# larskaislaniemi/PyLamp

Hardware: AMD Instinct MI355X
Metric: stokes_heat_mic_cell_updates_per_s (higher is better)
Workload: dtype f64

## Files before the change

include/pylamp_hip.h:

```cpp
#ifndef PYLAMP_HIP_H
#define PYLAMP_HIP_H

#include <stddef.h>
#include <stdint.h>

#ifdef __cplusplus
extern "C" {
#endif

typedef struct pl_ctx pl_ctx;

enum { PL_BC_NOSLIP = 0, PL_BC_FREESLIP = 1, PL_BC_CYCLIC = 2, PL_BC_FLOWTHRU = 4 };
enum { PL_BC_FIXTEMP = 0, PL_BC_FIXFLOW = 1 };
enum { PL_AVG_ARITHMETIC = 1, PL_AVG_GEOMETRIC = 2, PL_AVG_WEIGHTED = 4 };
enum { PL_INTERP_NEAREST = 8, PL_INTERP_LINEAR = 16, PL_INTERP_VELDIV = 32 };

typedef struct pl_solve_stats {
    int    iterations;
    int    converged;
    double rel_residual;
    double solve_ms;
    int    operator_applies;
    int    precond_applies;
    int    used_direct;
    int    reserved_;
    double error_estimate;
} pl_solve_stats;

int  pl_create(pl_ctx** out, int device, int nz, int nx, const double* zc, const double* xc);
void pl_destroy(pl_ctx* ctx);
const char* pl_last_error(const pl_ctx* ctx);
int  pl_sync(pl_ctx* ctx);
int  pl_device_info(pl_ctx* ctx, char* name, size_t name_len, int* cu_count, size_t* hbm_bytes);

typedef struct pl_comm_ops {
    int (*sendrecv)(void* user, int nmsg, const int* peer, const double* const* send, const int64_t* nsend,
                    double* const* recv, const int64_t* nrecv);
    int (*allreduce_host)(void* user, double* buf, int64_t n, int op);
    int (*allgather)(void* user, const double* send, double* recv, int64_t count);
    void* user;
} pl_comm_ops;
int  pl_set_comm(pl_ctx* ctx, int rank, int nranks, const pl_comm_ops* ops);
int  pl_set_comm_2d(pl_ctx* ctx, int rank, int Pz, int Px, const pl_comm_ops* ops);
int  pl_local_rows(pl_ctx* ctx, int* first_row, int* n_rows);
int  pl_local_block(pl_ctx* ctx, int* first_row, int* n_rows, int* first_col, int* n_cols, int* Pz, int* Px);
typedef struct pl_local_group pl_local_group;
int  pl_local_group_create(pl_local_group** out, int nranks);
void pl_local_group_destroy(pl_local_group* g);
void pl_local_group_abort(pl_local_group* g);
int  pl_set_comm_local(pl_ctx* ctx, pl_local_group* g, int rank, int Pz, int Px);
void pl_local_group_enter(pl_local_group* g);
void pl_local_group_leave(pl_local_group* g, pl_ctx* ctx);
int  pl_comm_info(pl_ctx* ctx, int* rank, int* nranks, int* native);
int  pl_comm_stats(pl_ctx* ctx, int64_t out[4], int reset);
int  pl_comm_times(pl_ctx* ctx, double out_ms[4], int reset);
int  pl_memcpy_d2h(pl_ctx* ctx, void* dst_host, const void* src_dev, size_t bytes);
int  pl_memcpy_h2d(pl_ctx* ctx, void* dst_dev, const void* src_host, size_t bytes);
int  pl_dev_add(pl_ctx* ctx, double* dst_dev, const double* src_dev, int64_t n);

int  pl_timer_start(pl_ctx* ctx);
int  pl_timer_stop_ms(pl_ctx* ctx, double* ms);

int  pl_stokes_set_coeffs(pl_ctx* ctx, const double* etas, const double* etan, const double* rho,
                          const int bc[4], int surfstab, double tstep, double theta);
int  pl_stokes_get_scaling(pl_ctx* ctx, double* kcont, double* kbond);
int  pl_stokes_apply(pl_ctx* ctx, const double* x, double* y);
int  pl_stokes_rhs(pl_ctx* ctx, double* rhs);
int  pl_stokes_residual_dd(pl_ctx* ctx, const double* rhs, const double* x, double* r);
int  pl_stokes_direct_info(pl_ctx* ctx, int* band, int* nb, double* factor_ms, double* solve_ms, int* nsolve);
int  pl_stokes_solve(pl_ctx* ctx, const double* rhs, double* x, int use_x0, double rtol,
                     int maxit, pl_solve_stats* stats);
int  pl_stokes_apply_bench(pl_ctx* ctx, int reps, double* avg_ms);
int  pl_stokes_apply_scaled_bench(pl_ctx* ctx, int reps, double* avg_ms);
int  pl_stream_triad_bench(pl_ctx* ctx, int64_t n, int reps, double* avg_ms);

int  pl_stokes_precond_apply(pl_ctx* ctx, const double* r, double* z);
int  pl_stokes_apply_reduce(pl_ctx* ctx, int mode, int rows, const double* x, const double* aux1, const double* aux2,
                            double* out, double* out2, double* sums);
int  pl_stokes_apply_probe(pl_ctx* ctx, int scaled, int mode, int rows, const double* x, const double* aux1,
                           const double* aux2, const double* add, double coef, double* out, double* out2, double* sums);
int  pl_stokes_scale_rows(pl_ctx* ctx, const double* v, double* out);
int  pl_stokes_mg_info(pl_ctx* ctx, int* nlevels, double* lmax, int max_levels);
int  pl_stokes_mg_plan(pl_ctx* ctx, int* smoother, int max_levels, int* nu, double* ratio, int* wall_ps);
int  pl_stokes_sweep_bench(pl_ctx* ctx, int reps, double* avg_ms);
int  pl_stokes_mg_precision(pl_ctx* ctx, int* nlevels, int* nlevels_fp32);
int  pl_stokes_set_mg_precision(pl_ctx* ctx, int fp32, long long min_nodes);
int  pl_mg_tail_launches(pl_ctx* ctx, long long* lds, long long* global);

int  pl_heat_set_coeffs(pl_ctx* ctx, const double* zmp, const double* xmp, const double* T,
                        const double* kz, const double* kx, const double* cp, const double* rho,
                        const double* H, const int bc[4], const double bcvalue[4], double tstep);
int  pl_heat_apply(pl_ctx* ctx, const double* x, double* y);
int  pl_heat_rhs(pl_ctx* ctx, double* rhs);
int  pl_heat_solve(pl_ctx* ctx, const double* rhs, double* x, double rtol, int maxit,
                   pl_solve_stats* stats);
int  pl_heat_apply_bench(pl_ctx* ctx, int reps, double* avg_ms);
int  pl_heat_fused_launches(pl_ctx* ctx, long long* n);

int  pl_trac2grid(pl_ctx* ctx, int64_t n, const double* tr_x, const double* tr_f, int64_t ld_f,
                  int nf, const int* avgscheme, double z0, double hz, double x0, double hx,
                  double* const* out);
int  pl_trac2grid_rect(pl_ctx* ctx, int64_t n, const double* tr_x, const double* tr_f, int64_t ld_f,
                       int nf, const int* avgscheme, const double* zc, const double* xc, double* const* out);
int  pl_mic_set_search(pl_ctx* ctx, int on);
int  pl_grid2trac(pl_ctx* ctx, int64_t n, const double* tr_x, int nf, const double* const* fields,
                  int gnz, int gnx, const double* gz, const double* gx, int method, double defval,
                  int stop_on_error, double* out, int64_t ld_out, int64_t* n_outside);
int  pl_rk4(pl_ctx* ctx, int64_t n, const double* tr_x, int gnz, int gnx, const double* gz,
            const double* gx, const double* vz, const double* vx, double tstep, double* v_out,
            double* x_out);

typedef struct pl_step_config {
    int    do_heatdiff, do_subgrid_heatdiff, tdep_rho, tdep_eta;
    double etamin, etamax, tref;
    double tstep_adv_max, tstep_adv_min, tstep_dif_max, tstep_dif_min, tstep_modifier;
    int    bcstokes[4];
    int    bcheat[4];
    double bcheatvals[4];
    double stokes_rtol, heat_rtol;
    int    stokes_maxit, heat_maxit;
    double length[2];
    int    tracdens, tracdens_min;
    uint64_t inject_seed;
    int    surface_stabilization;
    double surfstab_theta, surfstab_tstep;
    int    inject_unique_ids;
    int    tracs_fence_disabled;
} pl_step_config;

typedef struct pl_step_report {
    double tstep;
    int    limiter;
    double tstep_heat, tstep_stokes;
    pl_solve_stats stokes, heat;
    double ms_props, ms_scatter, ms_stokes, ms_heat, ms_gather, ms_advect, ms_sort, ms_total;
    int64_t ntrac;
    int64_t ninjected;
    int     stokes_resolves;
    int64_t nremoved;
} pl_step_report;

int  pl_tracers_upload(pl_ctx* ctx, int64_t n, const double* tr_x, const double* tr_f);
int  pl_tracers_download(pl_ctx* ctx, int64_t n, double* tr_x, double* tr_f);
int  pl_tracers_count(pl_ctx* ctx, int64_t* n);
int  pl_tracers_census(pl_ctx* ctx, int64_t ncells, int32_t* counts, int* first_cell_row, int* n_cell_rows);
int  pl_tracers_layout(pl_ctx* ctx, int* epoch_age, int* lazy);
int  pl_step(pl_ctx* ctx, const pl_step_config* cfg, int it, pl_step_report* rep);
int  pl_resident_scatter(pl_ctx* ctx, const pl_step_config* cfg, int it);
int  pl_resident_temp_to_tracers(pl_ctx* ctx, const pl_step_config* cfg, int first, const double* newtemp, double tstep);
int  pl_resident_rk4(pl_ctx* ctx, const double* vz_pad, const double* vx_pad, double tstep, int fence, const double length[2]);
int  pl_get_field(pl_ctx* ctx, const char* name, double* out);
int  pl_get_tracer_velocity(pl_ctx* ctx, int64_t n, double* out);

typedef struct pl3_ctx pl3_ctx;
int  pl3_create(pl3_ctx** out, int device, int nz, int nx, int ny, const double* zc, const double* xc, const double* yc);
void pl3_destroy(pl3_ctx* ctx);
const char* pl3_last_error(const pl3_ctx* ctx);
int  pl3_set_comm(pl3_ctx* ctx, pl_ctx* comm, int Pz, int Px, int Py);
int  pl3_local_block(pl3_ctx* ctx, int first[3], int count[3]);
int  pl3_comm_stats(pl3_ctx* ctx, int64_t out[2], int reset);
int  pl3_stokes_set_coeffs(pl3_ctx* ctx, const double* etas, const double* etan, const double* rho, const double grav[3]);
int  pl3_stokes_set_wall_rows(pl3_ctx* ctx, int slaved);
int  pl3_stokes_set_walls(pl3_ctx* ctx, const int bc[6]);
int  pl3_stokes_set_wall_velocity(pl3_ctx* ctx, const double vel[18]);
int  pl3_stokes_get_wall_velocity(pl3_ctx* ctx, double vel[18]);
int  pl3_stokes_get_scaling(pl3_ctx* ctx, double* kcont, double* kbond);
int  pl3_stokes_apply(pl3_ctx* ctx, const double* x, double* y);
int  pl3_stokes_rhs(pl3_ctx* ctx, double* rhs);
int  pl3_stokes_rhs_scaled(pl3_ctx* ctx, double* rhs);
int  pl3_stokes_solve(pl3_ctx* ctx, const double* rhs, double* x, int use_x0, double rtol, int maxit, pl_solve_stats* stats);
int  pl3_stokes_apply_bench(pl3_ctx* ctx, int scaled, int reps, double* avg_ms);
int  pl3_stokes_mg_info(pl3_ctx* ctx, int* nlevels, double* lmax, int max_levels);
int  pl3_stokes_precond_apply(pl3_ctx* ctx, const double* r, double* z);
int  pl3_stokes_mg_plan(pl3_ctx* ctx, int* nu, double* ratio, int* coarse_sweeps, double* coarse_ratio, int* lds, int max_levels);
int  pl3_heat_set_coeffs(pl3_ctx* ctx, const double* zmp, const double* xmp, const double* ymp, const double* T, const double* kz,
                         const double* kx, const double* ky, const double* cp, const double* rho, const double* H, const int bc[6],
                         const double bcvalue[6], double tstep);
int  pl3_heat_apply(pl3_ctx* ctx, const double* x, double* y);
int  pl3_heat_rhs(pl3_ctx* ctx, double* rhs);
int  pl3_heat_solve(pl3_ctx* ctx, const double* rhs, double* x, double rtol, int maxit, pl_solve_stats* stats);
int  pl3_get_solution(pl3_ctx* ctx, int which, double* out);

int  pl3_trac2grid(pl3_ctx* ctx, int64_t n, const double* tr_x, const double* tr_f, int64_t ld_f, int nf, const int* avgscheme,
                   const double* zc, int nzc, const double* xc, int nxc, const double* yc, int nyc, double* const* out);
int  pl3_grid2trac(pl3_ctx* ctx, int64_t n, const double* tr_x, int nf, const double* const* fields, int gnz, int gnx, int gny,
                   const double* gz, const double* gx, const double* gy, int method, double defval, int stop_on_error, double* out,
                   int64_t ld_out, int64_t* n_outside);
int  pl3_rk4(pl3_ctx* ctx, int64_t n, const double* tr_x, int gnz, int gnx, int gny, const double* gz, const double* gx, const double* gy,
             const double* vz, const double* vx, const double* vy, double tstep, double* v_out, double* x_out);
int  pl3_mic_set_search(pl3_ctx* ctx, int on);
int  pl3_mic_get_search(pl3_ctx* ctx, int* on);
int  pl3_mic_set_deletion(pl3_ctx* ctx, int on);
int  pl3_mic_get_deletion(pl3_ctx* ctx, int* on);
int  pl3_tracers_removed(pl3_ctx* ctx, int64_t out[2]);
int  pl3_tracers_upload(pl3_ctx* ctx, int64_t n, const double* tr_x, const double* tr_f);
int  pl3_tracers_download(pl3_ctx* ctx, int64_t n, double* tr_x, double* tr_f);
int  pl3_tracers_count(pl3_ctx* ctx, int64_t* n);
int  pl3_tracers_census(pl3_ctx* ctx, int64_t ncell, int32_t* counts);
int  pl3_resident_props(pl3_ctx* ctx, int tdep_rho, int tdep_eta, double tref, double etamin, double etamax);
int  pl3_resident_trac2grid(pl3_ctx* ctx, int nf, const int* columns, const int* avgscheme, const double* zc, int nzc, const double* xc,
                            int nxc, const double* yc, int nyc, double* const* out);
int  pl3_resident_temp_to_tracers(pl3_ctx* ctx, int absolute, const double* field, int subgrid, double tstep);
int  pl3_resident_rk4(pl3_ctx* ctx, const double* gz, const double* gx, const double* gy, const double* vz, const double* vx,
                      const double* vy, double tstep, int fence);
int  pl3_get_tracer_velocity(pl3_ctx* ctx, int64_t n, double* out);
int  pl3_resident_refill(pl3_ctx* ctx, int tracdens, int tracdens_min, uint64_t seed, int it, int unique_ids, int64_t out[4]);
int  pl3_resident_advect(pl3_ctx* ctx, const double* gz, const double* gx, const double* gy, const double* vz, const double* vx,
                         const double* vy, double tstep, int fence, int tracdens, int tracdens_min, uint64_t seed, int it,
                         int unique_ids, int64_t out[4]);
int  pl3_resident_times(pl3_ctx* ctx, double ms[4]);

typedef struct pl3_step_config {
    int    do_heatdiff, do_subgrid_heatdiff, tdep_rho, tdep_eta;
    double etamin, etamax, tref;
    double tstep_adv_max, tstep_adv_min, tstep_dif_max, tstep_dif_min, tstep_modifier;
    int    bcheat[6];
    double bcheatvals[6];
    double stokes_rtol, heat_rtol;
    int    stokes_maxit, heat_maxit;
    int    use_grav;
    int    reserved_;
    double grav[3];
    int    tracdens, tracdens_min;
    uint64_t inject_seed;
    int    inject_unique_ids;
    int    reserved2_;
} pl3_step_config;
typedef struct pl3_step_report {
    double tstep;
    int    limiter;
    int    reserved_;
    double tstep_heat, tstep_stokes;
    pl_solve_stats stokes, heat;
    int64_t ninjected, nrefilled, nempty, mincount;
    int64_t ntrac;
    int64_t nan_rho, nan_etas;
    double ms_scatter, ms_stokes, ms_heat, ms_gather, ms_rk4, ms_sort;
    double ms_total;
    int64_t nremoved;
} pl3_step_report;
// ... 13 lines not shown
```

pylamp_amd/_lib.py:

```python
import ctypes as C
import os

import numpy as np

_HERE = os.path.dirname(os.path.abspath(__file__))
LIB_PATH = os.path.join(_HERE, "libpylamp_hip.so")

c_double_p = C.POINTER(C.c_double)
c_int_p = C.POINTER(C.c_int)


class SolveStats(C.Structure):
    _fields_ = [("iterations", C.c_int), ("converged", C.c_int), ("rel_residual", C.c_double),
                ("solve_ms", C.c_double), ("operator_applies", C.c_int), ("precond_applies", C.c_int),
                ("used_direct", C.c_int), ("reserved_", C.c_int), ("error_estimate", C.c_double)]

    def as_dict(self):
        return {k: getattr(self, k) for k, _ in self._fields_}


class StepConfig(C.Structure):
    _fields_ = [("do_heatdiff", C.c_int), ("do_subgrid_heatdiff", C.c_int), ("tdep_rho", C.c_int),
                ("tdep_eta", C.c_int), ("etamin", C.c_double), ("etamax", C.c_double), ("tref", C.c_double),
                ("tstep_adv_max", C.c_double), ("tstep_adv_min", C.c_double), ("tstep_dif_max", C.c_double),
                ("tstep_dif_min", C.c_double), ("tstep_modifier", C.c_double), ("bcstokes", C.c_int * 4),
                ("bcheat", C.c_int * 4), ("bcheatvals", C.c_double * 4), ("stokes_rtol", C.c_double),
                ("heat_rtol", C.c_double), ("stokes_maxit", C.c_int), ("heat_maxit", C.c_int),
                ("length", C.c_double * 2), ("tracdens", C.c_int), ("tracdens_min", C.c_int),
                ("inject_seed", C.c_uint64), ("surface_stabilization", C.c_int), ("surfstab_theta", C.c_double),
                ("surfstab_tstep", C.c_double), ("inject_unique_ids", C.c_int), ("tracs_fence_disabled", C.c_int)]


class StepReport(C.Structure):
    _fields_ = [("tstep", C.c_double), ("limiter", C.c_int), ("tstep_heat", C.c_double),
                ("tstep_stokes", C.c_double), ("stokes", SolveStats), ("heat", SolveStats),
                ("ms_props", C.c_double), ("ms_scatter", C.c_double), ("ms_stokes", C.c_double),
                ("ms_heat", C.c_double), ("ms_gather", C.c_double), ("ms_advect", C.c_double),
                ("ms_sort", C.c_double), ("ms_total", C.c_double), ("ntrac", C.c_int64), ("ninjected", C.c_int64),
                ("stokes_resolves", C.c_int), ("nremoved", C.c_int64)]


class Step3Config(C.Structure):
    _fields_ = [("do_heatdiff", C.c_int), ("do_subgrid_heatdiff", C.c_int), ("tdep_rho", C.c_int), ("tdep_eta", C.c_int),
                ("etamin", C.c_double), ("etamax", C.c_double), ("tref", C.c_double),
                ("tstep_adv_max", C.c_double), ("tstep_adv_min", C.c_double), ("tstep_dif_max", C.c_double),
                ("tstep_dif_min", C.c_double), ("tstep_modifier", C.c_double), ("bcheat", C.c_int * 6),
                ("bcheatvals", C.c_double * 6), ("stokes_rtol", C.c_double), ("heat_rtol", C.c_double),
                ("stokes_maxit", C.c_int), ("heat_maxit", C.c_int), ("use_grav", C.c_int), ("reserved_", C.c_int),
                ("grav", C.c_double * 3), ("tracdens", C.c_int), ("tracdens_min", C.c_int), ("inject_seed", C.c_uint64),
                ("inject_unique_ids", C.c_int), ("reserved2_", C.c_int)]


class Step3Report(C.Structure):
    _fields_ = [("tstep", C.c_double), ("limiter", C.c_int), ("reserved_", C.c_int), ("tstep_heat", C.c_double),
                ("tstep_stokes", C.c_double), ("stokes", SolveStats), ("heat", SolveStats),
                ("ninjected", C.c_int64), ("nrefilled", C.c_int64), ("nempty", C.c_int64), ("mincount", C.c_int64),
                ("ntrac", C.c_int64), ("nan_rho", C.c_int64), ("nan_etas", C.c_int64),
                ("ms_scatter", C.c_double), ("ms_stokes", C.c_double), ("ms_heat", C.c_double), ("ms_gather", C.c_double),
                ("ms_rk4", C.c_double), ("ms_sort", C.c_double), ("ms_total", C.c_double), ("nremoved", C.c_int64)]


SIGNATURES = {
    "pl_create": (C.c_int, [C.POINTER(C.c_void_p), C.c_int, C.c_int, C.c_int, c_double_p, c_double_p]),
    "pl_destroy": (None, [C.c_void_p]),
    "pl_last_error": (C.c_char_p, [C.c_void_p]),
    "pl_sync": (C.c_int, [C.c_void_p]),
    "pl_abi_layout": (C.c_int, [C.POINTER(C.c_size_t)]),
    "pl3_create": (C.c_int, [C.POINTER(C.c_void_p), C.c_int, C.c_int, C.c_int, C.c_int, c_double_p, c_double_p, c_double_p]),
    "pl3_destroy": (None, [C.c_void_p]),
    "pl3_set_comm": (C.c_int, [C.c_void_p, C.c_void_p, C.c_int, C.c_int, C.c_int]),
    "pl3_local_block": (C.c_int, [C.c_void_p, c_int_p, c_int_p]),
    "pl3_comm_stats": (C.c_int, [C.c_void_p, C.POINTER(C.c_int64), C.c_int]),
    "pl3_last_error": (C.c_char_p, [C.c_void_p]),
    "pl3_stokes_set_coeffs": (C.c_int, [C.c_void_p, c_double_p, c_double_p, c_double_p, c_double_p]),
    "pl3_stokes_set_wall_rows": (C.c_int, [C.c_void_p, C.c_int]),
    "pl3_stokes_set_walls": (C.c_int, [C.c_void_p, C.POINTER(C.c_int)]),
    "pl3_stokes_set_wall_velocity": (C.c_int, [C.c_void_p, c_double_p]),
    "pl3_stokes_get_wall_velocity": (C.c_int, [C.c_void_p, c_double_p]),
    "pl3_stokes_get_scaling": (C.c_int, [C.c_void_p, c_double_p, c_double_p]),
    "pl3_stokes_apply": (C.c_int, [C.c_void_p, c_double_p, c_double_p]),
    "pl3_stokes_rhs": (C.c_int, [C.c_void_p, c_double_p]),
    "pl3_stokes_rhs_scaled": (C.c_int, [C.c_void_p, c_double_p]),
    "pl3_stokes_solve": (C.c_int, [C.c_void_p, c_double_p, c_double_p, C.c_int, C.c_double, C.c_int, C.POINTER(SolveStats)]),
    "pl3_stokes_apply_bench": (C.c_int, [C.c_void_p, C.c_int, C.c_int, c_double_p]),
    "pl3_stokes_mg_info": (C.c_int, [C.c_void_p, c_int_p, c_double_p, C.c_int]),
    "pl3_stokes_precond_apply": (C.c_int, [C.c_void_p, c_double_p, c_double_p]),
    "pl3_stokes_mg_plan": (C.c_int, [C.c_void_p, c_int_p, c_double_p, c_int_p, c_double_p, c_int_p, C.c_int]),
    "pl3_heat_set_coeffs": (C.c_int, [C.c_void_p] + [c_double_p] * 10 + [c_int_p, c_double_p, C.c_double]),
    "pl3_heat_apply": (C.c_int, [C.c_void_p, c_double_p, c_double_p]),
    "pl3_heat_rhs": (C.c_int, [C.c_void_p, c_double_p]),
    "pl3_heat_solve": (C.c_int, [C.c_void_p, c_double_p, c_double_p, C.c_double, C.c_int, C.POINTER(SolveStats)]),
    "pl3_get_solution": (C.c_int, [C.c_void_p, C.c_int, c_double_p]),
    "pl3_trac2grid": (C.c_int, [C.c_void_p, C.c_int64, c_double_p, c_double_p, C.c_int64, C.c_int, c_int_p, c_double_p, C.c_int,
                                c_double_p, C.c_int, c_double_p, C.c_int, C.POINTER(c_double_p)]),
    "pl3_grid2trac": (C.c_int, [C.c_void_p, C.c_int64, c_double_p, C.c_int, C.POINTER(c_double_p), C.c_int, C.c_int, C.c_int,
                                c_double_p, c_double_p, c_double_p, C.c_int, C.c_double, C.c_int, c_double_p, C.c_int64,
                                C.POINTER(C.c_int64)]),
    "pl3_rk4": (C.c_int, [C.c_void_p, C.c_int64, c_double_p, C.c_int, C.c_int, C.c_int] + [c_double_p] * 6 +
                [C.c_double, c_double_p, c_double_p]),
    "pl3_mic_set_search": (C.c_int, [C.c_void_p, C.c_int]),
    "pl3_mic_get_search": (C.c_int, [C.c_void_p, c_int_p]),
    "pl3_mic_set_deletion": (C.c_int, [C.c_void_p, C.c_int]),
    "pl3_mic_get_deletion": (C.c_int, [C.c_void_p, c_int_p]),
    "pl3_tracers_removed": (C.c_int, [C.c_void_p, C.POINTER(C.c_int64)]),
    "pl3_tracers_upload": (C.c_int, [C.c_void_p, C.c_int64, c_double_p, c_double_p]),
    "pl3_tracers_download": (C.c_int, [C.c_void_p, C.c_int64, c_double_p, c_double_p]),
    "pl3_tracers_count": (C.c_int, [C.c_void_p, C.POINTER(C.c_int64)]),
    "pl3_tracers_census": (C.c_int, [C.c_void_p, C.c_int64, C.POINTER(C.c_int32)]),
    "pl3_resident_props": (C.c_int, [C.c_void_p, C.c_int, C.c_int, C.c_double, C.c_double, C.c_double]),
    "pl3_resident_trac2grid": (C.c_int, [C.c_void_p, C.c_int, c_int_p, c_int_p, c_double_p, C.c_int, c_double_p, C.c_int,
                                         c_double_p, C.c_int, C.POINTER(c_double_p)]),
    "pl3_resident_temp_to_tracers": (C.c_int, [C.c_void_p, C.c_int, c_double_p, C.c_int, C.c_double]),
    "pl3_resident_rk4": (C.c_int, [C.c_void_p] + [c_double_p] * 6 + [C.c_double, C.c_int]),
    "pl3_get_tracer_velocity": (C.c_int, [C.c_void_p, C.c_int64, c_double_p]),
    "pl3_resident_refill": (C.c_int, [C.c_void_p, C.c_int, C.c_int, C.c_uint64, C.c_int, C.c_int, C.POINTER(C.c_int64)]),
    "pl3_resident_advect": (C.c_int, [C.c_void_p] + [c_double_p] * 6 + [C.c_double, C.c_int, C.c_int, C.c_int, C.c_uint64, C.c_int, C.c_int,
                                      C.POINTER(C.c_int64)]),
    "pl3_resident_times": (C.c_int, [C.c_void_p, c_double_p]),
    "pl3_resident_step": (C.c_int, [C.c_void_p, C.POINTER(Step3Config), C.c_int, C.POINTER(Step3Report)]),
    "pl3_get_field": (C.c_int, [C.c_void_p, C.c_char_p, c_double_p]),
    "pl3_advection_velocity": (C.c_int, [C.c_void_p] + [c_double_p] * 6),
    "pl3_transfer_stats": (C.c_int, [C.c_void_p, C.POINTER(C.c_int64), C.c_int]),
    "pl3_abi_layout": (C.c_int, [C.POINTER(C.c_size_t)]),
    "pl_device_info": (C.c_int, [C.c_void_p, C.c_char_p, C.c_size_t, c_int_p, C.POINTER(C.c_size_t)]),
    "pl_set_comm": (C.c_int, [C.c_void_p, C.c_int, C.c_int, C.c_void_p]),
    "pl_set_comm_2d": (C.c_int, [C.c_void_p, C.c_int, C.c_int, C.c_int, C.c_void_p]),
    "pl_local_rows": (C.c_int, [C.c_void_p, c_int_p, c_int_p]),
    "pl_local_block": (C.c_int, [C.c_void_p, c_int_p, c_int_p, c_int_p, c_int_p, c_int_p, c_int_p]),
    "pl_local_group_create": (C.c_int, [C.POINTER(C.c_void_p), C.c_int]),
    "pl_local_group_destroy": (None, [C.c_void_p]),
    "pl_local_group_abort": (None, [C.c_void_p]),
    "pl_local_group_enter": (None, [C.c_void_p]),
    "pl_local_group_leave": (None, [C.c_void_p, C.c_void_p]),
    "pl_set_comm_local": (C.c_int, [C.c_void_p, C.c_void_p, C.c_int, C.c_int, C.c_int]),
    "pl_comm_info": (C.c_int, [C.c_void_p, c_int_p, c_int_p, c_int_p]),
    "pl_comm_stats": (C.c_int, [C.c_void_p, C.POINTER(C.c_int64), C.c_int]),
    "pl_comm_times": (C.c_int, [C.c_void_p, c_double_p, C.c_int]),
    "pl_memcpy_d2h": (C.c_int, [C.c_void_p, C.c_void_p, C.c_void_p, C.c_size_t]),
    "pl_memcpy_h2d": (C.c_int, [C.c_void_p, C.c_void_p, C.c_void_p, C.c_size_t]),
    "pl_dev_add": (C.c_int, [C.c_void_p, c_double_p, c_double_p, C.c_int64]),
    "pl_timer_start": (C.c_int, [C.c_void_p]),
    "pl_timer_stop_ms": (C.c_int, [C.c_void_p, c_double_p]),
    "pl_stokes_set_coeffs": (C.c_int, [C.c_void_p, c_double_p, c_double_p, c_double_p, c_int_p, C.c_int,
                                       C.c_double, C.c_double]),
    "pl_stokes_get_scaling": (C.c_int, [C.c_void_p, c_double_p, c_double_p]),
    "pl_stokes_apply": (C.c_int, [C.c_void_p, c_double_p, c_double_p]),
    "pl_stokes_rhs": (C.c_int, [C.c_void_p, c_double_p]),
    "pl_stokes_residual_dd": (C.c_int, [C.c_void_p, c_double_p, c_double_p, c_double_p]),
    "pl_stokes_direct_info": (C.c_int, [C.c_void_p, c_int_p, c_int_p, c_double_p, c_double_p, c_int_p]),
    "pl_stokes_solve": (C.c_int, [C.c_void_p, c_double_p, c_double_p, C.c_int, C.c_double, C.c_int,
                                  C.POINTER(SolveStats)]),
    "pl_stokes_apply_bench": (C.c_int, [C.c_void_p, C.c_int, c_double_p]),
    "pl_stokes_apply_scaled_bench": (C.c_int, [C.c_void_p, C.c_int, c_double_p]),
    "pl_stream_triad_bench": (C.c_int, [C.c_void_p, C.c_int64, C.c_int, c_double_p]),
    "pl_stokes_precond_apply": (C.c_int, [C.c_void_p, c_double_p, c_double_p]),
    "pl_stokes_apply_reduce": (C.c_int, [C.c_void_p, C.c_int, C.c_int] + [c_double_p] * 6),
    "pl_stokes_apply_probe": (C.c_int, [C.c_void_p, C.c_int, C.c_int, C.c_int] + [c_double_p] * 4 + [C.c_double] + [c_double_p] * 3),
    "pl_stokes_scale_rows": (C.c_int, [C.c_void_p, c_double_p, c_double_p]),
    "pl_stokes_mg_info": (C.c_int, [C.c_void_p, c_int_p, c_double_p, C.c_int]),
    "pl_stokes_mg_plan": (C.c_int, [C.c_void_p, c_int_p, C.c_int, c_int_p, c_double_p, c_int_p]),
    "pl_stokes_mg_precision": (C.c_int, [C.c_void_p, c_int_p, c_int_p]),
    "pl_stokes_set_mg_precision": (C.c_int, [C.c_void_p, C.c_int, C.c_longlong]),
    "pl_stokes_sweep_bench": (C.c_int, [C.c_void_p, C.c_int, c_double_p]),
    "pl_mg_tail_launches": (C.c_int, [C.c_void_p, C.POINTER(C.c_longlong), C.POINTER(C.c_longlong)]),
    "pl_heat_set_coeffs": (C.c_int, [C.c_void_p] + [c_double_p] * 8 + [c_int_p, c_double_p, C.c_double]),
    "pl_heat_apply": (C.c_int, [C.c_void_p, c_double_p, c_double_p]),
    "pl_heat_rhs": (C.c_int, [C.c_void_p, c_double_p]),
    "pl_heat_solve": (C.c_int, [C.c_void_p, c_double_p, c_double_p, C.c_double, C.c_int, C.POINTER(SolveStats)]),
    "pl_heat_apply_bench": (C.c_int, [C.c_void_p, C.c_int, c_double_p]),
    "pl_heat_fused_launches": (C.c_int, [C.c_void_p, C.POINTER(C.c_longlong)]),
    "pl_trac2grid": (C.c_int, [C.c_void_p, C.c_int64, c_double_p, c_double_p, C.c_int64, C.c_int, c_int_p,
                               C.c_double, C.c_double, C.c_double, C.c_double, C.POINTER(c_double_p)]),
    "pl_trac2grid_rect": (C.c_int, [C.c_void_p, C.c_int64, c_double_p, c_double_p, C.c_int64, C.c_int, c_int_p,
                                    c_double_p, c_double_p, C.POINTER(c_double_p)]),
    "pl_mic_set_search": (C.c_int, [C.c_void_p, C.c_int]),
    "pl_grid2trac": (C.c_int, [C.c_void_p, C.c_int64, c_double_p, C.c_int, C.POINTER(c_double_p), C.c_int,
                               C.c_int, c_double_p, c_double_p, C.c_int, C.c_double, C.c_int, c_double_p,
                               C.c_int64, C.POINTER(C.c_int64)]),
    "pl_rk4": (C.c_int, [C.c_void_p, C.c_int64, c_double_p, C.c_int, C.c_int, c_double_p, c_double_p,
                         c_double_p, c_double_p, C.c_double, c_double_p, c_double_p]),
    "pl_tracers_upload": (C.c_int, [C.c_void_p, C.c_int64, c_double_p, c_double_p]),
    "pl_tracers_download": (C.c_int, [C.c_void_p, C.c_int64, c_double_p, c_double_p]),
    "pl_tracers_count": (C.c_int, [C.c_void_p, C.POINTER(C.c_int64)]),
    "pl_tracers_census": (C.c_int, [C.c_void_p, C.c_int64, C.POINTER(C.c_int32), c_int_p, c_int_p]),
    "pl_tracers_layout": (C.c_int, [C.c_void_p, c_int_p, c_int_p]),
    "pl_step": (C.c_int, [C.c_void_p, C.POINTER(StepConfig), C.c_int, C.POINTER(StepReport)]),
    "pl_resident_scatter": (C.c_int, [C.c_void_p, C.POINTER(StepConfig), C.c_int]),
    "pl_resident_temp_to_tracers": (C.c_int, [C.c_void_p, C.POINTER(StepConfig), C.c_int, c_double_p, C.c_double]),
    "pl_resident_rk4": (C.c_int, [C.c_void_p, c_double_p, c_double_p, C.c_double, C.c_int, c_double_p]),
    "pl_get_field": (C.c_int, [C.c_void_p, C.c_char_p, c_double_p]),
    "pl_get_tracer_velocity": (C.c_int, [C.c_void_p, C.c_int64, c_double_p]),
}

_lib = None


def load():
    global _lib
    if _lib is not None:
        return _lib
    if not os.path.exists(LIB_PATH):
        raise Exception("pylamp_amd: %s is missing — run `python -c 'import __graft_entry__ as g; g.build()'` "
                        "(there is no CPU fallback)" % LIB_PATH)
    try:
        import torch
    except Exception:
        pass
    lib = C.CDLL(LIB_PATH)
    for name, (res, args) in SIGNATURES.items():
        fn = getattr(lib, name)
        fn.restype = res
        fn.argtypes = args
    _lib = lib
    return lib


def dptr(a):
    return a.ctypes.data_as(c_double_p)


def f64(a):
    return np.ascontiguousarray(a, dtype=np.float64)


def check(ctx_handle, rc):
    if rc != 0:
        msg = load().pl_last_error(ctx_handle)
        raise Exception(msg.decode() if msg else "libpylamp_hip error %d" % rc)
```

pylamp_amd/csrc/pl_solver.hip:

```cpp
#include "pl_internal.h"
#include <chrono>
#include <cmath>
#include <functional>
#include <limits>

#define TB(tab, k) (tab)[(k) + PL_TOFF]

void pl_launch_heat_rhs(pl_ctx* ctx, const PlHeatOp& op, const double* Told, const double* H, double* rhs);

template <typename T>
struct PlVvOpT {
    PlGeom g;
    const T* etas; const T* etan;
    const T *rdz, *rDz, *rdx, *rDx;
    int slave_x;
    int slave_z0, slave_zL;
    T s0, sL;
    const T* szz; const T* szx;
};
typedef PlVvOpT<double> PlVvOp;
typedef PlVvOpT<float> PlVvOpF;

enum { VV_ZERO = 0, VV_INT = 1, VV_SLAVE = 2 };

// ... 1145 lines not shown
        fx = rs[c + P] * sum + 2.0 * op.Kc * rDx_j * (zp_c - prec_p_value(op, rs_p, i, j - 1, c - 1));
    }
    f[c] = (TF)(fz * fscale); f[c + P] = (TF)(fx * fscale); z[c + 2 * P] = zp_c;
}

template <typename TF>
__global__ __launch_bounds__(256) void k_prec_stage1(PlStokesOp op, PlVvOpT<TF> vop, const double* __restrict__ rs,
                                                     double* __restrict__ z, TF* __restrict__ f, int iters, double fscale) {
    PL_ROW_LOOP(op.g, iters) stage1_node(op, vop, rs, z, f, li, lj, fscale);
}

template <typename TF>
__global__ __launch_bounds__(256) void k_prec_stage1_v2(PlStokesOp op, PlVvOpT<TF> vop, const double* __restrict__ rs,
                                                        double* __restrict__ z, TF* __restrict__ f, TF* __restrict__ v1, double c2,
                                                        double fscale, double v1scale) {
    typedef typename PlVec2<TF>::type VF2;
    const PlGeom& g = op.g;
    const int lane = threadIdx.x;
    const int lj0 = (blockIdx.x * 64 + lane) * 2;
    const int li = blockIdx.y * 4 + threadIdx.y;
    if (li >= g.lnz) return;
    const bool has_right = (lj0 + 2) < g.lnx;
    const int p = g.pitch, nz = g.nz, nx = g.nx;
    const long long PLN = g.plane;
    const int c = (int)pl_idx(g, li, lj0);
    const int i = g.gi0 + li;
    const int jw = g.gj0 + blockIdx.x * 128;
    (void)nz; (void)nx;
    if (!stage1_fast_wave(g, i, jw, blockIdx.x, op.anchor_i, op.anchor_j, op.wall_ps)) {
        for (int q = 0; q < 2 && lj0 + q < g.lnx; q++) stage1_node(op, vop, rs, z, f, li, lj0 + q, fscale);
        return;
    }
#define ROW(ptr, dr, w, e) load_row2((ptr) + (long long)c - lj0 + (long long)(dr) * p, lj0, true, w, e, lane, has_right)
    const double2 rz = *reinterpret_cast<const double2*>(rs + c), rx = *reinterpret_cast<const double2*>(rs + PLN + c);
    const Row2 rp_i = ROW(rs + 2 * PLN, 0, true, false), rp_s = ROW(rs + 2 * PLN, -1, false, false);
    const Row2 en_s = ROW(op.etan, -1, false, false), en_i = ROW(op.etan, 0, true, false);
    const Row2 es_i = ROW(op.etas, 0, false, true), es_n = ROW(op.etas, 1, false, false);
#undef ROW
    const Row2 t_rdx = load_row2(g.rdx + PL_TOFF + g.gj0, lj0, true, true, false, lane, has_right);
    const Row2 t_rDx = load_row2(g.rDx + PL_TOFF + g.gj0, lj0, true, false, true, lane, has_right);
    const double rdz_i = TB(g.rdz, i), rdz_m = TB(g.rdz, i - 1), rDz_i = TB(g.rDz, i), rDz_p = TB(g.rDz, i + 1);
    const double Az = 4.0 * rdz_i * rDz_i, Azm = 4.0 * rdz_m * rDz_i, r2 = 2.0 * rdz_i, twoKc = 2.0 * op.Kc, Pz = twoKc * rDz_i;
    const double iKc = op.iKc;
    double fz[2], fx[2], zp[2], dz[2], dx[2];
    {
        const double rdx_j = t_rdx.v.x, rdx_m = t_rdx.w, rDx_j = t_rDx.v.x, rDx_p = t_rDx.v.y, k2 = 2.0 * rdx_j, B4 = 4.0 * rDx_j;
        zp[0] = rp_i.v.x * (rdx_j + rdz_i) * en_i.v.x * iKc;
        const double zp_s = rp_s.v.x * (rdx_j + rdz_m) * en_s.v.x * iKc, zp_w = rp_i.w * (rdx_m + rdz_i) * en_i.w * iKc;
        const double sz = en_i.v.x * Az + en_s.v.x * Azm + (es_i.v.y * k2) * rDx_p + (es_i.v.x * k2) * rDx_j;
        const double sx = en_i.v.x * (B4 * rdx_j) + en_i.w * (B4 * rdx_m) + (es_n.v.x * r2) * rDz_p + (es_i.v.x * r2) * rDz_i;
        fz[0] = rz.x * sz + Pz * (zp[0] - zp_s);
        fx[0] = rx.x * sx + (twoKc * rDx_j) * (zp[0] - zp_w);
        dz[0] = sz; dx[0] = sx;
    }
    {
        const double rdx_j = t_rdx.v.y, rdx_m = t_rdx.v.x, rDx_j = t_rDx.v.y, rDx_p = t_rDx.e, k2 = 2.0 * rdx_j, B4 = 4.0 * rDx_j;
        zp[1] = rp_i.v.y * (rdx_j + rdz_i) * en_i.v.y * iKc;
        const double zp_s = rp_s.v.y * (rdx_j + rdz_m) * en_s.v.y * iKc;
        const double sz = en_i.v.y * Az + en_s.v.y * Azm + (es_i.e * k2) * rDx_p + (es_i.v.y * k2) * rDx_j;
        const double sx = en_i.v.y * (B4 * rdx_j) + en_i.v.x * (B4 * rdx_m) + (es_n.v.y * r2) * rDz_p + (es_i.v.y * r2) * rDz_i;
        fz[1] = rz.y * sz + Pz * (zp[1] - zp_s);
        fx[1] = rx.y * sx + (twoKc * rDx_j) * (zp[1] - zp[0]);
        dz[1] = sz; dx[1] = sx;
    }
    *reinterpret_cast<VF2*>(f + c) = PlVec2<TF>::make((TF)(fz[0] * fscale), (TF)(fz[1] * fscale));
    *reinterpret_cast<VF2*>(f + PLN + c) = PlVec2<TF>::make((TF)(fx[0] * fscale), (TF)(fx[1] * fscale));
    *reinterpret_cast<double2*>(z + 2 * PLN + c) = make_double2(zp[0], zp[1]);
    if (v1) {
        const double nc2 = -c2 * v1scale;
        *reinterpret_cast<VF2*>(v1 + c) = PlVec2<TF>::make((TF)((nc2 * fz[0]) * pl_rcp(dz[0])), (TF)((nc2 * fz[1]) * pl_rcp(dz[1])));
        *reinterpret_cast<VF2*>(v1 + PLN + c) = PlVec2<TF>::make((TF)((nc2 * fx[0]) * pl_rcp(dx[0])), (TF)((nc2 * fx[1]) * pl_rcp(dx[1])));
    }
}

__global__ __launch_bounds__(256) void k_close_constraints(PlStokesOp op, PlVvOp vop, const double* __restrict__ bs,
                                                           double* __restrict__ x) {
    PL_NODE_PROLOGUE(op.g)
    const long long P = op.g.plane;
    int moff; double s;
    int cls = vv_cls_z(vop, i, j, moff, s);
    if (cls == VV_ZERO) x[c] = bs[c];
    else if (cls == VV_SLAVE) x[c] = s * x[c + moff] + bs[c];
    cls = vv_cls_x(vop, i, j, moff, s);
    if (cls == VV_ZERO) x[c + P] = bs[c + P];
    else if (cls == VV_SLAVE) {
        double g0 = bs[c + P];
        if (i == 0 && op.bc_z0 != PL_BC_FREESLIP) g0 /= (-TB(op.g.rDz, 1) - TB(op.g.rdz, 0));
        if (i == op.g.nz - 2 && op.bc_zL != PL_BC_FREESLIP) g0 /= (TB(op.g.rDz, op.g.nz - 2) + TB(op.g.rdz, op.g.nz - 2));
        x[c + P] = s * x[c + moff + P] + g0;
    }
}

#define PL_HYDRO_CHUNK 64
__global__ __launch_bounds__(64) void k_hydro_chunk(PlStokesOp op, double* __restrict__ x, double* __restrict__ ctot) {
    const PlGeom& g = op.g;
    const int lj = blockIdx.x * 64 + threadIdx.x, ch = blockIdx.y;
    if (lj >= g.lnx) return;
    double* P = x + 2 * g.plane;
    const double* r = op.rho;
    const int l0 = ch * PL_HYDRO_CHUNK, l1 = min(l0 + PL_HYDRO_CHUNK, g.lnz);
    const int jn = (g.gj0 + lj + 1 < g.nx) ? 1 : 0;
    double acc = 0.0;
    for (int li = l0; li < l1; li++) {
        const int i = g.gi0 + li;
        const long long c = pl_idx(g, li, lj);
        if (i >= 1 && i <= g.nz - 2) acc += 0.5 * (r[c] + r[c + jn]) * op.gz / (2.0 * op.Kc * TB(g.rDz, i));
        P[c] = acc;
    }
    ctot[(long long)ch * g.lnx + lj] = acc;
}
__global__ __launch_bounds__(64) void k_hydro_chunk_scan(PlGeom g, int nch, double* __restrict__ ctot, double* __restrict__ coltot) {
    const int lj = blockIdx.x * 64 + threadIdx.x;
    if (lj >= g.lnx) return;
    double acc = 0.0;
    for (int ch = 0; ch < nch; ch++) { const double t = ctot[(long long)ch * g.lnx + lj]; ctot[(long long)ch * g.lnx + lj] = acc; acc += t; }
    coltot[lj] = acc;
}
__global__ __launch_bounds__(256) void k_hydro_add(PlGeom g, double* __restrict__ x, const double* __restrict__ cpre) {
    PL_NODE_PROLOGUE(g)
    (void)i; (void)j;
    x[2 * g.plane + c] += cpre[(long long)(li / PL_HYDRO_CHUNK) * g.lnx + lj];
}

__global__ __launch_bounds__(256) void k_hydrostatic_apply_shift(PlStokesOp op, double* __restrict__ x,
                                                                 const double* __restrict__ prefix, double pa) {
    PL_NODE_PROLOGUE(op.g)
    const PlGeom& g = op.g;
    double* P = x + 2 * g.plane;
    x[c] = 0.0; x[c + g.plane] = 0.0;
    P[c] = (i >= g.nz - 1 || j >= g.nx - 1) ? 0.0 : P[c] + prefix[lj] - pa;
}

struct MgLevel {
    PlGeomHost gh;
    bool dist = false;
    PlGeom win{};
    long long win_shift = 0;
    PlVvOp op{};
    double* etas = nullptr; double* etan = nullptr; bool own_visc = false;
    double *rho = nullptr, *szz = nullptr, *szx = nullptr;
    double* eig = nullptr; bool eig_valid = false;
    int eig_confirm = 0, eig_skip = 0;
    bool own_rho = false;
    double* v[3] = {nullptr, nullptr, nullptr};
    double *f = nullptr, *r = nullptr;
    double lmax = 3.0;
    bool line_z = false;
    int line_ax = 0;
    bool f32 = false;
    PlVvOpF opf{};
    float *etas_f = nullptr, *etan_f = nullptr, *tab_f = nullptr;
    float* vf[3] = {nullptr, nullptr, nullptr};
    float *ff = nullptr, *rf = nullptr;
};
template <typename T> struct LevelT;
template <> struct LevelT<double> {
    static const PlVvOp& op(const MgLevel* L) { return L->op; }
    static double** v(MgLevel* L) { return L->v; }
    static double* f(MgLevel* L) { return L->f; }
    static double* r(MgLevel* L) { return L->r; }
};
template <> struct LevelT<float> {
    static const PlVvOpF& op(const MgLevel* L) { return L->opf; }
    static float** v(MgLevel* L) { return L->vf; }
    static float* f(MgLevel* L) { return L->ff; }
    static float* r(MgLevel* L) { return L->rf; }
};

struct PlSolver {
    std::vector<MgLevel*> levels;
    int bc_key[4] = {-1, -1, -1, -1};
    int repl_start = -1;
    long long repl_max_nodes = 300000;
    double *r = nullptr, *rt = nullptr, *p = nullptr, *v = nullptr, *s = nullptr, *t = nullptr, *y = nullptr,
           *z = nullptr, *b = nullptr, *x = nullptr, *xb = nullptr, *dx = nullptr, *r0 = nullptr, *xh = nullptr,
           *bu = nullptr;
    double* scal = nullptr;
    double* hpart = nullptr;
    double* epi = nullptr;
    long long epi_blocks = 0;
    int nu_pre = 2, nu_post = 2, coarse_sweeps = 12;
    int nu0_pre = -1, nu0_post = -1;
    bool aniso_auto = true, ratio_knob = false;
    int power_its_warm = 1;
    bool nu_auto = true;
    bool use_tail = true;
    bool any_line = false;
    long long tail_knob = 0;
    long long tail_max_nodes = 33 * 33;
    int min_cells = 4;
    bool f32_enable = false; long long f32_min_nodes = 200000;
    double etol = 3e-8;
    double kappa = 1.0, sigma = 1.0;
    bool defl_enable = true;
    bool defl_persistent = false;
    bool defl_valid = false, defl_active = false;
    double *wdefl = nullptr, *udefl = nullptr;
    double defl_yAw = 0.0, defl_wvel2 = 0.0;
    double* Awdefl = nullptr;
    bool defl_lazy = false;
    double schur_scale = 1.0;
    double ref_cached = 0.0, ref_kc = 0.0; int ref_age = 0;
    long long fused_max_nodes = 1100000;
    long long tile32_min_nodes = 250000;
    bool fused = true;
    bool fuse_first = true;
    bool l0_mixed = true;
    bool l0_mixed_now = true;
    bool deep = true;
    int tail_nu_pre = -1, tail_nu_post = -1;
    double cheb_ratio = 6.0, lmax_safety = 1.1;
    double* h[11] = {nullptr};
    double* hc3 = nullptr;
    double* hc[9] = {nullptr}; double* hc_part = nullptr; int hc_nb = 0, hc_last_its = 0;
    int napply = 0, nprec = 0;
    long long heat_fused_launches = 0;
    long long tail_lds_launches = 0, tail_global_launches = 0;
};

static PlSolver* solver_of(pl_ctx* ctx) {
    if (!ctx->krylov) {
        PlSolver* S = new PlSolver();
        if (const char* e = getenv("PYLAMP_MG_NU")) { int a = 0, b = 0; if (sscanf(e, "%d,%d", &a, &b) == 2 && a >= 0 && b >= 0 && a + b > 0) { S->nu_pre = a; S->nu_post = b; S->nu_auto = false; } }
        if (const char* e = getenv("PYLAMP_MG_NU0")) { int a = 0, b = 0; if (sscanf(e, "%d,%d", &a, &b) == 2 && a >= 1 && b >= 1) { S->nu0_pre = a; S->nu0_post = b; S->nu_auto = false; } }
        if (const char* e = getenv("PYLAMP_MG_POWER")) { int a = atoi(e); if (a >= 1) S->power_its_warm = a; }
        if (const char* e = getenv("PYLAMP_MG_COARSE")) { int a = atoi(e); if (a > 0) S->coarse_sweeps = a; }
        if (const char* e = getenv("PYLAMP_MG_TAIL")) S->use_tail = atoi(e) != 0;
        if (const char* e = getenv("PYLAMP_MG_REPL_NODES")) { long long v = atoll(e); if (v >= 25) S->repl_max_nodes = v; }
        if (const char* e = getenv("PYLAMP_MG_TAIL_NODES")) { long long v = atoll(e); if (v >= 25 && v <= PL_TAIL_MAX_NODES) S->tail_knob = v; }
        if (const char* e = getenv("PYLAMP_MG_DEEP")) S->deep = atoi(e) != 0;
        if (const char* e = getenv("PYLAMP_DEFLATE")) S->defl_enable = atoi(e) != 0;
        if (const char* e = getenv("PYLAMP_STOKES_ETOL")) { const double v = atof(e); if (v >= 0.0) S->etol = v; }
        if (const char* e = getenv("PYLAMP_MG_FP32")) S->f32_enable = atoi(e) != 0;
        if (const char* e = getenv("PYLAMP_MG_FP32_NODES")) { long long v = atoll(e); if (v >= 1) S->f32_min_nodes = v; }
        if (const char* e = getenv("PYLAMP_L0_MIXED")) S->l0_mixed = atoi(e) != 0;
        if (const char* e = getenv("PYLAMP_MG_FUSED")) S->fused = atoi(e) != 0;
        if (const char* e = getenv("PYLAMP_MG_TS32")) { long long v = atoll(e); if (v > 0) S->tile32_min_nodes = v; }
        if (const char* e = getenv("PYLAMP_MG_FUSED_MAX")) { long long v = atoll(e); if (v > 0) S->fused_max_nodes = v; }
        if (const char* e = getenv("PYLAMP_SCHUR_SCALE")) { double v = atof(e); if (v > 0.0) S->schur_scale = v; }
        if (const char* e = getenv("PYLAMP_MG_TAIL_NU")) { int a = 0, b = 0; if (sscanf(e, "%d,%d", &a, &b) == 2 && a + b > 0) { S->tail_nu_pre = a; S->tail_nu_post = b; } }
        if (const char* e = getenv("PYLAMP_MG_RATIO")) { double v = atof(e); if (v > 1.5) { S->cheb_ratio = v; S->ratio_knob = true; } }
        if (const char* e = getenv("PYLAMP_MG_ANISO")) S->aniso_auto = atoi(e) != 0;
        if (const char* e = getenv("PYLAMP_MG_SAFETY")) { double v = atof(e); if (v >= 1.0) S->lmax_safety = v; }
        ctx->krylov = S;
    }
    return (PlSolver*)ctx->krylov;
}

static void free_levels(PlSolver* S) {
    for (MgLevel* L : S->levels) {
        if (L->own_visc) { (void)hipFree(L->etas); (void)hipFree(L->etan); }
        if (L->own_rho && L->rho) (void)hipFree(L->rho);
        for (double* q : {L->szz, L->szx, L->eig}) if (q) (void)hipFree(q);
        for (double* q : {L->v[0], L->v[1], L->v[2], L->f, L->r}) if (q) (void)hipFree(q);
        for (float* q : {L->etas_f, L->etan_f, L->tab_f, L->vf[0], L->vf[1], L->vf[2], L->ff, L->rf}) if (q) (void)hipFree(q);
        pl_geom_free(L->gh);
        delete L;
    }
    S->levels.clear();
}

void pl_solver_free(pl_ctx* ctx) {
    PlSolver* S = (PlSolver*)ctx->krylov;
    if (!S) return;
    free_levels(S);
    for (double* q : {S->r, S->rt, S->p, S->v, S->s, S->t, S->y, S->z, S->b, S->x, S->xb, S->dx, S->r0, S->xh, S->bu, S->scal, S->wdefl, S->udefl, S->Awdefl})
        if (q) (void)hipFree(q);
    for (double* q : S->h) if (q) (void)hipFree(q);
    for (double* q : S->hc) if (q) (void)hipFree(q);
    if (S->hc_part) (void)hipFree(S->hc_part);
    if (S->hc3) (void)hipFree(S->hc3);
    if (S->hpart) (void)hipHostFree(S->hpart);
    if (S->epi) (void)hipFree(S->epi);
    delete S;
    ctx->krylov = nullptr;
}

static int dmalloc0(pl_ctx* ctx, double** p, size_t bytes) {
    PL_HIP(ctx, hipMalloc((void**)p, bytes));
    PL_HIP(ctx, hipMemsetAsync(*p, 0, bytes, ctx->stream));
    return 0;
}
static int scal_alloc(pl_ctx* ctx, PlSolver* S) {
    if (S->scal) return 0;
    PL_TRY(dmalloc0(ctx, &S->scal, (PL_SCAL_N + PL_PART_N * DOT_BLOCKS) * sizeof(double)));
    PL_HIP(ctx, hipHostMalloc((void**)&S->hpart, (PL_HSCAL + PL_SCAL_N) * sizeof(double)));
    return 0;
}

__global__ void k_scalar_alpha(double* __restrict__ sc, double rho_new) { sc[SC_ALPHA] = rho_new / sc[SC_SUM_A]; sc[SC_RHO] = rho_new; }
__global__ void k_s_update_dev(long long n, double* __restrict__ y, const double* __restrict__ a, const double* __restrict__ b,
                               const double* __restrict__ sc) {
    const double alpha = sc[SC_ALPHA];
    long long k = (long long)blockIdx.x * blockDim.x + threadIdx.x;
    for (; k < n; k += (long long)gridDim.x * blockDim.x) y[k] = a[k] - alpha * b[k];
}
template <bool FIRST>
__global__ void k_xrp_update_dev(long long n, double* __restrict__ x, const double* __restrict__ y, const double* __restrict__ z,
                                 double* __restrict__ r, const double* __restrict__ s, const double* __restrict__ t,
                                 double* __restrict__ p, const double* __restrict__ v, const double* __restrict__ sc,
                                 const double* __restrict__ wd, const double* __restrict__ awd, const double* __restrict__ p0) {
    const double alpha = sc[SC_ALPHA], omega = sc[SC_OMEGA], beta = sc[SC_BETA];
    const double cw = wd ? alpha * sc[SC_CY] + omega * sc[SC_CZ] : 0.0;
    const double cz = awd ? sc[SC_CZ] : 0.0;
    long long k = (long long)blockIdx.x * blockDim.x + threadIdx.x;
    for (; k < n; k += (long long)gridDim.x * blockDim.x) {
        double xn = FIRST ? alpha * y[k] + omega * z[k] : x[k] + alpha * y[k] + omega * z[k];
        if (wd) xn += cw * wd[k];
        x[k] = xn;
        const double rn = s[k] - omega * (awd ? t[k] + cz * awd[k] : t[k]);
        r[k] = rn;
        p[k] = rn + beta * ((FIRST ? p0[k] : p[k]) - omega * v[k]);
    }
}
__global__ void k_xr_update_dev(long long n, double* __restrict__ x, const double* __restrict__ y, const double* __restrict__ z,
                                double* __restrict__ r, const double* __restrict__ s, const double* __restrict__ t,
                                const double* __restrict__ sc) {
    const double alpha = sc[SC_ALPHA], omega = sc[SC_OMEGA];
    long long k = (long long)blockIdx.x * blockDim.x + threadIdx.x;
    for (; k < n; k += (long long)gridDim.x * blockDim.x) { x[k] += alpha * y[k] + omega * z[k]; r[k] = s[k] - omega * t[k]; }
}

__global__ __launch_bounds__(1024) void k_sum_partials(int nb, const double* __restrict__ part, double* __restrict__ out,
                                                       int mode = 0, double rho_new = 0.0) {
    double s0 = 0.0, s1 = 0.0;
    const int nt = blockDim.x, nw = nt >> 6;
#pragma unroll 2
    for (int k = threadIdx.x; k < nb; k += nt) { s0 += part[2 * k]; s1 += part[2 * k + 1]; }
    __shared__ double sh[2][16];
#pragma unroll
    for (int o = 32; o > 0; o >>= 1) { s0 += __shfl_down(s0, o, 64); s1 += __shfl_down(s1, o, 64); }
    if ((threadIdx.x & 63) == 0) { sh[0][threadIdx.x >> 6] = s0; sh[1][threadIdx.x >> 6] = s1; }
    __syncthreads();
    if (threadIdx.x == 0) {
        double a0 = sh[0][0], a1 = sh[1][0];
        for (int w = 1; w < nw; w++) { a0 += sh[0][w]; a1 += sh[1][w]; }
        out[0] = a0; out[1] = a1;
        if (mode == 1) { out[SC_ALPHA] = rho_new / a0; out[SC_RHO] = rho_new; }
    }
}

static int dots(pl_ctx* ctx, PlSolver* S, const PlGeom& g, int np, const double* a, const double* b, const double* c,
                const double* d, double* out2) {
    long long rows = (long long)g.lnz * np;
    const int nb = (int)(rows < DOT_BLOCKS ? rows : DOT_BLOCKS);
    if (a && c) hipLaunchKernelGGL((k_dot2<true, true>), dim3(nb), dim3(256), 0, ctx->stream, g, np, a, b, c, d, S->scal + SC_PART);
    else if (a) hipLaunchKernelGGL((k_dot2<true, false>), dim3(nb), dim3(256), 0, ctx->stream, g, np, a, b, c, d, S->scal + SC_PART);
    else hipLaunchKernelGGL((k_dot2<false, true>), dim3(nb), dim3(256), 0, ctx->stream, g, np, a, b, c, d, S->scal + SC_PART);
    if (ctx->nranks > 1 && pl_geom_is_dist(g)) {
        hipLaunchKernelGGL(k_sum_partials, dim3(1), dim3(256), 0, ctx->stream, nb, S->scal + SC_PART, S->scal + SC_SUM_A);
        PL_TRY(pl_comm_allreduce_dev(ctx, S->scal + SC_SUM_A, 2));
        PL_HIP(ctx, hipMemcpyAsync(S->hpart, S->scal + SC_SUM_A, 2 * sizeof(double), hipMemcpyDeviceToHost, ctx->stream));
        PL_HIP(ctx, hipStreamSynchronize(ctx->stream));
        out2[0] = S->hpart[0]; out2[1] = S->hpart[1];
        return 0;
    }
    PL_HIP(ctx, hipMemcpyAsync(S->hpart, S->scal + SC_PART, (size_t)2 * nb * sizeof(double), hipMemcpyDeviceToHost, ctx->stream));
    PL_HIP(ctx, hipStreamSynchronize(ctx->stream));
    double s0 = 0.0, s1 = 0.0;
    for (int k = 0; k < nb; k++) { s0 += S->hpart[2 * k]; s1 += S->hpart[2 * k + 1]; }
    out2[0] = s0; out2[1] = s1;
    return 0;
}

static int dots5_dev(pl_ctx* ctx, PlSolver* S, const PlGeom& g, int np, int nsplit, const double* t, const double* sv, const double* rt,
                     const double* aw_ride = nullptr) {
    long long rows = (long long)g.lnz * np;
    const int nb = (int)(rows < DOT_BLOCKS ? rows : DOT_BLOCKS);
    hipLaunchKernelGGL(k_dot5, dim3(nb), dim3(256), 0, ctx->stream, g, np, nsplit, t, sv, rt, S->scal + SC_PART);
    const bool reduce = ctx->nranks > 1 && pl_geom_is_dist(g);
    hipLaunchKernelGGL(k_sum_partials5, dim3(1), dim3(256), 0, ctx->stream, nb, S->scal + SC_PART, S->scal, reduce ? 0 : 1);
    if (reduce && aw_ride) {
        double* part2 = S->scal + SC_PART2;
        hipLaunchKernelGGL(k_dot4w, dim3(nb), dim3(256), 0, ctx->stream, g, np, nsplit, aw_ride, sv, t, part2);
        hipLaunchKernelGGL(k_sum_partials4, dim3(1), dim3(256), 0, ctx->stream, nb, (const double*)part2, S->scal + SC_AW_S);
        hipLaunchKernelGGL(k_bicg_pack_defl, dim3(1), dim3(64), 0, ctx->stream, S->scal);
        PL_TRY(pl_comm_allreduce_dev(ctx, S->scal + SC_STAGE, SC_STAGE_N));
        hipLaunchKernelGGL(k_bicg_unpack_defl, dim3(1), dim3(1), 0, ctx->stream, S->scal);
        return 0;
    }
    if (reduce) {
        PL_TRY(pl_comm_allreduce_dev(ctx, S->scal + SC_RED2, SC_RED2_N));
        hipLaunchKernelGGL(k_bicg_derive, dim3(1), dim3(1), 0, ctx->stream, S->scal);
    }
    return 0;
}
__global__ __launch_bounds__(256) void k_norm2_sum(PlGeom g, int nplanes, const double* __restrict__ a, const double* __restrict__ b,
                                                   double* __restrict__ part) {
    double s0 = 0.0;
// ... 410 lines not shown

static void level_nu(const PlSolver* S, size_t l, int& npre, int& npost) {
    npre = (l == 0 && S->nu0_pre > 0) ? S->nu0_pre : S->nu_pre;
    npost = (l == 0 && S->nu0_post > 0) ? S->nu0_post : S->nu_post;
}
static bool level_deep_plan(const PlSolver* S, const MgLevel* L, size_t l, int& e_last, int& f_depth) {
    int npre, npost;
    level_nu(S, l, npre, npost);
    e_last = std::max(2, npost);
    f_depth = e_last + std::max(npre, 1) - 1;
    if (!L->dist || !S->deep || l + 1 == S->levels.size() || npre < 1) return false;
    return f_depth <= PL_RING - 1 && f_depth + 1 <= std::min(L->gh.d.lnz, L->gh.d.lnx);
}

template <typename T> static void vcycle(pl_ctx* ctx, PlSolver* S, size_t l, const T* f, T** out, bool* wrote_final, double* final_out,
                                         double final_scale, int f_valid_depth, const int* first_done_anchor);
static bool mg_fused_level_ok(pl_ctx* ctx, const PlSolver* S, size_t l);
static bool mg_tail_lds_fits(const PlSolver* S, size_t l);
static bool mg_tail_cheb_fits(int nlev, int nu_pre, int nu_post, int coarse_sweeps);
__global__ void k_mg_tail_lds(TailArgs a);
static void vcycle_fused_level(pl_ctx* ctx, PlSolver* S, size_t l, const double* f, double** out, double* final_out, double final_scale,
                               const PlStokesOp* sop, const double* rs, double* z);

template <typename T, typename TC>
static void coarse_correction(pl_ctx* ctx, PlSolver* S, size_t l, MgLevel* L, MgLevel* C, T* buf[3], bool deep, int npost) {
    const PlGeom& g = L->gh.d;
    T* r = LevelT<T>::r(L);
    TC* cf = LevelT<TC>::f(C);
    const TC cscale = (std::is_same<T, float>::value && std::is_same<TC, double>::value) ? (TC)S->sigma : TC(1);
    if (L->dist && !C->dist) {
        PlVvOpT<TC> wop = LevelT<TC>::op(C); wop.g = C->win;
        const long long sh = C->win_shift;
        hipLaunchKernelGGL((k_vv_restrict<T, TC>), grid2d(C->win), dim3(64, 4), 0, ctx->stream, g, wop, (const T*)r, cf + sh, cscale);
        if constexpr (std::is_same<TC, double>::value) (void)pl_gather_blocks(ctx, C->gh.d, cf, 2, C->gh.d.plane);
    } else {
        hipLaunchKernelGGL((k_vv_restrict<T, TC>), grid2d(C->gh.d), dim3(64, 4), 0, ctx->stream, g, LevelT<TC>::op(C), (const T*)r, cf, cscale);
    }
    TC* ec = nullptr;
    bool wf = false;
    vcycle<TC>(ctx, S, l + 1, cf, &ec, &wf, nullptr, 1.0, 0, nullptr);
    const int pe = deep ? npost : (L->dist ? 1 : 0);
    if (C->dist)
        (void)pl_halo(ctx, C->gh.d, ec, 2, C->gh.d.plane, std::min(std::max((pe + 1) / 2 + 1, 2), std::min(PL_RING, std::min(C->gh.d.lnz, C->gh.d.lnx))));
    ExtViewT<T> V = ext_view<T>(ctx, L, pe);
    if (!deep && pe == 1) {
        V.op = LevelT<T>::op(L);
        const int lo = ctx->pz > 0 ? 1 : 0, hi = ctx->pz < ctx->Pz - 1 ? 1 : 0, we = ctx->px > 0 ? 1 : 0, ea = ctx->px < ctx->Px - 1 ? 1 : 0;
        V.op.g.gi0 -= lo; V.op.g.lnz += lo + hi; V.op.g.gj0 -= we; V.op.g.lnx += we + ea;
        V.sh = (long long)lo * g.pitch + we;
    }
    hipLaunchKernelGGL((k_vv_prolong_add<T, TC>), grid2d(V.op.g), dim3(64, 4), 0, ctx->stream, V.op, C->gh.d, (const TC*)ec, (const T*)(buf[0] - V.sh),
                       buf[2] - V.sh);
}

template <typename T>
static void vcycle(pl_ctx* ctx, PlSolver* S, size_t l, const T* f, T** out, bool* wrote_final, double* final_out,
                   double final_scale, int f_valid_depth, const int* first_done_anchor) {
    MgLevel* L = S->levels[l];
    const PlGeom& g = L->gh.d;
    *wrote_final = false;
    if constexpr (std::is_same<T, double>::value) {
        if (S->use_tail && !S->any_line && l > 0 && (long long)g.nz * g.nx <= S->tail_max_nodes &&
            S->levels.size() - l <= PL_TAIL_MAX_LEVELS && f == L->f) {
            TailArgs ta{};
            ta.nlev = (int)(S->levels.size() - l);
            ta.nu_pre = S->tail_nu_pre >= 0 ? S->tail_nu_pre : S->nu_pre; ta.nu_post = S->tail_nu_post >= 0 ? S->tail_nu_post : S->nu_post;
            ta.coarse_sweeps = coarsest_sweeps(S, S->levels.back()->gh.d); ta.ratio = S->cheb_ratio;
            for (int q = 0; q < ta.nlev; q++) {
                MgLevel* T_ = S->levels[l + q];
                ta.L[q].op = T_->op; ta.L[q].f = T_->f; ta.L[q].r = T_->r; ta.L[q].lmax = T_->lmax;
                for (int b = 0; b < 3; b++) ta.L[q].v[b] = T_->v[b];
            }
            if (S->fused && !L->dist && !L->op.szz && ta.nu_pre >= 1 && ta.nu_post >= 1 && ta.coarse_sweeps >= 1 && mg_tail_lds_fits(S, l) &&
                mg_tail_cheb_fits(ta.nlev, ta.nu_pre, ta.nu_post, ta.coarse_sweeps)) {
                hipLaunchKernelGGL(k_mg_tail_lds, dim3(1), dim3(1024), 0, ctx->stream, ta);
                S->tail_lds_launches++;
            } else {
                hipLaunchKernelGGL(k_mg_tail, dim3(1), dim3(1024), 0, ctx->stream, ta);
                S->tail_global_launches++;
            }
            *out = L->v[0];
            return;
        }
    }
    if constexpr (std::is_same<T, double>::value) {
        if (l > 0 && !final_out && f == L->f && mg_fused_level_ok(ctx, S, l)) {
            vcycle_fused_level(ctx, S, l, f, out, nullptr, 1.0, nullptr, nullptr, nullptr);
            return;
        }
    }
    T** lv = LevelT<T>::v(L);
    T* buf[3] = {lv[0], lv[1], lv[2]};
    const bool coarsest = l + 1 == S->levels.size();
    if (!coarsest && S->nu_pre == 0)
        (void)hipMemsetAsync(buf[0], 0, (size_t)2 * g.plane * sizeof(T), ctx->stream);
    if (coarsest) {
        double ratio = 0.4 * g.nz * g.nx; if (ratio < 30.0) ratio = 30.0;
        smooth<T>(ctx, L, buf, f, coarsest_sweeps(S, g), ratio, nullptr, 1.0, true);
        *out = buf[0];
        return;
    }
    int npre, npost, e_last, f_depth;
    level_nu(S, l, npre, npost);
    const bool deep = level_deep_plan(S, L, l, e_last, f_depth);
    MgLevel* C = S->levels[l + 1];
    T* r = LevelT<T>::r(L);
    if (deep) {
        if (f_valid_depth < f_depth) (void)pl_halo(ctx, g, (T*)f, 2, g.plane, f_depth);
        smooth<T>(ctx, L, buf, f, npre, S->cheb_ratio, nullptr, 1.0, true, false, e_last + npre - 1, first_done_anchor);
        const ExtViewT<T> V = ext_view<T>(ctx, L, e_last - 1);
        if (g_vv_vec)
            hipLaunchKernelGGL((k_vv_sweep2<1, T, T>), pl_grid_rows2(V.op.g), dim3(64, 4), 0, ctx->stream, V.op, (const T*)(buf[0] - V.sh),
                               (const T*)nullptr, f - V.sh, r - V.sh, T(0), T(0), T(1));
        else
            hipLaunchKernelGGL(k_vv_residual<T>, pl_grid_rows(V.op.g), dim3(64, 4), 0, ctx->stream, V.op, (const T*)(buf[0] - V.sh), f - V.sh,
                               r - V.sh, pl_row_iters(V.op.g));
    } else {
        smooth<T>(ctx, L, buf, f, npre, S->cheb_ratio, nullptr, 1.0, true, false, -1, first_done_anchor);
        if (L->dist) (void)pl_halo(ctx, g, buf[0], 2, g.plane);
        if (g_vv_vec)
            hipLaunchKernelGGL((k_vv_sweep2<1, T, T>), pl_grid_rows2(g), dim3(64, 4), 0, ctx->stream, LevelT<T>::op(L), (const T*)buf[0], (const T*)nullptr, f,
                               r, T(0), T(0), T(1));
        else
            hipLaunchKernelGGL(k_vv_residual<T>, pl_grid_rows(g), dim3(64, 4), 0, ctx->stream, LevelT<T>::op(L), (const T*)buf[0], f, r, pl_row_iters(g));
        if (L->dist) (void)pl_halo(ctx, g, r, 2, g.plane, 2);
    }
    if constexpr (std::is_same<T, float>::value) {
        if (C->f32) coarse_correction<float, float>(ctx, S, l, L, C, buf, deep, npost);
        else coarse_correction<float, double>(ctx, S, l, L, C, buf, deep, npost);
    } else {
        coarse_correction<double, double>(ctx, S, l, L, C, buf, deep, npost);
    }
    std::swap(buf[0], buf[2]);
    if (deep) *wrote_final = smooth<T>(ctx, L, buf, f, npost, S->cheb_ratio, final_out, final_scale, false, true, npost - 1);
    else *wrote_final = smooth<T>(ctx, L, buf, f, npost, S->cheb_ratio, final_out, final_scale, false, L->dist);
    *out = buf[0];
}

#define MGT_TS 16
#ifndef MGT_NT
#define MGT_NT 1024
#endif
struct MgTileArgs {
    PlVvOp op;
    PlVvOp opc;
    const double* f; double* fout;
    double* v;
    double* fc;
    const double* ec;
    double* out; double oscale; long long out_plane;
    double c1[4], c2[4];
    PlStokesOp sop; const double* rs; double* z;
    int tiles_x;
};

struct MgtTab { const double* es; const double* en; const double* rdz; const double* rDz; const double* rdx; const double* rDx; };

__device__ inline int mgt_cls_z(const PlVvOp& op, int i, int j, int& db, double& s) {
    db = 0; s = 1.0;
    if (i <= 0 || i >= op.g.nz - 1 || j < 0 || j >= op.g.nx - 1) return VV_ZERO;
    if (op.slave_x) {
        if (j == 0) { db = 1; return VV_SLAVE; }
        if (j == op.g.nx - 2) { db = -1; return VV_SLAVE; }
    }
    return VV_INT;
}
__device__ inline int mgt_cls_x(const PlVvOp& op, int i, int j, int& da, double& s) {
    const double s0 = op.s0, sL = op.sL;
    da = 0; s = 1.0;
    if (j <= 0 || j >= op.g.nx - 1 || i < 0 || i >= op.g.nz - 1) return VV_ZERO;
    if (i == 0 && op.slave_z0) da = 1;
    else if (i == op.g.nz - 2 && op.slave_zL) da = -1;
    s = da > 0 ? s0 : (da < 0 ? sL : 1.0);
    return da ? VV_SLAVE : VV_INT;
}
struct MgtC { double c0, c1, c2, c3, x0, x1, rdg, s, f; int cm, d; bool on, interior; };
template <bool ZC>
__device__ inline MgtC mgt_classify(const PlVvOp& op, int CR, int NR, int ci0, int cj0, int a, int b) {
    MgtC k; k.c0 = k.c1 = k.c2 = k.c3 = k.x0 = k.x1 = k.rdg = k.f = 0.0; k.s = 1.0; k.cm = a * CR + b; k.d = 0; k.on = false; k.interior = false;
    if (a < 1 || a > NR - 2 || b < 1 || b > CR - 2) return k;
    int d; double s;
    const int cls = ZC ? mgt_cls_z(op, ci0 + a, cj0 + b, d, s) : mgt_cls_x(op, ci0 + a, cj0 + b, d, s);
    const int am = ZC ? a : a + d, bm = ZC ? b + d : b;
    if (cls == VV_ZERO || am < 1 || am > NR - 2 || bm < 1 || bm > CR - 2) return k;
    k.s = s; k.cm = am * CR + bm; k.d = d; k.on = true; k.interior = cls == VV_INT;
    return k;
}
template <bool ZC>
__device__ inline void mgt_coefficients(MgtC& k, const MgtTab& t, int CR) {
    if (!k.on) return;
    const int c = k.cm, am = c / CR, bm = c - am * CR;
    if (ZC) {
        const double rdz_i = t.rdz[am + 1], rdz_m = t.rdz[am], rDz_i = t.rDz[am + 1];
        const double rdx_j = t.rdx[bm + 1], rDx_j = t.rDx[bm + 1], rDx_p = t.rDx[bm + 2];
        const double esC = t.es[c], esE = t.es[c + 1];
        k.c0 = 4.0 * t.en[c] * rdz_i * rDz_i; k.c1 = 4.0 * t.en[c - CR] * rdz_m * rDz_i;
        k.c2 = 2.0 * esE * rDx_p * rdx_j; k.c3 = 2.0 * esC * rDx_j * rdx_j;
        k.x0 = 2.0 * esE * rDz_i * rdx_j; k.x1 = 2.0 * esC * rDz_i * rdx_j;
    } else {
        const double rdx_j = t.rdx[bm + 1], rdx_m = t.rdx[bm], rDx_j = t.rDx[bm + 1];
        const double rdz_i = t.rdz[am + 1], rDz_i = t.rDz[am + 1], rDz_p = t.rDz[am + 2];
        const double esC = t.es[c], esN = t.es[c + CR];
        k.c0 = 4.0 * t.en[c] * rdx_j * rDx_j; k.c1 = 4.0 * t.en[c - 1] * rdx_m * rDx_j;
        k.c2 = 2.0 * esN * rDz_p * rdz_i; k.c3 = 2.0 * esC * rDz_i * rdz_i;
        k.x0 = 2.0 * esN * rDx_j * rdz_i; k.x1 = 2.0 * esC * rDx_j * rdz_i;
    }
    k.rdg = pl_rcp(k.c0 + k.c1 + k.c2 + k.c3);
}
__device__ inline double mgt_dg(const MgtC& k) { return k.c0 + k.c1 + k.c2 + k.c3; }
__device__ inline double mgt_av_z(const MgtC& k, int CR, const double* vz, const double* vx, double& v0) {
    const int c = k.cm; v0 = vz[c];
    return k.c0 * (vz[c + CR] - v0) - k.c1 * (v0 - vz[c - CR]) + k.c2 * (vz[c + 1] - v0) - k.c3 * (v0 - vz[c - 1]) +
           k.x0 * (vx[c + 1] - vx[c - CR + 1]) - k.x1 * (vx[c] - vx[c - CR]);
}
__device__ inline double mgt_av_x(const MgtC& k, int CR, const double* vz, const double* vx, double& v0) {
    const int c = k.cm; v0 = vx[c];
    return k.c0 * (vx[c + 1] - v0) - k.c1 * (v0 - vx[c - 1]) + k.c2 * (vx[c + CR] - v0) - k.c3 * (v0 - vx[c - CR]) +
           k.x0 * (vz[c + CR] - vz[c + CR - 1]) - k.x1 * (vz[c] - vz[c - 1]);
}
__device__ inline void mgt_cheb(const MgtC& kz, const MgtC& kx, int CR, const double* vz, const double* vx, double& pvz, double& pvx,
                                double c1, double c2, double& oz, double& ox) {
    oz = 0.0; ox = 0.0;
    if (kz.on) {
        double v0; const double Av = mgt_av_z(kz, CR, vz, vx, v0);
        const double mom = (c1 != 0.0) ? c1 * (v0 - pvz) : 0.0;
        oz = kz.s * (v0 + mom + (c2 * (Av - kz.f)) * kz.rdg);
        pvz = v0;
    }
    if (kx.on) {
        double v0; const double Av = mgt_av_x(kx, CR, vz, vx, v0);
        const double mom = (c1 != 0.0) ? c1 * (v0 - pvx) : 0.0;
        ox = kx.s * (v0 + mom + (c2 * (Av - kx.f)) * kx.rdg);
        pvx = v0;
    }
}
__device__ inline bool mgt_owns(int ra, int rb, int HC, int TS, int i, int j, const PlGeom& g) {
    return ra >= HC && (ra < HC + TS || (ra == HC + TS && i == g.nz - 1)) && rb >= HC && (rb < HC + TS || (rb == HC + TS && j == g.nx - 1));
}
__host__ __device__ constexpr int mgt_npt(int nn) { return (nn + 1023) / 1024; }
__host__ __device__ constexpr int mgt_nt(int nn) { return ((nn + mgt_npt(nn) - 1) / mgt_npt(nn) + 63) / 64 * 64; }
__host__ __device__ constexpr int mgt_pre_nn(int NS, int TS) { return (TS + 2 * (NS + 2)) * (TS + 2 * (NS + 2)); }
__host__ __device__ constexpr int mgt_post_nn(int NS, int TS) { return (TS + 2 * (NS + 1)) * (TS + 2 * (NS + 1)); }

template <int NPT> struct MgtRawE { double es[NPT], en[NPT], tab; };
template <int NPT> struct MgtRawF { double fz[NPT], fx[NPT]; };
template <int NPT> struct MgtRawV { double vz[NPT], vx[NPT]; };
struct MgtRawC { double ez, ex; };
#define MGT_SLOT(q) const int idx = tid + (q) * NT; const bool have = idx < CR * CR; \
    const int ra = have ? idx / CR : 0, rb = have ? idx % CR : 0, i = ci0 + ra, j = cj0 + rb; \
    const bool inmem = have && i - g.gi0 >= -PL_RING && i - g.gi0 < g.lnz + PL_RING && j - g.gj0 >= -PL_RING && j - g.gj0 < g.lnx + PL_RING; \
    const long long c = inmem ? pl_idx(g, i - g.gi0, j - g.gj0) : pl_idx(g, 0, 0);
#define MGT_TAB_SLOT const int w = __builtin_amdgcn_readfirstlane(tid >> 6), k = tid & 63; \
    const int gk = (w < 2 ? ci0 : cj0) - 1 + k, n = w < 2 ? g.nz : g.nx; \
    const bool intab = w < 4 && k < CR + 3 && gk >= -PL_TOFF && gk < n + PL_TOFF;
template <int NPT, int NT, int CR, int HC, int TS>
__device__ inline void mgt_fetch_visc(MgtRawE<NPT>& r, const MgTileArgs& a, int tile, int tid) {
    static_assert(CR + 3 <= 64 && NT >= 256, "one table per wave");
    const PlGeom& g = a.op.g;
    const int ci0 = g.gi0 + tile / a.tiles_x * TS - HC, cj0 = g.gj0 + tile % a.tiles_x * TS - HC;
    MGT_TAB_SLOT
    const double* const tab = w == 0 ? a.op.rdz : w == 1 ? a.op.rDz : w == 2 ? a.op.rdx : a.op.rDx;
    r.tab = TB(tab, intab ? gk : -PL_TOFF);
#pragma unroll
    for (int q = 0; q < NPT; q++) {
        MGT_SLOT(q)
        r.es[q] = a.op.etas[c]; r.en[q] = a.op.etan[c];
    }
}
template <int NPT, int NT, int CR, int HC, int TS>
__device__ inline void mgt_store_visc(const MgtRawE<NPT>& r, const MgTileArgs& a, int tile, double* es, double* en, double* tab, int tid) {
    const PlGeom& g = a.op.g;
    const int ci0 = g.gi0 + tile / a.tiles_x * TS - HC, cj0 = g.gj0 + tile % a.tiles_x * TS - HC;
#pragma unroll
    for (int q = 0; q < NPT; q++) {
        MGT_SLOT(q)
        (void)c;
        if (have) { es[idx] = inmem ? r.es[q] : 0.0; en[idx] = inmem ? r.en[q] : 0.0; }
    }
    MGT_TAB_SLOT
    if (w < 4 && k < CR + 3) tab[w * (CR + 4) + k] = intab ? r.tab : 0.0;
}
template <int NPT, int NT, int CR, int HC, int TS>
__device__ inline void mgt_fetch_rhs(MgtRawF<NPT>& r, const MgTileArgs& a, const double* fsrc, int tile, int tid) {
    const PlGeom& g = a.op.g;
    const int ci0 = g.gi0 + tile / a.tiles_x * TS - HC, cj0 = g.gj0 + tile % a.tiles_x * TS - HC;
#pragma unroll
    for (int q = 0; q < NPT; q++) {
        MGT_SLOT(q)
        const MgtC kz = mgt_classify<true>(a.op, CR, CR, ci0, cj0, ra, rb), kx = mgt_classify<false>(a.op, CR, CR, ci0, cj0, ra, rb);
        const long long c0 = pl_idx(g, 0, 0), cn = pl_idx(g, i - g.gi0, j - g.gj0);
        (void)c;
        r.fz[q] = fsrc[kz.on ? cn + kz.d : c0];
        r.fx[q] = fsrc[(kx.on ? cn + (long long)kx.d * g.pitch : c0) + g.plane];
    }
}
template <int NPT, int NT, int CR, int HC, int TS>
__device__ inline void mgt_fetch_v(MgtRawV<NPT>& r, const MgTileArgs& a, int tile, int tid) {
    const PlGeom& g = a.op.g;
    const int ci0 = g.gi0 + tile / a.tiles_x * TS - HC, cj0 = g.gj0 + tile % a.tiles_x * TS - HC;
#pragma unroll
    for (int q = 0; q < NPT; q++) {
        MGT_SLOT(q)
        r.vz[q] = a.v[c]; r.vx[q] = a.v[c + g.plane];
    }
}
template <int NPT, int NT, int CR, int HC, int TS>
__device__ inline void mgt_store_v(const MgtRawV<NPT>& r, const MgTileArgs& a, int tile, double* pvz, double* pvx, int tid) {
    const PlGeom& g = a.op.g;
    const int ci0 = g.gi0 + tile / a.tiles_x * TS - HC, cj0 = g.gj0 + tile % a.tiles_x * TS - HC;
#pragma unroll
    for (int q = 0; q < NPT; q++) {
        MGT_SLOT(q)
        (void)c;
        if (have) { pvz[idx] = inmem ? r.vz[q] : 0.0; pvx[idx] = inmem ? r.vx[q] : 0.0; }
    }
}
#define MGT_EC_SLOT const PlGeom& gc = a.opc.g; \
    const int e = min(tid, ECR * ECR - 1), I = ((a.op.g.gi0 + tile / a.tiles_x * TS - H) >> 1) - 2 + e / ECR, J = ((a.op.g.gj0 + tile % a.tiles_x * TS - H) >> 1) - 2 + e % ECR; \
    const bool inmem = I - gc.gi0 >= -PL_RING && I - gc.gi0 < gc.lnz + PL_RING && J - gc.gj0 >= -PL_RING && J - gc.gj0 < gc.lnx + PL_RING; \
    const long long cc = inmem ? pl_idx(gc, I - gc.gi0, J - gc.gj0) : pl_idx(gc, 0, 0);
template <int NT, int TS, int H, int ECR>
__device__ inline void mgt_fetch_ec(MgtRawC& r, const MgTileArgs& a, int tile, int tid) {
    static_assert(ECR * ECR <= NT, "one node of the coarse window per thread");
    MGT_EC_SLOT
    r.ez = a.ec[cc]; r.ex = a.ec[cc + gc.plane];
}
template <int NT, int TS, int H, int ECR>
__device__ inline void mgt_store_ec(const MgtRawC& r, const MgTileArgs& a, int tile, double* ecz, double* ecx, int tid) {
    MGT_EC_SLOT
    (void)cc;
    if (tid < ECR * ECR) { ecz[tid] = inmem ? r.ez : 0.0; ecx[tid] = inmem ? r.ex : 0.0; }
}
#undef MGT_EC_SLOT
#undef MGT_SLOT
#undef MGT_TAB_SLOT

template <int NS, bool L0, int TS, int EXT = 0>
__global__ __launch_bounds__(mgt_nt(mgt_pre_nn(NS + EXT, TS))) void k_mg_pre(MgTileArgs a) {
    constexpr int H = NS + 1 + EXT, HC = H + 1, CR = TS + 2 * HC, NN = CR * CR, NPT = mgt_npt(NN), NT = mgt_nt(NN);
    __shared__ double V[2][2][NN];
    __shared__ double ZP[L0 ? NN : 1];
    __shared__ double TAB[4][CR + 4];
    double* const ES = V[1][0]; double* const EN = V[1][1];
    const PlGeom& g = a.op.g;
    const int tid = threadIdx.x;
    MgtTab t; t.es = ES; t.en = EN; t.rdz = TAB[0]; t.rDz = TAB[1]; t.rdx = TAB[2]; t.rDx = TAB[3];
    const long long P = g.plane;
    const double* const fsrc = L0 ? a.rs : a.f;
    MgtRawE<NPT> rawe;
    MgtRawF<NPT> rawf;
    mgt_fetch_visc<NPT, NT, CR, HC, TS>(rawe, a, blockIdx.x, tid);
    mgt_fetch_rhs<NPT, NT, CR, HC, TS>(rawf, a, fsrc, blockIdx.x, tid);
    mgt_store_visc<NPT, NT, CR, HC, TS>(rawe, a, blockIdx.x, ES, EN, TAB[0], tid);
    const int tile = blockIdx.x, ty = tile / a.tiles_x, tx = tile % a.tiles_x;
    const int ti0 = g.gi0 + ty * TS, tj0 = g.gj0 + tx * TS;
    const int ci0 = ti0 - HC, cj0 = tj0 - HC;
    MgtC kz[NPT], kx[NPT];
    int depth[NPT];
#pragma unroll
    for (int q = 0; q < NPT; q++) {
        const int idx = tid + q * NT;
        const bool have = idx < NN;
        const int ra = have ? idx / CR : 0, rb = have ? idx % CR : 0, i = ci0 + ra, j = cj0 + rb;
        depth[q] = have ? min(min(ra, CR - 1 - ra), min(rb, CR - 1 - rb)) : -1;
        kz[q] = mgt_classify<true>(a.op, CR, CR, ci0, cj0, ra, rb);
        kx[q] = mgt_classify<false>(a.op, CR, CR, ci0, cj0, ra, rb);
        if (kz[q].on) kz[q].f = rawf.fz[q];
        if (kx[q].on) kx[q].f = rawf.fx[q];
        if (L0 && have) {
            const long long c = pl_idx(g, i - g.gi0, j - g.gj0);
            const bool indom = i >= 0 && i < g.nz && j >= 0 && j < g.nx;
            ZP[idx] = indom ? prec_p_value(a.sop, a.rs + 2 * P, i, j, c) : 0.0;
        }
    }
    __syncthreads();
#pragma unroll
    for (int q = 0; q < NPT; q++) {
        mgt_coefficients<true>(kz[q], t, CR); mgt_coefficients<false>(kx[q], t, CR);
        if (L0) {
            const int idx = tid + q * NT;
            const int ra = depth[q] >= 0 ? idx / CR : 0, rb = depth[q] >= 0 ? idx % CR : 0, i = ci0 + ra, j = cj0 + rb;
            if (kz[q].on) kz[q].f = kz[q].f * mgt_dg(kz[q]) + 2.0 * a.sop.Kc * TAB[1][ra + 1] * (ZP[kz[q].cm] - ZP[kz[q].cm - CR]);
            if (kx[q].on) kx[q].f = kx[q].f * mgt_dg(kx[q]) + 2.0 * a.sop.Kc * TAB[3][rb + 1] * (ZP[kx[q].cm] - ZP[kx[q].cm - 1]);
            if (depth[q] >= 0 && mgt_owns(ra, rb, HC, TS, i, j, g) && i < g.nz && j < g.nx && i - g.gi0 < g.lnz && j - g.gj0 < g.lnx) {
                const long long c = pl_idx(g, i - g.gi0, j - g.gj0);
                a.fout[c] = kz[q].interior ? kz[q].f : 0.0; a.fout[c + P] = kx[q].interior ? kx[q].f : 0.0; a.z[c + 2 * P] = ZP[idx];
            }
        }
    }
    int cur = 0;
#pragma unroll
    for (int q = 0; q < NPT; q++) {
        const int idx = tid + q * NT;
        if (depth[q] >= HC - H) {
            V[0][0][idx] = kz[q].on ? (-kz[q].s * a.c2[0] * kz[q].f) * kz[q].rdg : 0.0;
            V[0][1][idx] = kx[q].on ? (-kx[q].s * a.c2[0] * kx[q].f) * kx[q].rdg : 0.0;
        }
    }
    __syncthreads();
    double pvz[NPT], pvx[NPT];
#pragma unroll
    for (int q = 0; q < NPT; q++) { pvz[q] = 0.0; pvx[q] = 0.0; }
#pragma unroll
    for (int k = 1; k < NS; k++) {
        const int h = H - k;
#pragma unroll
        for (int q = 0; q < NPT; q++) {
            const int idx = tid + q * NT;
            if (depth[q] >= HC - h) {
                double oz, ox;
                mgt_cheb(kz[q], kx[q], CR, V[cur][0], V[cur][1], pvz[q], pvx[q], a.c1[k], a.c2[k], oz, ox);
                V[cur ^ 1][0][idx] = oz; V[cur ^ 1][1][idx] = ox;
            }
        }
        __syncthreads();
        cur ^= 1;
    }
    const int nxt = cur ^ 1;
#pragma unroll
    for (int q = 0; q < NPT; q++) {
        const int idx = tid + q * NT;
        if (depth[q] >= HC - 1) {
            double v0, rz = 0.0, rx = 0.0;
            if (kz[q].interior) rz = kz[q].f - mgt_av_z(kz[q], CR, V[cur][0], V[cur][1], v0);
            if (kx[q].interior) rx = kx[q].f - mgt_av_x(kx[q], CR, V[cur][0], V[cur][1], v0);
            V[nxt][0][idx] = rz; V[nxt][1][idx] = rx;
        }
        if (depth[q] >= HC - (EXT ? NS : 1)) {
            const int ra = idx / CR, rb = idx % CR, i = ci0 + ra, j = cj0 + rb, li = i - g.gi0, lj = j - g.gj0;
            const bool owned = li >= 0 && li < g.lnz && lj >= 0 && lj < g.lnx;
            const bool ring = EXT && !owned && li >= -NS && li < g.lnz + NS && lj >= -NS && lj < g.lnx + NS;
            if (i >= 0 && i < g.nz && j >= 0 && j < g.nx && ((owned && mgt_owns(ra, rb, HC, TS, i, j, g)) || ring)) {
                const long long c = pl_idx(g, li, lj);
                a.v[c] = V[cur][0][idx]; a.v[c + P] = V[cur][1][idx];
            }
        }
    }
    __syncthreads();
    const PlGeom& gc = a.opc.g;
    for (int idx = tid; idx < (TS / 2 + 1) * (TS / 2 + 1); idx += NT) {
        const int u_ = idx / (TS / 2 + 1), w_ = idx % (TS / 2 + 1);
        const int I = (ti0 >> 1) + u_, J = (tj0 >> 1) + w_;
        if ((u_ == TS / 2 && I != gc.nz - 1) || (w_ == TS / 2 && J != gc.nx - 1)) continue;
        if (I >= gc.nz || J >= gc.nx || 2 * I - g.gi0 >= g.lnz || 2 * J - g.gj0 >= g.lnx) continue;
        const int b0 = (2 * I - ci0) * CR + (2 * J - cj0);
        int d; double s;
        double oz = 0.0, ox = 0.0;
        if (vv_cls_z(a.opc, I, J, d, s) == VV_INT) {
            const double wz[3] = {0.25, 0.5, 0.25}, wx[4] = {0.125, 0.375, 0.375, 0.125};
#pragma unroll
            for (int u = 0; u < 3; u++)
#pragma unroll
                for (int w = 0; w < 4; w++) oz += wz[u] * wx[w] * V[nxt][0][b0 + (u - 1) * CR + (w - 1)];
        }
        if (vv_cls_x(a.opc, I, J, d, s) == VV_INT) {
            const double wz[4] = {0.125, 0.375, 0.375, 0.125}, wx[3] = {0.25, 0.5, 0.25};
#pragma unroll
            for (int u = 0; u < 4; u++)
#pragma unroll
                for (int w = 0; w < 3; w++) ox += wz[u] * wx[w] * V[nxt][1][b0 + (u - 1) * CR + (w - 1)];
        }
        const long long cc = pl_idx(gc, I - gc.gi0, J - gc.gj0);
        a.fc[cc] = oz; a.fc[cc + gc.plane] = ox;
    }
}

template <int NS, int TS>
__global__ __launch_bounds__(mgt_nt(mgt_post_nn(NS, TS))) void k_mg_post(MgTileArgs a) {
    constexpr int H = NS, HC = H + 1, CR = TS + 2 * HC, NN = CR * CR, ECR = TS / 2 + H + 6, ENN = ECR * ECR, NPT = mgt_npt(NN), NT = mgt_nt(NN);
    __shared__ double V[2][2][NN];
    __shared__ double EC[2][ENN];
    __shared__ double TAB[4][CR + 4];
    double* const ES = V[0][0]; double* const EN = V[0][1];
    double* const PVz = V[1][0]; double* const PVx = V[1][1];
    const PlGeom& g = a.op.g; const PlGeom& gc = a.opc.g;
    const int tid = threadIdx.x;
    MgtTab t; t.es = ES; t.en = EN; t.rdz = TAB[0]; t.rDz = TAB[1]; t.rdx = TAB[2]; t.rDx = TAB[3];
    MgtRawV<NPT> rawv;
    MgtRawC rawc;
    MgtRawE<NPT> rawe;
    MgtRawF<NPT> rawf;
    mgt_fetch_v<NPT, NT, CR, HC, TS>(rawv, a, blockIdx.x, tid);
    mgt_fetch_ec<NT, TS, H, ECR>(rawc, a, blockIdx.x, tid);
    mgt_fetch_visc<NPT, NT, CR, HC, TS>(rawe, a, blockIdx.x, tid);
    mgt_fetch_rhs<NPT, NT, CR, HC, TS>(rawf, a, a.f, blockIdx.x, tid);
    mgt_store_v<NPT, NT, CR, HC, TS>(rawv, a, blockIdx.x, PVz, PVx, tid);
    mgt_store_ec<NT, TS, H, ECR>(rawc, a, blockIdx.x, EC[0], EC[1], tid);
    mgt_store_visc<NPT, NT, CR, HC, TS>(rawe, a, blockIdx.x, ES, EN, TAB[0], tid);
    const int tile = blockIdx.x, ty = tile / a.tiles_x, tx = tile % a.tiles_x;
    const int ti0 = g.gi0 + ty * TS, tj0 = g.gj0 + tx * TS;
    const int ci0 = ti0 - HC, cj0 = tj0 - HC;
    const int eI0 = ((ti0 - H) >> 1) - 2, eJ0 = ((tj0 - H) >> 1) - 2;
    MgtC kz[NPT], kx[NPT];
    int depth[NPT];
#pragma unroll
    for (int q = 0; q < NPT; q++) {
        const int idx = tid + q * NT;
        const bool have = idx < NN;
        const int ra = have ? idx / CR : 0, rb = have ? idx % CR : 0;
        depth[q] = have ? min(min(ra, CR - 1 - ra), min(rb, CR - 1 - rb)) : -1;
        kz[q] = mgt_classify<true>(a.op, CR, CR, ci0, cj0, ra, rb);
        kx[q] = mgt_classify<false>(a.op, CR, CR, ci0, cj0, ra, rb);
        if (kz[q].on) kz[q].f = rawf.fz[q];
        if (kx[q].on) kx[q].f = rawf.fx[q];
    }
    __syncthreads();
#pragma unroll
    for (int q = 0; q < NPT; q++) { mgt_coefficients<true>(kz[q], t, CR); mgt_coefficients<false>(kx[q], t, CR); }
    __syncthreads();
    auto ecz = [&](int I, int J) { return EC[0][(I - eI0) * ECR + (J - eJ0)]; };
    auto ecx = [&](int I, int J) { return EC[1][(I - eI0) * ECR + (J - eJ0)]; };
#pragma unroll
    for (int q = 0; q < NPT; q++) {
        const int idx = tid + q * NT;
        if (depth[q] >= HC - H) {
            const int ra = idx / CR, rb = idx % CR, i = ci0 + ra, j = cj0 + rb;
            int d; double s;
            double oz = 0.0, ox = 0.0;
            if (mgt_cls_z(a.op, i, j, d, s) != VV_ZERO) {
                const int jm = j + d;
                const int I0 = i >> 1, I1 = (i + 1) >> 1;
                int Jn = jm >> 1, Jo = (jm & 1) ? Jn + 1 : Jn - 1;
                Jn = min(max(Jn, 0), gc.nx - 2); Jo = min(max(Jo, 0), gc.nx - 2);
                const double pa = 0.5 * (ecz(I0, Jn) + ecz(I1, Jn)), pb = 0.5 * (ecz(I0, Jo) + ecz(I1, Jo));
                oz = s * (PVz[idx + d] + (0.75 * pa + 0.25 * pb));
            }
            if (mgt_cls_x(a.op, i, j, d, s) != VV_ZERO) {
                const int im = i + d;
                const int J0 = j >> 1, J1 = (j + 1) >> 1;
                int In = im >> 1, Io = (im & 1) ? In + 1 : In - 1;
                In = min(max(In, 0), gc.nz - 2); Io = min(max(Io, 0), gc.nz - 2);
                const double pa = 0.5 * (ecx(In, J0) + ecx(In, J1)), pb = 0.5 * (ecx(Io, J0) + ecx(Io, J1));
                ox = s * (PVx[idx + d * CR] + (0.75 * pa + 0.25 * pb));
            }
            V[0][0][idx] = oz; V[0][1][idx] = ox;
        }
    }
    __syncthreads();
    int cur = 0;
    double pvz[NPT], pvx[NPT];
#pragma unroll
    for (int q = 0; q < NPT; q++) { pvz[q] = 0.0; pvx[q] = 0.0; }
#pragma unroll
    for (int k = 0; k < NS; k++) {
        const int h = H - 1 - k;
#pragma unroll
        for (int q = 0; q < NPT; q++) {
            const int idx = tid + q * NT;
            if (depth[q] >= HC - h) {
                double oz, ox;
                mgt_cheb(kz[q], kx[q], CR, V[cur][0], V[cur][1], pvz[q], pvx[q], k == 0 ? 0.0 : a.c1[k], a.c2[k], oz, ox);
                if (k == NS - 1) {
                    const int ra = idx / CR, rb = idx % CR, i = ci0 + ra, j = cj0 + rb;
                    if (i < g.nz && j < g.nx && i - g.gi0 < g.lnz && j - g.gj0 < g.lnx) {
                        const long long c = pl_idx(g, i - g.gi0, j - g.gj0); a.out[c] = oz * a.oscale; a.out[c + a.out_plane] = ox * a.oscale;
                    }
                } else { V[cur ^ 1][0][idx] = oz; V[cur ^ 1][1][idx] = ox; }
            }
        }
        if (k < NS - 1) { __syncthreads(); cur ^= 1; }
    }
#pragma unroll
    for (int q = 0; q < NPT; q++) {
        const int idx = tid + q * NT;
        if (depth[q] == HC - 1) {
            const int ra = idx / CR, rb = idx % CR, i = ci0 + ra, j = cj0 + rb;
            if (mgt_owns(ra, rb, HC, TS, i, j, g) && i - g.gi0 < g.lnz && j - g.gj0 < g.lnx) {
                const long long c = pl_idx(g, i - g.gi0, j - g.gj0); a.out[c] = 0.0; a.out[c + a.out_plane] = 0.0;
            }
        }
    }
}

#define MGT_TAIL_POOL 18600
#define MGT_TAIL_CHEB 256
#define MGT_TAIL_LDS 11520
struct TailLvl { int base, NR, CR, N; };
#define TL_V(D, buf, c) (pool + (D).base + (2 * (buf) + (c)) * (D).N)
#define TL_ES(D) (pool + (D).base + 4 * (D).N)
#define TL_EN(D) (pool + (D).base + 5 * (D).N)
#define TL_TAB(D, k) (pool + (D).base + 6 * (D).N + ((k) < 2 ? (k) * ((D).NR + 3) : 2 * ((D).NR + 3) + ((k) - 2) * ((D).CR + 3)))
__host__ __device__ inline TailLvl mgt_tail_lvl(const PlGeom& g, int base) {
    TailLvl D; D.base = base; D.NR = g.nz + 2; D.CR = g.nx + 2; D.N = D.NR * D.CR;
    return D;
}
__host__ __device__ inline int mgt_tail_lvl_size(const TailLvl& D) { return 6 * D.N + 2 * (D.NR + 3) + 2 * (D.CR + 3); }
struct MgtTailRows {
    MgtC kz, kx; int ij, o;
    __device__ inline int i() const { return ij >> 16; }
    __device__ inline int j() const { return ij & 0xffff; }
};
__device__ inline int mgt_tail_dz(const MgtTailRows& R) { return R.kz.cm - R.o; }
__device__ inline int mgt_tail_dx(const MgtTailRows& R) { const int t = R.kx.cm - R.o; return (t > 0) - (t < 0); }
__device__ inline double mgt_uniform(double x) {
    const long long b = __double_as_longlong(x);
    const unsigned lo = __builtin_amdgcn_readfirstlane((unsigned)b), hi = __builtin_amdgcn_readfirstlane((unsigned)(b >> 32));
    return __longlong_as_double((long long)(((unsigned long long)hi << 32) | lo));
}
__device__ inline void mgt_tail_rows(MgtTailRows& R, const PlVvOp& op, const TailLvl& D, int q) {
    const int nxm = op.g.nx - 1;
    const int i = q / nxm, j = q - i * nxm;
    R.ij = i << 16 | j; R.o = (i + 1) * D.CR + (j + 1);
    R.kz = mgt_classify<true>(op, D.CR, D.NR, -1, -1, i + 1, j + 1);
    R.kx = mgt_classify<false>(op, D.CR, D.NR, -1, -1, i + 1, j + 1);
    const double s0 = op.s0, sL = op.sL;
    R.kx.s = R.kx.d > 0 ? s0 : (R.kx.d < 0 ? sL : 1.0);
}
__device__ inline void mgt_tail_coefficients(double* pool, const TailLvl& D, MgtTailRows& R) {
    MgtTab t; t.es = TL_ES(D); t.en = TL_EN(D); t.rdz = TL_TAB(D, 0); t.rDz = TL_TAB(D, 1); t.rdx = TL_TAB(D, 2); t.rDx = TL_TAB(D, 3);
    mgt_coefficients<true>(R.kz, t, D.CR); mgt_coefficients<false>(R.kx, t, D.CR);
}
__device__ inline void mgt_tail_cheb_coeffs(double* ch, double lmax, double ratio, int n) {
    const double lmin = lmax / ratio;
    const double theta = 0.5 * (lmax + lmin), delta = 0.5 * (lmax - lmin), sigma = theta / delta;
    double rho_old = 1.0 / sigma;
    for (int k = 0; k < n; k++) {
        double c1, c2;
        if (k == 0) { c1 = 0.0; c2 = 1.0 / theta; }
        else { const double rho = 1.0 / (2.0 * sigma - rho_old); c1 = rho * rho_old; c2 = 2.0 * rho / delta; rho_old = rho; }
        ch[2 * k] = c1; ch[2 * k + 1] = c2;
    }
}
__device__ inline void mgt_tail_smooth(double* pool, const double* ch, const TailLvl& D, MgtTailRows& R, bool mine, int& cur, int nsweep, bool zero_guess) {
    double pvz = 0.0, pvx = 0.0;
    double c1 = mgt_uniform(ch[0]), c2 = mgt_uniform(ch[1]);
    for (int k = 0; k < nsweep; k++) {
        if (mine) {
            double oz, ox;
            if (k == 0 && zero_guess) {
                oz = R.kz.on ? (-R.kz.s * c2 * R.kz.f) * R.kz.rdg : 0.0;
                ox = R.kx.on ? (-R.kx.s * c2 * R.kx.f) * R.kx.rdg : 0.0;
            } else {
                mgt_cheb(R.kz, R.kx, D.CR, TL_V(D, cur, 0), TL_V(D, cur, 1), pvz, pvx, c1, c2, oz, ox);
            }
            TL_V(D, cur ^ 1, 0)[R.o] = oz; TL_V(D, cur ^ 1, 1)[R.o] = ox;
        }
        double n1 = 0.0, n2 = 0.0;
        if (k + 1 < nsweep) { n1 = ch[2 * k + 2]; n2 = ch[2 * k + 3]; }
        __syncthreads();
        c1 = mgt_uniform(n1); c2 = mgt_uniform(n2);
        cur ^= 1;
    }
}
__device__ inline void mgt_tail_residual(double* pool, const TailLvl& D, const MgtTailRows& R, bool mine, int cur) {
    if (mine) {
        double v0, rz = 0.0, rx = 0.0;
        if (R.kz.interior) rz = R.kz.f - mgt_av_z(R.kz, D.CR, TL_V(D, cur, 0), TL_V(D, cur, 1), v0);
        if (R.kx.interior) rx = R.kx.f - mgt_av_x(R.kx, D.CR, TL_V(D, cur, 0), TL_V(D, cur, 1), v0);
        TL_V(D, cur ^ 1, 0)[R.o] = rz; TL_V(D, cur ^ 1, 1)[R.o] = rx;
    }
    __syncthreads();
}
__device__ inline void mgt_tail_prolong(double* pool, const TailLvl& D, const TailLvl& Dc, const PlGeom& gc, const MgtTailRows& R, bool mine, int cur,
                                        int curc) {
    if (mine) {
        const double* const ez = TL_V(Dc, curc, 0); const double* const ex = TL_V(Dc, curc, 1);
        double oz = 0.0, ox = 0.0;
        if (R.kz.on) {
            const int i = R.i(), jm = R.j() + mgt_tail_dz(R), I0 = i >> 1, I1 = (i + 1) >> 1;
            int Jn = jm >> 1, Jo = (jm & 1) ? Jn + 1 : Jn - 1;
            Jn = min(max(Jn, 0), gc.nx - 2); Jo = min(max(Jo, 0), gc.nx - 2);
            const double pa = 0.5 * (ez[(I0 + 1) * Dc.CR + Jn + 1] + ez[(I1 + 1) * Dc.CR + Jn + 1]);
            const double pb = 0.5 * (ez[(I0 + 1) * Dc.CR + Jo + 1] + ez[(I1 + 1) * Dc.CR + Jo + 1]);
            oz = R.kz.s * (TL_V(D, cur, 0)[R.kz.cm] + (0.75 * pa + 0.25 * pb));
        }
        if (R.kx.on) {
            const int im = R.i() + mgt_tail_dx(R), j = R.j(), J0 = j >> 1, J1 = (j + 1) >> 1;
            int In = im >> 1, Io = (im & 1) ? In + 1 : In - 1;
            In = min(max(In, 0), gc.nz - 2); Io = min(max(Io, 0), gc.nz - 2);
            const double pa = 0.5 * (ex[(In + 1) * Dc.CR + J0 + 1] + ex[(In + 1) * Dc.CR + J1 + 1]);
            const double pb = 0.5 * (ex[(Io + 1) * Dc.CR + J0 + 1] + ex[(Io + 1) * Dc.CR + J1 + 1]);
            ox = R.kx.s * (TL_V(D, cur, 1)[R.kx.cm] + (0.75 * pa + 0.25 * pb));
        }
        TL_V(D, cur ^ 1, 0)[R.o] = oz; TL_V(D, cur ^ 1, 1)[R.o] = ox;
    }
    __syncthreads();
}
__global__ __launch_bounds__(MGT_NT) void k_mg_tail_lds(TailArgs a) {
    __shared__ double pool[MGT_TAIL_LDS];
    __shared__ double chb[2 * MGT_TAIL_CHEB];
    const int tid = threadIdx.x;
    const int nlev = a.nlev, ksm = max(a.nu_pre, a.nu_post);
    const TailLevel& L0 = a.L[0]; const PlGeom& g0 = L0.op.g; const TailLvl D0 = mgt_tail_lvl(g0, 0);
    MgtTailRows A, B = {};
    B.kz.s = 1.0;
    const bool haveA = tid < (g0.nz - 1) * (g0.nx - 1);
    mgt_tail_rows(A, L0.op, D0, haveA ? tid : 0);
    if (haveA) {
        const long long c = pl_idx(g0, A.i() - g0.gi0, A.j() - g0.gj0);
        if (A.kz.on) A.kz.f = L0.f[c + A.kz.d];
        if (A.kx.on) A.kx.f = L0.f[c + (long long)A.kx.d * g0.pitch + g0.plane];
    }
    double e0[2][2]; int e0o[2];
#pragma unroll
    for (int q = 0; q < 2; q++) {
        const int idx = tid + q * MGT_NT;
        const bool ok = idx < g0.nz * g0.nx;
        const int i = ok ? idx / g0.nx : 0, j = ok ? idx - i * g0.nx : 0;
        const long long c = pl_idx(g0, i - g0.gi0, j - g0.gj0);
        e0[q][0] = L0.op.etas[c]; e0[q][1] = L0.op.etan[c];
        e0o[q] = ok ? (i + 1) * D0.CR + (j + 1) : -1;
    }
    int lb = 0, eco = -1, ecN = 0;
    bool riz = false, rix = false;
    const double* pes = nullptr; const double* pen = nullptr;
    {
        int base = mgt_tail_lvl_size(D0), start = 0, vstart = 0;
        for (int l = 1; l < nlev; l++) {
            const PlVvOp& op = a.L[l].op; const PlGeom& g = op.g; const TailLvl D = mgt_tail_lvl(g, base);
            const int n = (g.nz - 1) * (g.nx - 1), nv = g.nz * g.nx;
            if (tid >= start && tid < start + n) {
                lb = l;
                mgt_tail_rows(B, op, D, tid - start);
                int d; double s;
                riz = B.kz.on && mgt_cls_z(op, B.i(), B.j() + B.kz.d, d, s) == VV_INT;
                rix = B.kx.on && mgt_cls_x(op, B.i() + B.kx.d, B.j(), d, s) == VV_INT;
            }
            if (tid >= vstart && tid < vstart + nv) {
                const int q = tid - vstart, i = q / g.nx, j = q - i * g.nx;
                const long long c = pl_idx(g, i - g.gi0, j - g.gj0);
                pes = op.etas + c; pen = op.etan + c;
                eco = D.base + 4 * D.N + (i + 1) * D.CR + (j + 1); ecN = D.N;
            }
            start = (start + n + 63) & ~63; vstart += nv; base += mgt_tail_lvl_size(D);
        }
    }
    int tdst = -1;
    const double* ptab = nullptr;
    {
        int base = 0, tstart = 0;
        for (int l = 0; l < nlev; l++) {
            const PlVvOp& op = a.L[l].op; const TailLvl D = mgt_tail_lvl(op.g, base);
#pragma unroll
            for (int k = 0; k < 4; k++) {
                const double* const tab = k == 0 ? op.rdz : k == 1 ? op.rDz : k == 2 ? op.rdx : op.rDx;
                const int n = k < 2 ? op.g.nz : op.g.nx, count = n + 5, e = tid - tstart;
                if (e >= 0 && e < count) { tdst = (int)(TL_TAB(D, k) - pool) + e; ptab = e < n + 2 * PL_TOFF ? tab + e : nullptr; }
                tstart += count;
            }
            base += mgt_tail_lvl_size(D);
        }
    }
    const double ec0 = pes ? *pes : 0.0, ec1 = pen ? *pen : 0.0, tabv = ptab ? *ptab : 0.0;
    {
        const int l = __builtin_amdgcn_readfirstlane(tid >> 6);
        if (l < nlev && (tid & 63) == 0) {
            const PlGeom& g = a.L[l].op.g;
            double ratio = 0.4 * g.nz * g.nx; if (ratio < 30.0) ratio = 30.0;
            if (l == nlev - 1) mgt_tail_cheb_coeffs(chb + 2 * l * ksm, a.L[l].lmax, ratio, a.coarse_sweeps);
            else mgt_tail_cheb_coeffs(chb + 2 * l * ksm, a.L[l].lmax, a.ratio, ksm);
        }
    }
    {
        int base = 0;
        for (int l = 0; l < nlev; l++) {
            const TailLvl D = mgt_tail_lvl(a.L[l].op.g, base);
            for (int k = tid; k < 4 * D.N; k += MGT_NT) pool[base + k] = 0.0;
            base += mgt_tail_lvl_size(D);
        }
    }
#pragma unroll
    for (int q = 0; q < 2; q++)
        if (e0o[q] >= 0) { TL_ES(D0)[e0o[q]] = e0[q][0]; TL_EN(D0)[e0o[q]] = e0[q][1]; }
    if (eco >= 0) { pool[eco] = ec0; pool[eco + ecN] = ec1; }
    if (tdst >= 0) pool[tdst] = tabv;
    __syncthreads();
    if (haveA) mgt_tail_coefficients(pool, D0, A);
    int base = mgt_tail_lvl_size(D0);
    for (int l = 1; l < nlev; l++) {
        const TailLvl D = mgt_tail_lvl(a.L[l].op.g, base);
        if (lb == l) mgt_tail_coefficients(pool, D, B);
        base += mgt_tail_lvl_size(D);
    }
    const int cur_pre = a.nu_pre & 1, cur_coarse = a.coarse_sweeps & 1, cur_post = (a.nu_pre + 1 + a.nu_post) & 1;
    int cur = 0;
    if (nlev == 1) {
        mgt_tail_smooth(pool, chb, D0, A, haveA, cur, a.coarse_sweeps, true);
    } else {
        TailLvl D = D0;
        for (int l = 0; l < nlev; l++) {
            const bool coarsest = l == nlev - 1, mine = l == 0 ? haveA : lb == l;
            const double* const ch = chb + 2 * l * ksm;
            cur = 0;
            if (l == 0) {
                mgt_tail_smooth(pool, ch, D, A, mine, cur, a.nu_pre, true);
                mgt_tail_residual(pool, D, A, mine, cur);
            } else {
                mgt_tail_smooth(pool, ch, D, B, mine, cur, coarsest ? a.coarse_sweeps : a.nu_pre, true);
                if (coarsest) break;
                mgt_tail_residual(pool, D, B, mine, cur);
            }
            if (lb == l + 1) {
                const double* const rz = TL_V(D, cur ^ 1, 0); const double* const rx = TL_V(D, cur ^ 1, 1);
                const int rbz = (2 * B.i() + 1) * D.CR + 2 * (B.j() + mgt_tail_dz(B)) + 1;
                const int rbx = (2 * (B.i() + mgt_tail_dx(B)) + 1) * D.CR + 2 * B.j() + 1;
                double oz = 0.0, ox = 0.0;
                if (riz) {
                    const double wz[3] = {0.25, 0.5, 0.25}, wx[4] = {0.125, 0.375, 0.375, 0.125};
#pragma unroll
                    for (int u = 0; u < 3; u++)
#pragma unroll
                        for (int w = 0; w < 4; w++) oz += wz[u] * wx[w] * rz[rbz + (u - 1) * D.CR + (w - 1)];
                }
                if (rix) {
                    const double wz[4] = {0.125, 0.375, 0.375, 0.125}, wx[3] = {0.25, 0.5, 0.25};
#pragma unroll
                    for (int u = 0; u < 4; u++)
#pragma unroll
                        for (int w = 0; w < 3; w++) ox += wz[u] * wx[w] * rx[rbx + (u - 1) * D.CR + (w - 1)];
                }
                B.kz.f = oz; B.kx.f = ox;
            }
            __syncthreads();
            D = mgt_tail_lvl(a.L[l + 1].op.g, D.base + mgt_tail_lvl_size(D));
        }
        for (int l = nlev - 2; l >= 0; l--) {
            const TailLvl Dc = D;
            D = mgt_tail_lvl(a.L[l].op.g, 0); D.base = Dc.base - mgt_tail_lvl_size(D);
            const double* const ch = chb + 2 * l * ksm;
            const int curc = l + 1 == nlev - 1 ? cur_coarse : cur_post;
            cur = cur_pre;
            if (l == 0) {
                mgt_tail_prolong(pool, D, Dc, a.L[l + 1].op.g, A, haveA, cur, curc);
                cur ^= 1;
                mgt_tail_smooth(pool, ch, D, A, haveA, cur, a.nu_post, false);
            } else {
                mgt_tail_prolong(pool, D, Dc, a.L[l + 1].op.g, B, lb == l, cur, curc);
                cur ^= 1;
                mgt_tail_smooth(pool, ch, D, B, lb == l, cur, a.nu_post, false);
            }
        }
    }
    {
        const double* const cz = TL_V(D0, cur, 0); const double* const cx = TL_V(D0, cur, 1);
        for (int idx = tid; idx < g0.nz * g0.nx; idx += MGT_NT) {
            const int i = idx / g0.nx, j = idx - i * g0.nx, o = (i + 1) * D0.CR + (j + 1);
            const long long c = pl_idx(g0, i - g0.gi0, j - g0.gj0);
            L0.v[0][c] = cz[o]; L0.v[0][c + g0.plane] = cx[o];
        }
    }
}
static bool mg_tail_cheb_fits(int nlev, int nu_pre, int nu_post, int coarse_sweeps) {
    return (long long)(nlev - 1) * std::max(nu_pre, nu_post) + coarse_sweeps <= MGT_TAIL_CHEB;
}
static bool mg_tail_lds_fits(const PlSolver* S, size_t l) {
    long long need = 0, lds = 0, coarse_threads = 0, coarse_nodes = 0, table_entries = 0;
    for (size_t q = l; q < S->levels.size(); q++) {
        const PlGeom& g = S->levels[q]->gh.d;
        need += 10LL * (g.nz + 2) * (g.nx + 2) + 2LL * (g.nz + 5) + 2LL * (g.nx + 5);
        lds += mgt_tail_lvl_size(mgt_tail_lvl(g, 0)); table_entries += 2LL * (g.nz + 5) + 2LL * (g.nx + 5);
        if (q > l) { coarse_threads = (coarse_threads + 63) / 64 * 64 + (long long)(g.nz - 1) * (g.nx - 1); coarse_nodes += (long long)g.nz * g.nx; }
    }
    const PlGeom& g0 = S->levels[l]->gh.d;
    return need <= MGT_TAIL_POOL && lds <= MGT_TAIL_LDS && (long long)(g0.nz - 1) * (g0.nx - 1) <= MGT_NT && (long long)g0.nz * g0.nx <= 2 * MGT_NT &&
           coarse_threads <= MGT_NT && coarse_nodes <= MGT_NT && table_entries <= MGT_NT;
}

static void cheb_coeffs(double lmax, double ratio, int n, double* c1, double* c2) {
    const double lmin = lmax / ratio, theta = 0.5 * (lmax + lmin), delta = 0.5 * (lmax - lmin), sigma = theta / delta;
    double rho_old = 1.0 / sigma;
    for (int k = 0; k < n; k++) {
        if (k == 0) { c1[k] = 0.0; c2[k] = 1.0 / theta; }
        else { const double rho = 1.0 / (2.0 * sigma - rho_old); c1[k] = rho * rho_old; c2[k] = 2.0 * rho / delta; rho_old = rho; }
    }
}
static bool mg_fused_level_ok(pl_ctx* ctx, const PlSolver* S, size_t l) {
    if (!S->fused || l + 1 >= S->levels.size() || S->any_line) return false;
    const MgLevel* L = S->levels[l];
    if (L->f32 || L->op.szz) return false;
    const PlGeom& g = L->gh.d;
    int npre_, npost_;
    level_nu(S, l, npre_, npost_);
    if (L->dist) {
        const bool dist_fused = !(getenv("PYLAMP_MG_FUSED_DIST") && atoi(getenv("PYLAMP_MG_FUSED_DIST")) == 0);
        const MgLevel* C = S->levels[l + 1];
        if (!dist_fused || l == 0 || npre_ + 2 > std::min(g.lnz, g.lnx) || npre_ + 3 > PL_RING) return false;
        if (C->dist && std::min(C->gh.d.lnz, C->gh.d.lnx) < 4) return false;
        if ((g.gi0 & 1) || (g.gj0 & 1)) return false;
    } else if (S->levels[l + 1]->dist) return false;
    if ((long long)g.lnz * g.lnx > S->fused_max_nodes) return false;
    if (S->use_tail && l > 0 && (long long)g.nz * g.nx <= S->tail_max_nodes && S->levels.size() - l <= PL_TAIL_MAX_LEVELS) return false;
    int npre, npost;
    level_nu(S, l, npre, npost);
    return npre >= 1 && npre <= 3 && npost >= 1 && npost <= 3;
}
static void vcycle_fused_level(pl_ctx* ctx, PlSolver* S, size_t l, const double* f, double** out, double* final_out, double final_scale,
                               const PlStokesOp* sop, const double* rs, double* z) {
    MgLevel* L = S->levels[l];
    MgLevel* C = S->levels[l + 1];
    const PlGeom& g = L->gh.d;
    int npre, npost;
    level_nu(S, l, npre, npost);
    MgTileArgs a{};
    a.op = L->op; a.opc = C->op;
    a.f = rs ? (const double*)L->f : f; a.fout = L->f; a.v = L->v[0]; a.fc = C->f;
    const int TS = (long long)g.lnz * g.lnx >= S->tile32_min_nodes ? 32 : MGT_TS;
    const int own_z = g.lnz - (g.gi0 + g.lnz == g.nz ? 1 : 0), own_x = g.lnx - (g.gj0 + g.lnx == g.nx ? 1 : 0);
    a.tiles_x = (own_x + TS - 1) / TS;
    const dim3 grid((unsigned)(a.tiles_x * ((own_z + TS - 1) / TS)));
    cheb_coeffs(L->lmax, S->cheb_ratio, npre, a.c1, a.c2);
    if (rs) { a.sop = *sop; a.rs = rs; a.z = z; }
#define MGT_PRE(NS, L0, EXT) do { if (TS == 32) hipLaunchKernelGGL((k_mg_pre<NS, L0, 32, EXT>), grid, dim3(mgt_nt(mgt_pre_nn(NS + EXT, 32))), 0, ctx->stream, a); \
                                  else hipLaunchKernelGGL((k_mg_pre<NS, L0, MGT_TS, EXT>), grid, dim3(mgt_nt(mgt_pre_nn(NS + EXT, MGT_TS))), 0, ctx->stream, a); } while (0)
    if (L->dist) {
        (void)pl_halo(ctx, g, (double*)a.f, 2, g.plane, npre + 2);
        if (npre == 1) MGT_PRE(1, false, 1); else if (npre == 2) MGT_PRE(2, false, 1); else MGT_PRE(3, false, 1);
        if (!C->dist) (void)pl_gather_blocks(ctx, C->gh.d, C->f, 2, C->gh.d.plane);
    }
    else if (rs) { if (npre == 1) MGT_PRE(1, true, 0); else if (npre == 2) MGT_PRE(2, true, 0); else MGT_PRE(3, true, 0); }
    else { if (npre == 1) MGT_PRE(1, false, 0); else if (npre == 2) MGT_PRE(2, false, 0); else MGT_PRE(3, false, 0); }
#undef MGT_PRE
    double* ec = nullptr;
    bool wf = false;
    vcycle<double>(ctx, S, l + 1, C->f, &ec, &wf, nullptr, 1.0, 0, nullptr);
    if (L->dist && C->dist) (void)pl_halo(ctx, C->gh.d, ec, 2, C->gh.d.plane, 4);
    a.ec = ec; a.out = final_out ? final_out : L->v[2]; a.oscale = final_out ? final_scale : 1.0; a.out_plane = g.plane;
    cheb_coeffs(L->lmax, S->cheb_ratio, npost, a.c1, a.c2);
#define MGT_POST(NS) do { if (TS == 32) hipLaunchKernelGGL((k_mg_post<NS, 32>), grid, dim3(mgt_nt(mgt_post_nn(NS, 32))), 0, ctx->stream, a); \
                          else hipLaunchKernelGGL((k_mg_post<NS, MGT_TS>), grid, dim3(mgt_nt(mgt_post_nn(NS, MGT_TS))), 0, ctx->stream, a); } while (0)
    if (npost == 1) MGT_POST(1); else if (npost == 2) MGT_POST(2); else MGT_POST(3);
#undef MGT_POST
    *out = final_out ? nullptr : L->v[2];
}

template <typename T>
__global__ __launch_bounds__(256) void k_copy_vel(PlGeom g, const T* __restrict__ e, double* __restrict__ z, double oscale) {
    PL_NODE_PROLOGUE(g)
    (void)i; (void)j;
    z[c] = (double)e[c] * oscale; z[c + g.plane] = (double)e[c + g.plane] * oscale;
}

__global__ __launch_bounds__(256) void k_vv_close_frame(PlVvOp op, double* __restrict__ z) {
    const PlGeom& g = op.g;
    const int t = blockIdx.x * 256 + threadIdx.x;
    int i, j;
    if (t < 3 * g.lnx) { const int q = t / g.lnx; i = q == 0 ? 0 : g.nz - 3 + q; j = g.gj0 + t % g.lnx; }
    else if (t < 3 * g.lnx + 3 * g.lnz) { const int u = t - 3 * g.lnx, q = u / g.lnz; j = q == 0 ? 0 : g.nx - 3 + q; i = g.gi0 + u % g.lnz; }
    else return;
    const int li = i - g.gi0, lj = j - g.gj0;
    if (li < 0 || li >= g.lnz || lj < 0 || lj >= g.lnx) return;
    const long long c = pl_idx(g, li, lj), P = g.plane;
    int moff; double s;
    int cls = vv_cls_z(op, i, j, moff, s);
    if (cls == VV_ZERO) z[c] = 0.0; else if (cls == VV_SLAVE) z[c] = s * z[c + moff];
    cls = vv_cls_x(op, i, j, moff, s);
    if (cls == VV_ZERO) z[c + P] = 0.0; else if (cls == VV_SLAVE) z[c + P] = s * z[c + moff + P];
}

template <typename T>
static int stokes_precond_t(pl_ctx* ctx, PlSolver* S, const double* rs, double* z) {
    PlStokesOp op = ctx->sop;
    MgLevel* L0 = S->levels[0];
    MgLevel* L = L0;
    const PlGeom& g = ctx->sop.g;
    const bool f32 = std::is_same<T, float>::value;
    const double kappa = f32 ? S->kappa : 1.0, fscale = f32 ? S->kappa / S->sigma : 1.0, oscale = f32 ? 1.0 / S->kappa : 1.0;
    int e_last = 0, f_depth = 0;
    const bool deep = level_deep_plan(S, L0, 0, e_last, f_depth);
    ExtViewT<T> V = ext_view<T>(ctx, L0, deep ? f_depth : 0);
    if (L0->dist) {
        if (deep) PL_TRY(pl_halo(ctx, g, (double*)rs, 3, g.plane, f_depth + 1));
        else PL_TRY(pl_halo(ctx, g, (double*)rs + 2 * g.plane, 1, g.plane));
    }
    op.g = V.op.g; op.etas -= V.sh; op.etan -= V.sh; if (op.rho) op.rho -= V.sh;
    op.iKc /= S->schur_scale;
    if constexpr (std::is_same<T, double>::value) {
        if (mg_fused_level_ok(ctx, S, 0)) {
            double* e2 = nullptr;
            vcycle_fused_level(ctx, S, 0, nullptr, &e2, z, 1.0, &op, rs, z);
            PL_HIP(ctx, hipGetLastError());
            S->nprec++;
            return 0;
        }
    }
    int npre0, npost0;
    level_nu(S, 0, npre0, npost0);
    if constexpr (std::is_same<T, double>::value) {
        const double hmean = 0.5 * ((ctx->geom.zc.back() - ctx->geom.zc.front()) / (ctx->nz - 1) + (ctx->geom.xc.back() - ctx->geom.xc.front()) / (ctx->nx - 1));
        const double sig = ctx->sop.Kc / hmean, ik = 1.0 / S->kappa;
        const bool range_ok = std::isfinite(sig) && sig > 0.0 && ik * std::min(1.0, sig) > 1e-30 && ik * std::max(1.0, sig) < 1e22;
        if (S->l0_mixed && S->l0_mixed_now && !S->any_line && range_ok && !L0->dist && !L0->op.szz && g_vv_vec && (g.plane % 2) == 0 && S->levels.size() > 1 && npre0 == 1 && npost0 == 1 &&
            S->fuse_first && ctx->nranks == 1 && !S->levels[1]->dist && !S->levels[1]->f32) {
            MgLevel* C = S->levels[1];
            for (float** q : {&L0->ff, &L0->rf, &L0->vf[0]}) if (!*q) PL_TRY(fmalloc0(ctx, q, (size_t)2 * g.plane * sizeof(float)));
            float* ff = L0->ff; float* rf = L0->rf; float* v1f = L0->vf[0];
            double* vd = L0->v[0];
            PlVvOpT<float> cls{};
            cls.g = L0->op.g; cls.slave_x = L0->op.slave_x; cls.slave_z0 = L0->op.slave_z0; cls.slave_zL = L0->op.slave_zL;
            cls.s0 = (float)L0->op.s0; cls.sL = (float)L0->op.sL;
            const double lmax = L0->lmax, lmin = lmax / S->cheb_ratio, c2 = 1.0 / (0.5 * (lmax + lmin));
            const dim3 rows2 = pl_grid_rows2(g), bl(64, 4);
            hipLaunchKernelGGL(k_prec_stage1_v2<float>, rows2, bl, 0, ctx->stream, op, cls, rs, z, ff, v1f, c2, 1.0, 1.0);
            hipLaunchKernelGGL((k_vv_first2<double, float, float>), dim3(3 * rows2.x + 3 * rows2.y + 2), bl, 0, ctx->stream, L0->op, (const float*)ff, v1f, c2, 2,
                               ctx->sop.anchor_i, ctx->sop.anchor_j, ctx->sop.wall_ps);
            hipLaunchKernelGGL((k_vv_sweep2<1, double, float, float, float>), rows2, bl, 0, ctx->stream, L0->op, (const float*)v1f, (const float*)nullptr,
                               (const float*)ff, rf, 0.0, 0.0, 1.0f);
            hipLaunchKernelGGL((k_vv_restrict<float, double>), grid2d(C->gh.d), bl, 0, ctx->stream, g, C->op, (const float*)rf, C->f, 1.0);
            double* ec = nullptr; bool wf = false;
            vcycle<double>(ctx, S, 1, C->f, &ec, &wf, nullptr, 1.0, 0, nullptr);
            hipLaunchKernelGGL((k_vv_prolong_add<double, double, float>), grid2d(g), bl, 0, ctx->stream, L0->op, C->gh.d, (const double*)ec, (const float*)v1f, vd);
            hipLaunchKernelGGL((k_vv_sweep2<0, double, double, double, float>), rows2, bl, 0, ctx->stream, L0->op, (const double*)vd, (const double*)nullptr,
                               (const float*)ff, z, 0.0, c2, 1.0);
            PL_HIP(ctx, hipGetLastError());
            S->nprec++;
            return 0;
        }
    }
    const bool fuse_first = S->fuse_first && !S->any_line && g_vv_vec && (g.plane % 2) == 0 && S->levels.size() > 1 && npre0 >= 1 && !L0->op.szz;
    const int anchor[2] = {ctx->sop.anchor_i, ctx->sop.anchor_j};
    T* f0 = LevelT<T>::f(L0);
    if (g_vv_vec && (g.plane % 2) == 0) {
        const double lmax = L0->lmax, lmin = lmax / S->cheb_ratio, c2 = 1.0 / (0.5 * (lmax + lmin));
        hipLaunchKernelGGL(k_prec_stage1_v2<T>, pl_grid_rows2(op.g), dim3(64, 4), 0, ctx->stream, op, V.op, rs - V.sh, z - V.sh, f0 - V.sh,
                           fuse_first ? LevelT<T>::v(L0)[2] - V.sh : (T*)nullptr, c2, fscale, kappa);
    } else
        hipLaunchKernelGGL(k_prec_stage1<T>, pl_grid_rows(op.g), dim3(64, 4), 0, ctx->stream, op, V.op, rs - V.sh, z - V.sh, f0 - V.sh,
                           pl_row_iters(op.g), fscale);
    T* e = nullptr;
    bool wrote = false;
    const bool direct = S->levels.size() > 1 && S->nu_post > 0;
    vcycle<T>(ctx, S, 0, f0, &e, &wrote, direct ? z : nullptr, oscale, deep ? f_depth : 0, fuse_first ? anchor : nullptr);
    if (!wrote) hipLaunchKernelGGL(k_copy_vel<T>, grid2d(g), dim3(64, 4), 0, ctx->stream, g, (const T*)e, z, oscale);
    if (f32) hipLaunchKernelGGL(k_vv_close_frame, dim3((3 * g.lnx + 3 * g.lnz + 255) / 256), dim3(256), 0, ctx->stream, L0->op, z);
    PL_HIP(ctx, hipGetLastError());
    S->nprec++;
    return 0;
}
static int stokes_precond(pl_ctx* ctx, PlSolver* S, const double* rs, double* z) {
    return S->levels[0]->f32 ? stokes_precond_t<float>(ctx, S, rs, z) : stokes_precond_t<double>(ctx, S, rs, z);
}

__global__ void k_defl_ysum(PlStokesOp op, const double* __restrict__ rp, double* __restrict__ part);
__global__ void k_defl_init(double* __restrict__ sc);

typedef std::function<int(const double*, double*)> VecOp;

struct BicgVecs { double *r, *rt, *p, *v, *s, *t, *y, *z; double* xbest; double *dx, *r0; };

#define PL_MAX_RESTARTS 4
static int bicgstab(pl_ctx* ctx, PlSolver* S, const PlGeom& g, int np, const VecOp& A, const VecOp* M,
                    const double* b, double* x, bool use_x0, double rtol, int maxit, BicgVecs w,
                    pl_solve_stats* st, double ref_norm = 0.0, double etol = 0.0, int np_vel = 0, const EpiOp* AE = nullptr) {
    const long long n = (long long)np * g.plane;
    const size_t bytes = (size_t)n * sizeof(double);
    double d2[2];
    const bool on_device = !getenv("PYLAMP_HOST_SCALARS");
    static const int shadow_mode = getenv("PYLAMP_SHADOW") ? atoi(getenv("PYLAMP_SHADOW")) : 1;
    const bool fused = AE && M && np == 3 && on_device && ctx->nranks == 1 && !pl_geom_is_dist(g) && krylov_fused_knob() &&
                       (!(etol > 0.0 && np_vel > 0) || np_vel == 2);
    const bool fused_setup = fused && use_x0 && shadow_mode == 1;
    const bool epi_dot1 = fused && krylov_fused_level() >= 2;
    if (fused) PL_TRY(epi_alloc(ctx, S, g));
    const bool lazy_defl = S->defl_lazy && S->defl_active && np == 3 && M;
    double rsum[PL_EPI_NSUM] = {0.0, 0.0, 0.0, 0.0, 0.0, 0.0, 0.0, 0.0};
    if (fused_setup) {
        PlApplyArgs e; e.a1 = b; e.want_xx = (etol > 0.0 && np_vel > 0 && np > np_vel) ? 1 : 0; e.want_ysum = lazy_defl ? 1 : 0;
        PL_TRY(apply_resid(ctx, S, *AE, g, x, w.r0, e, lazy_defl, rsum));
        d2[0] = rsum[PL_RS_BB];
    } else
        PL_TRY(dots(ctx, S, g, np, b, b, nullptr, nullptr, d2));
    double bnorm = std::sqrt(d2[0]);
    if (ref_norm > 0.0 && bnorm > 0.0) bnorm = ref_norm;
    st->iterations = 0; st->converged = 0; st->rel_residual = 0.0;
    if (!(bnorm > 0.0)) {
        PL_HIP(ctx, hipMemsetAsync(x, 0, bytes, ctx->stream));
        st->converged = 1;
        return 0;
    }
    double* dx = x; const double* r0 = b;
    const double* rt = w.rt;
// ... 1202 lines not shown
    if (unsuited) *unsuited = false;
    if (multi && !cheb_ok) {
        if (unsuited) *unsuited = true;
        double ms0 = 0; PL_TRY(pl_timer_stop_ms(ctx, &ms0));
        return 0;
    }
    st->iterations = 0; st->converged = 0; st->rel_residual = 0.0; st->error_estimate = 0.0;
    S->napply = 0;
    double ref = 0.0, hist[4] = {0, 0, 0, 0};
    int it = 0;
    if (multi && E > 0) PL_TRY(pl_halo(ctx, g, (double*)b_dev, 1, g.plane, E));
    for (int pass = 0; pass < 5; pass++) {
        if (multi && E > 0) {
            PL_TRY(pl_halo(ctx, g, x, 1, g.plane, E));
            PL_HIP(ctx, hipMemsetAsync(d, 0, pb, ctx->stream));
        }
        hipLaunchKernelGGL(k_heat_cg_residual, grX, bl, 0, ctx->stream, X.op, b_dev - X.sh, (const double*)(x - X.sh), r - X.sh, dinv - X.sh, z - X.sh, pa - X.sh,
                           d - X.sh, 0, S->hc_part, own);
        hipLaunchKernelGGL(k_heat_cg_scalars, dim3(1), dim3(1024), 0, ctx->stream, nb, (const double*)S->hc_part, sc, 0);
        if (multi) {
            PL_HIP(ctx, hipMemcpyAsync(sc + HC_ALPHA, sc + HC_REF, sizeof(double), hipMemcpyDeviceToDevice, ctx->stream));
            PL_TRY(pl_comm_allreduce_dev(ctx, sc + HC_RZ, 3, 0));
            PL_HIP(ctx, hipMemcpyAsync(sc + HC_REF, sc + HC_ALPHA, sizeof(double), hipMemcpyDeviceToDevice, ctx->stream));
        }
        S->napply++;
        PL_TRY(fetch());
        if (pass == 0 && !multi) read_norms();
        if (pass == 0) ref = std::sqrt(hs[HC_REF]);
        double znorm = std::sqrt(hs[HC_ZZ]);
        if (!(ref > 0.0)) { st->converged = 1; break; }
        st->rel_residual = znorm / ref;
        if (znorm <= rtol * ref || it >= maxit || pass == 4) { st->converged = znorm <= rtol * ref ? 1 : 0; break; }
        double* pold = pa; double* pnew = pbuf;
        bool first = true, ok = true;
        if (cheb_ok) {
            const double sigma = 1.0 / rho_g, target = 0.25 * rtol * ref / znorm;
            int ks = 1; double t0 = 1.0, t1 = sigma;
            while (1.0 / t1 > target && ks < 200) { const double t2 = 2.0 * sigma * t1 - t0; t0 = t1; t1 = t2; ks++; }
            ks = std::min(ks, std::max(maxit - it, 1));
            const double theta = 1.0, delta = rho_g;
            double rho_old = 1.0 / sigma;
            double* bufs[4] = {d, pa, pbuf, S->hc[8]};
            int ext = E - 1;
            auto coef = [&](int k, double* c1, double* c2) {
                if (k == 0) { *c1 = 0.0; *c2 = 1.0 / theta; }
                else { const double rr = 1.0 / (2.0 * sigma - rho_old); *c1 = rr * rho_old; *c2 = 2.0 * rr / delta; rho_old = rr; }
            };
            for (int k = 0; k < ks;) {
                const int kf = fuse ? std::min(ks - k, PL_HEAT_KMAX) : 1;
                if (kf >= 2) {
                    HeatChebCoef cf{};
                    for (int q = 0; q < kf; q++) coef(k + q, &cf.c1[q], &cf.c2[q]);
                    launch_heat_cheb_fused(ctx, kf, hop, bufs[0], bufs[1], r, bufs[2], bufs[3], cf);
                    S->heat_fused_launches++;
                    std::swap(bufs[0], bufs[2]); std::swap(bufs[1], bufs[3]);
                    k += kf; S->napply += kf;
                    continue;
                }
                double c1, c2;
                coef(k, &c1, &c2);
                if (multi && ext < 0) {
                    PL_TRY(pl_halo(ctx, g, S->hc3, 3, g.plane, E));
                    ext = E - 1;
                }
                const HeatExt V = heat_ext(ctx, hop, multi ? ext : 0);
                hipLaunchKernelGGL(k_heat_cheb, grid2d(V.op.g), bl, 0, ctx->stream, V.op, (const double*)(bufs[0] - V.sh), (const double*)(bufs[1] - V.sh),
                                   (const double*)(r - V.sh), (const double*)(dinv - V.sh), bufs[2] - V.sh, c1, c2);
                double* nx = bufs[2]; bufs[2] = bufs[1]; bufs[1] = bufs[0]; bufs[0] = nx;
                ext--;
                k++; S->napply++;
            }
            it += ks;
            hipLaunchKernelGGL(k_add_inplace, grid1d(g.plane), dim3(256), 0, ctx->stream, (long long)g.plane, x, (const double*)bufs[0]);
            close_walls(x);
            continue;
        }
        while (it < maxit) {
            it++;
            hipLaunchKernelGGL(k_heat_cg_apply, gr, bl, 0, ctx->stream, hop, (const double*)z, (const double*)pold, pnew, q, (const double*)sc, first ? 0 : 1, S->hc_part);
            hipLaunchKernelGGL(k_heat_cg_scalars, dim3(1), dim3(1024), 0, ctx->stream, nb, (const double*)S->hc_part, sc, 1);
            hipLaunchKernelGGL(k_heat_cg_update, gr, bl, 0, ctx->stream, g, (const double*)pnew, (const double*)q, (const double*)dinv, d, r, z, (const double*)sc, S->hc_part);
            hipLaunchKernelGGL(k_heat_cg_scalars, dim3(1), dim3(1024), 0, ctx->stream, nb, (const double*)S->hc_part, sc, 2);
            S->napply++;
            std::swap(pold, pnew); first = false;
            if (it + 3 < S->hc_last_its && it < maxit) continue;
            PL_TRY(fetch());
            hist[it & 3] = hs[HC_HS];
            znorm = std::sqrt(hs[HC_ZZ]);
            if (!std::isfinite(znorm) || !(hs[HC_PQ] > 0.0)) { ok = false; break; }
            if (znorm <= rtol * ref) break;
        }
        hipLaunchKernelGGL(k_add_inplace, grid1d(g.plane), dim3(256), 0, ctx->stream, (long long)g.plane, x, (const double*)d);
        close_walls(x);
        if (!ok) break;
    }
    PL_HIP(ctx, hipGetLastError());
    st->iterations = it;
    S->hc_last_its = st->converged ? it : 0;
    if (xmass > 0.0) st->error_estimate = std::sqrt(std::fabs(hist[0]) + std::fabs(hist[1]) + std::fabs(hist[2]) + std::fabs(hist[3])) / std::sqrt(xmass);
    if (cheb_ok && xmass > 0.0 && hs[HC_RZ] >= 0.0) st->error_estimate = std::sqrt(hs[HC_RZ] / (1.0 - rho_g)) / std::sqrt(xmass);
    double ms = 0;
    PL_TRY(pl_timer_stop_ms(ctx, &ms));
    st->solve_ms = ms; st->operator_applies = S->napply; st->precond_applies = 0;
    *x_out = x;
    return 0;
}

int pl_heat_solve_device(pl_ctx* ctx, const double* b_dev, double rtol, int maxit, pl_solve_stats* st,
                         double** x_out, const double* x0_dev) {
    PlSolver* S = solver_of(ctx);
    if (ctx->nz >= 3 && ctx->nx >= 3 && (ctx->nranks == 1 || std::min(ctx->geom.d.lnz, ctx->geom.d.lnx) >= 2)) {
        bool unsuited = false;
        PL_TRY(heat_solve_cg(ctx, S, b_dev, rtol, maxit, st, x_out, x0_dev, &unsuited));
        if (!unsuited) return 0;
    }
    const PlGeom& g = ctx->geom.d;
    size_t pb = (size_t)g.plane * sizeof(double);
    for (int k = 0; k < 11; k++) if (!S->h[k]) PL_TRY(dmalloc0(ctx, &S->h[k], pb));
    PL_TRY(scal_alloc(ctx, S));
    PL_TRY(pl_timer_start(ctx));
    PlHeatOp hop = ctx->hop;
    S->napply = 0;
    VecOp A = [&](const double* in, double* out) -> int {
        PL_TRY(pl_halo(ctx, g, (double*)in, 1, g.plane));
        pl_launch_heat_apply(ctx, hop, in, out, true);
        S->napply++;
        return 0;
    };
    double* b = S->h[8];
    PL_HIP(ctx, hipMemcpyAsync(b, b_dev, pb, hipMemcpyDeviceToDevice, ctx->stream));
    hipLaunchKernelGGL(k_heat_dinv, grid2d(g), dim3(64, 4), 0, ctx->stream, hop, b);
    BicgVecs w{S->h[0], S->h[1], S->h[2], S->h[3], S->h[4], S->h[5], nullptr, nullptr, S->h[6], S->h[9], S->h[10]};
    if (x0_dev) PL_HIP(ctx, hipMemcpyAsync(S->h[7], x0_dev, pb, hipMemcpyDeviceToDevice, ctx->stream));
    PL_TRY(bicgstab(ctx, S, g, 1, A, nullptr, b, S->h[7], x0_dev != nullptr, rtol, maxit, w, st));
    double ms = 0;
    PL_TRY(pl_timer_stop_ms(ctx, &ms));
    st->solve_ms = ms; st->operator_applies = S->napply; st->precond_applies = 0;
    *x_out = S->h[7];
    return 0;
}

extern "C" int pl_heat_fused_launches(pl_ctx* ctx, long long* n) {
    if (!n) return pl_fail(ctx, "pl_heat_fused_launches: n is NULL");
    *n = solver_of(ctx)->heat_fused_launches;
    return 0;
}

extern "C" int pl_mg_tail_launches(pl_ctx* ctx, long long* lds, long long* global) {
    if (!lds || !global) return pl_fail(ctx, "pl_mg_tail_launches: lds or global is NULL");
    *lds = solver_of(ctx)->tail_lds_launches; *global = solver_of(ctx)->tail_global_launches;
    return 0;
}

extern "C" int pl_heat_solve(pl_ctx* ctx, const double* rhs, double* x, double rtol, int maxit,
                             pl_solve_stats* stats) {
    if (!ctx->hop_ready) return pl_fail(ctx, "heat operator not set");
    if (!x) return pl_fail(ctx, "pl_heat_solve: x is NULL");
    PL_HIP(ctx, hipSetDevice(ctx->device));
    const PlGeom& g = ctx->geom.d;
    double* db;
    PL_TRY(pl_buf(ctx, "api_hx", (size_t)g.plane * sizeof(double), &db));
    if (rhs) PL_TRY(pl_plane_upload(ctx, g, rhs, db));
    else pl_launch_heat_rhs(ctx, ctx->hop, ctx->bufs["f_T"], ctx->bufs["H"], db);
    pl_solve_stats st{};
    if (rtol <= 0) rtol = 1e-12;
    if (maxit <= 0) maxit = 2000;
    double* xs = nullptr;
    PL_TRY(pl_heat_solve_device(ctx, db, rtol, maxit, &st, &xs));
    PL_TRY(pl_plane_download(ctx, g, xs, x));
    if (stats) *stats = st;
    return 0;
}
```

pylamp_amd/pylamp_stokes.py:

```python
import ctypes as C

import numpy as np

from .pylamp_const import *
from .pylamp_const import DIM, IZ, IX
from . import _lib
from ._context import get_context

BC_TYPE_NOSLIP = 0
BC_TYPE_FREESLIP = 1
BC_TYPE_CYCLIC = 2
BC_TYPE_FLOWTHRU = 4

DEFAULT_RTOL = 1e-7
DEFAULT_MAXIT = 400


def gidx(idxs, nx, dim):
    if len(idxs) != dim:
        raise Exception("num of idxs != dimensions")
    if dim == 2:
        ret = idxs[IZ] * nx[IX] * (dim + 1) + idxs[IX] * (dim + 1)
    else:
        print("!!! NOT IMPLEMENTED")
        raise Exception("gidx: only 2D is implemented")
    return ret


def x2vp(x, nx):
    dof = int(np.prod(nx)) * (DIM + 1)
    x = np.asarray(x)
    newvel = [[]] * DIM
    for d in range(DIM):
        newvel[d] = x[d:dof:DIM + 1].reshape(nx)
    newpres = x[DIM:dof:DIM + 1].reshape(nx)
    return (newvel, newpres)


class StokesOperator:

    def __init__(self, ctx, nx, coeffs):
        self._ctx = ctx
        self.nx = [int(nx[0]), int(nx[1])]
        n = 3 * self.nx[0] * self.nx[1]
        self.shape = (n, n)
        self.dtype = np.dtype(np.float64)
        self.last_stats = None
        self._coeffs = coeffs
        self._gen = -1
        self._activate()
        kc = C.c_double(); kb = C.c_double()
        ctx.check(ctx.lib.pl_stokes_get_scaling(ctx.handle(), C.byref(kc), C.byref(kb)))
        self.Kcont, self.Kbond = kc.value, kb.value
        ctx.operators.add(self)

    def _activate(self):
        ctx = self._ctx
        if self._gen == ctx.stokes_gen and self._gen >= 0:
            return
        es, en, rho, bc, surfstab, tstep, theta = self._coeffs
        bc_arr = (C.c_int * 4)(*bc)
        ctx.check(ctx.lib.pl_stokes_set_coeffs(ctx.handle(), _lib.dptr(es), _lib.dptr(en), _lib.dptr(rho), bc_arr,
                                               surfstab, tstep, theta))
        ctx.stokes_gen += 1
        self._gen = ctx.stokes_gen

    def matvec(self, x):
        x = _lib.f64(x).reshape(-1)
        if x.size != self.shape[0]:
            raise Exception("dimension mismatch")
        self._activate()
        y = np.empty_like(x)
        self._ctx.check(self._ctx.lib.pl_stokes_apply(self._ctx.handle(), _lib.dptr(x), _lib.dptr(y)))
        return y

    dot = matvec

    def __matmul__(self, x):
        return self.matvec(x)

    def rhs(self):
        self._activate()
        r = np.empty(self.shape[0])
        self._ctx.check(self._ctx.lib.pl_stokes_rhs(self._ctx.handle(), _lib.dptr(r)))
        return r

    def residual_dd(self, rhs, x):
        rhs = _lib.f64(rhs).reshape(-1); x = _lib.f64(x).reshape(-1)
        if x.size != self.shape[0] or rhs.size != self.shape[0]:
            raise Exception("dimension mismatch")
        self._activate()
        r = np.empty_like(x)
        self._ctx.check(self._ctx.lib.pl_stokes_residual_dd(self._ctx.handle(), _lib.dptr(rhs), _lib.dptr(x), _lib.dptr(r)))
        return r

    def direct_info(self):
        band = C.c_int(); nb = C.c_int(); fms = C.c_double(); sms = C.c_double(); ns = C.c_int()
        self._ctx.check(self._ctx.lib.pl_stokes_direct_info(self._ctx.handle(), C.byref(band), C.byref(nb), C.byref(fms), C.byref(sms),
                                                            C.byref(ns)))
        return {"band": band.value, "nb": nb.value, "factor_ms": fms.value, "solve_ms": sms.value, "nsolve": ns.value}

    def precond(self, r):
        r = _lib.f64(r).reshape(-1)
        z = np.empty_like(r)
        self._activate()
        self._ctx.check(self._ctx.lib.pl_stokes_precond_apply(self._ctx.handle(), _lib.dptr(r), _lib.dptr(z)))
        return z

    def mg_info(self):
        n = C.c_int(); lm = (C.c_double * 32)()
        self._ctx.check(self._ctx.lib.pl_stokes_mg_info(self._ctx.handle(), C.byref(n), lm, 32))
        return n.value, [lm[k] for k in range(n.value)]

    def mg_tail_launches(self):
        lds = C.c_longlong(); glob = C.c_longlong()
        self._ctx.check(self._ctx.lib.pl_mg_tail_launches(self._ctx.handle(), C.byref(lds), C.byref(glob)))
        return lds.value, glob.value

    def mg_plan(self):
        n = self.mg_info()[0]
        sm = (C.c_int * 32)(); nu = (C.c_int * 4)(); ratio = C.c_double(); wall = C.c_int()
        self._ctx.check(self._ctx.lib.pl_stokes_mg_plan(self._ctx.handle(), sm, 32, nu, C.byref(ratio), C.byref(wall)))
        return dict(smoother=[sm[k] for k in range(n)], nu=(nu[0], nu[1]), nu0=(nu[2], nu[3]), ratio=ratio.value, wall=bool(wall.value))

    def mg_precision(self):
        n = C.c_int(); nf = C.c_int()
        self._ctx.check(self._ctx.lib.pl_stokes_mg_precision(self._ctx.handle(), C.byref(n), C.byref(nf)))
        return n.value, nf.value

    def set_mg_precision(self, fp32, min_nodes=0):
        self._ctx.check(self._ctx.lib.pl_stokes_set_mg_precision(self._ctx.handle(), int(bool(fp32)), int(min_nodes)))

    def tocsc(self):
        import scipy.sparse as sp
        nz, nxx = self.nx
        ii, jj = np.meshgrid(np.arange(nz), np.arange(nxx), indexing='ij')
        rows, cols, vals = [], [], []
        node = (ii * nxx + jj)
        for ci in range(3):
            for cj in range(3):
                mask = ((ii % 3) == ci) & ((jj % 3) == cj)
                for q in range(3):
                    e = np.zeros((nz, nxx, 3))
                    e[mask, q] = 1.0
                    y = self.matvec(e.reshape(-1)).reshape(nz, nxx, 3)
                    ri, rj, rq = np.nonzero(y)
                    pi = ri + ((ci - ri % 3 + 1) % 3 - 1)
                    pj = rj + ((cj - rj % 3 + 1) % 3 - 1)
                    ok = (pi >= 0) & (pi < nz) & (pj >= 0) & (pj < nxx)
                    rows.append((node[ri, rj] * 3 + rq)[ok])
                    cols.append((pi * nxx + pj)[ok] * 3 + q)
                    vals.append(y[ri, rj, rq][ok])
        A = sp.coo_matrix((np.concatenate(vals), (np.concatenate(rows), np.concatenate(cols))), shape=self.shape)
        return A.tocsc()


def makeStokesMatrix(nx, grid, f_etas, f_etan, f_rho, bc, surfstab=False, tstep=None, surfstab_theta=0.5,
                     strict_reference=True):
    ctx = get_context(nx, grid)
    if surfstab and tstep is None:
        raise Exception("surface stabilization needs predetermined tstep")
    es, en, rho = (np.array(a, dtype=np.float64, order="C") for a in (f_etas, f_etan, f_rho))
    for a in (es, en, rho):
        if a.shape != (int(nx[0]), int(nx[1])):
            raise Exception("field shape does not match nx")
    coeffs = (es, en, rho, [int(b) for b in bc], 1 if surfstab else 0, float(tstep) if tstep is not None else 0.0,
              float(surfstab_theta) if strict_reference else -float(surfstab_theta))
    A = StokesOperator(ctx, nx, coeffs)
    return (A, A.rhs())


def solve(A, rhs, x0=None, rtol=DEFAULT_RTOL, maxit=DEFAULT_MAXIT):
    ctx = A._ctx
    A._activate()
    rhs = _lib.f64(rhs).reshape(-1)
    x = np.zeros_like(rhs) if x0 is None else _lib.f64(x0).reshape(-1).copy()
    st = _lib.SolveStats()
    ctx.check(ctx.lib.pl_stokes_solve(ctx.handle(), _lib.dptr(rhs), _lib.dptr(x), 0 if x0 is None else 1, float(rtol),
                                      int(maxit), C.byref(st)))
    A.last_stats = st.as_dict()
    return x
```

Baseline: 201.4 million.

## Specialize fused multigrid tile kernels for interior tiles and add XCD-aware tile order

Adds a host-computed box of interior tiles per multigrid level, where boundary classification, bounds checks and clamping are provably unnecessary. The pre and post smoothing kernels now dispatch to a specialized IN=true path for those tiles, which skips the classification and masking logic. It also remaps block indices so that neighbouring tiles land on the same XCD, meant to improve L2 locality. This costs more template instantiations and code size, plus extra branching per block and host-side box computation cached by key.

After: 202.2 million (median of 4 runs). Within noise of the previous version (+0.4%).

```diff
diff --git a/include/pylamp_hip.h b/include/pylamp_hip.h
--- a/include/pylamp_hip.h
+++ b/include/pylamp_hip.h
@@ -86,6 +86,7 @@
 int  pl_stokes_mg_precision(pl_ctx* ctx, int* nlevels, int* nlevels_fp32);
 int  pl_stokes_set_mg_precision(pl_ctx* ctx, int fp32, long long min_nodes);
 int  pl_mg_tail_launches(pl_ctx* ctx, long long* lds, long long* global);
+int  pl_mg_interior_tiles(pl_ctx* ctx, long long out[2]);
 
 int  pl_heat_set_coeffs(pl_ctx* ctx, const double* zmp, const double* xmp, const double* T,
                         const double* kz, const double* kx, const double* cp, const double* rho,
diff --git a/pylamp_amd/_lib.py b/pylamp_amd/_lib.py
--- a/pylamp_amd/_lib.py
+++ b/pylamp_amd/_lib.py
@@ -163,6 +163,7 @@
     "pl_stokes_set_mg_precision": (C.c_int, [C.c_void_p, C.c_int, C.c_longlong]),
     "pl_stokes_sweep_bench": (C.c_int, [C.c_void_p, C.c_int, c_double_p]),
     "pl_mg_tail_launches": (C.c_int, [C.c_void_p, C.POINTER(C.c_longlong), C.POINTER(C.c_longlong)]),
+    "pl_mg_interior_tiles": (C.c_int, [C.c_void_p, C.POINTER(C.c_longlong)]),
     "pl_heat_set_coeffs": (C.c_int, [C.c_void_p] + [c_double_p] * 8 + [c_int_p, c_double_p, C.c_double]),
     "pl_heat_apply": (C.c_int, [C.c_void_p, c_double_p, c_double_p]),
     "pl_heat_rhs": (C.c_int, [C.c_void_p, c_double_p]),
diff --git a/pylamp_amd/csrc/pl_solver.hip b/pylamp_amd/csrc/pl_solver.hip
--- a/pylamp_amd/csrc/pl_solver.hip
+++ b/pylamp_amd/csrc/pl_solver.hip
@@ -1321,6 +1321,7 @@
     float *etas_f = nullptr, *etan_f = nullptr, *tab_f = nullptr;
     float* vf[3] = {nullptr, nullptr, nullptr};
     float *ff = nullptr, *rf = nullptr;
+    long long mgt_key[2] = {0, 0}, mgt_in[2] = {0, 0}; int mgt_box[2][4] = {};
 };
 template <typename T> struct LevelT;
 template <> struct LevelT<double> {
@@ -1385,6 +1386,9 @@
     int napply = 0, nprec = 0;
     long long heat_fused_launches = 0;
     long long tail_lds_launches = 0, tail_global_launches = 0;
+    bool mg_xcd_order = true;
+    bool mg_interior = true;
+    long long mgt_tiles_interior = 0, mgt_tiles_rim = 0;
 };
 
 static PlSolver* solver_of(pl_ctx* ctx) {
@@ -1404,6 +1408,8 @@
         if (const char* e = getenv("PYLAMP_MG_FP32_NODES")) { long long v = atoll(e); if (v >= 1) S->f32_min_nodes = v; }
         if (const char* e = getenv("PYLAMP_L0_MIXED")) S->l0_mixed = atoi(e) != 0;
         if (const char* e = getenv("PYLAMP_MG_FUSED")) S->fused = atoi(e) != 0;
+        if (const char* e = getenv("PYLAMP_MG_INTERIOR")) S->mg_interior = atoi(e) != 0;
+        if (const char* e = getenv("PYLAMP_MG_XCD_ORDER")) S->mg_xcd_order = atoi(e) != 0;
         if (const char* e = getenv("PYLAMP_MG_TS32")) { long long v = atoll(e); if (v > 0) S->tile32_min_nodes = v; }
         if (const char* e = getenv("PYLAMP_MG_FUSED_MAX")) { long long v = atoll(e); if (v > 0) S->fused_max_nodes = v; }
         if (const char* e = getenv("PYLAMP_SCHUR_SCALE")) { double v = atof(e); if (v > 0.0) S->schur_scale = v; }
@@ -2120,11 +2126,31 @@
     double c1[4], c2[4];
     PlStokesOp sop; const double* rs; double* z;
     int tiles_x;
+    int ntiles, xcd_order;
+    int in_ty0, in_ty1, in_tx0, in_tx1;
 };
+__device__ inline int mgt_tile_of(const MgTileArgs& a, int b) {
+    if (!a.xcd_order) return b;
+    const int x = b & 7, k = b >> 3, base = a.ntiles >> 3, rem = a.ntiles & 7;
+    return x * base + min(x, rem) + k;
+}
+__device__ inline bool mgt_in_box(const MgTileArgs& a, int tile) {
+    const int ty = tile / a.tiles_x, tx = tile % a.tiles_x;
+    return ty >= a.in_ty0 && ty <= a.in_ty1 && tx >= a.in_tx0 && tx <= a.in_tx1;
+}
+__device__ __forceinline__ void mgt_request_args(const MgTileArgs& a, bool post) {
+    const PlGeom& g = a.op.g;
+    asm volatile("" :: "s"(a.op.etas), "s"(a.op.etan), "s"(a.op.rdz), "s"(a.op.rDz), "s"(a.op.rdx), "s"(a.op.rDx), "s"(a.f),
+                       "s"(g.nz), "s"(g.nx), "s"(g.lnz), "s"(g.lnx), "s"(g.gi0), "s"(g.gj0), "s"(g.pitch), "s"(g.plane));
+    if (post) {
+        const PlGeom& gc = a.opc.g;
+        asm volatile("" :: "s"(a.v), "s"(a.ec), "s"(gc.nz), "s"(gc.nx), "s"(gc.lnz), "s"(gc.lnx), "s"(gc.gi0), "s"(gc.gj0), "s"(gc.pitch), "s"(gc.plane));
+    }
+}
 
 struct MgtTab { const double* es; const double* en; const double* rdz; const double* rDz; const double* rdx; const double* rDx; };
 
-__device__ inline int mgt_cls_z(const PlVvOp& op, int i, int j, int& db, double& s) {
+__host__ __device__ inline int mgt_cls_z(const PlVvOp& op, int i, int j, int& db, double& s) {
     db = 0; s = 1.0;
     if (i <= 0 || i >= op.g.nz - 1 || j < 0 || j >= op.g.nx - 1) return VV_ZERO;
     if (op.slave_x) {
@@ -2133,7 +2159,7 @@
     }
     return VV_INT;
 }
-__device__ inline int mgt_cls_x(const PlVvOp& op, int i, int j, int& da, double& s) {
+__host__ __device__ inline int mgt_cls_x(const PlVvOp& op, int i, int j, int& da, double& s) {
     const double s0 = op.s0, sL = op.sL;
     da = 0; s = 1.0;
     if (j <= 0 || j >= op.g.nx - 1 || i < 0 || i >= op.g.nz - 1) return VV_ZERO;
@@ -2143,10 +2169,11 @@
     return da ? VV_SLAVE : VV_INT;
 }
 struct MgtC { double c0, c1, c2, c3, x0, x1, rdg, s, f; int cm, d; bool on, interior; };
-template <bool ZC>
+template <bool ZC, bool IN = false>
 __device__ inline MgtC mgt_classify(const PlVvOp& op, int CR, int NR, int ci0, int cj0, int a, int b) {
     MgtC k; k.c0 = k.c1 = k.c2 = k.c3 = k.x0 = k.x1 = k.rdg = k.f = 0.0; k.s = 1.0; k.cm = a * CR + b; k.d = 0; k.on = false; k.interior = false;
     if (a < 1 || a > NR - 2 || b < 1 || b > CR - 2) return k;
+    if (IN) { k.on = true; k.interior = true; return k; }
     int d; double s;
     const int cls = ZC ? mgt_cls_z(op, ci0 + a, cj0 + b, d, s) : mgt_cls_x(op, ci0 + a, cj0 + b, d, s);
     const int am = ZC ? a : a + d, bm = ZC ? b + d : b;
@@ -2186,29 +2213,44 @@
     return k.c0 * (vx[c + 1] - v0) - k.c1 * (v0 - vx[c - 1]) + k.c2 * (vx[c + CR] - v0) - k.c3 * (v0 - vx[c - CR]) +
            k.x0 * (vz[c + CR] - vz[c + CR - 1]) - k.x1 * (vz[c] - vz[c - 1]);
 }
+template <bool IN = false>
 __device__ inline void mgt_cheb(const MgtC& kz, const MgtC& kx, int CR, const double* vz, const double* vx, double& pvz, double& pvx,
                                 double c1, double c2, double& oz, double& ox) {
     oz = 0.0; ox = 0.0;
-    if (kz.on) {
+    if (IN || kz.on) {
         double v0; const double Av = mgt_av_z(kz, CR, vz, vx, v0);
         const double mom = (c1 != 0.0) ? c1 * (v0 - pvz) : 0.0;
         oz = kz.s * (v0 + mom + (c2 * (Av - kz.f)) * kz.rdg);
         pvz = v0;
     }
-    if (kx.on) {
+    if (IN || kx.on) {
         double v0; const double Av = mgt_av_x(kx, CR, vz, vx, v0);
         const double mom = (c1 != 0.0) ? c1 * (v0 - pvx) : 0.0;
         ox = kx.s * (v0 + mom + (c2 * (Av - kx.f)) * kx.rdg);
         pvx = v0;
     }
 }
-__device__ inline bool mgt_owns(int ra, int rb, int HC, int TS, int i, int j, const PlGeom& g) {
+__host__ __device__ inline bool mgt_owns(int ra, int rb, int HC, int TS, int i, int j, const PlGeom& g) {
     return ra >= HC && (ra < HC + TS || (ra == HC + TS && i == g.nz - 1)) && rb >= HC && (rb < HC + TS || (rb == HC + TS && j == g.nx - 1));
 }
 __host__ __device__ constexpr int mgt_npt(int nn) { return (nn + 1023) / 1024; }
 __host__ __device__ constexpr int mgt_nt(int nn) { return ((nn + mgt_npt(nn) - 1) / mgt_npt(nn) + 63) / 64 * 64; }
 __host__ __device__ constexpr int mgt_pre_nn(int NS, int TS) { return (TS + 2 * (NS + 2)) * (TS + 2 * (NS + 2)); }
 __host__ __device__ constexpr int mgt_post_nn(int NS, int TS) { return (TS + 2 * (NS + 1)) * (TS + 2 * (NS + 1)); }
+
+__host__ __device__ inline bool mgt_rows_interior(const PlVvOp& op, int i, int j) {
+    int d; double s;
+    return mgt_cls_z(op, i, j, d, s) == VV_INT && mgt_cls_x(op, i, j, d, s) == VV_INT &&
+           i >= op.g.gi0 && i < op.g.gi0 + op.g.lnz && j >= op.g.gj0 && j < op.g.gj0 + op.g.lnx;
+}
+__host__ __device__ inline bool mgt_tile_interior(const PlVvOp& op, const PlVvOp& opc, int TS, int HC, int ty, int tx) {
+    const PlGeom& g = op.g;
+    const int ti0 = g.gi0 + ty * TS, tj0 = g.gj0 + tx * TS, ci0 = ti0 - HC, cj0 = tj0 - HC, CR = TS + 2 * HC;
+    if (!mgt_rows_interior(op, ci0, cj0) || !mgt_rows_interior(op, ci0 + CR - 1, cj0 + CR - 1)) return false;
+    if (mgt_owns(HC + TS, HC, HC, TS, ti0 + TS, tj0, g) || mgt_owns(HC, HC + TS, HC, TS, ti0, tj0 + TS, g)) return false;
+    const int eI0 = ((ci0 + 1) >> 1) - 2, eJ0 = ((cj0 + 1) >> 1) - 2, ECR = TS / 2 + HC + 5;
+    return mgt_rows_interior(opc, eI0, eJ0) && mgt_rows_interior(opc, eI0 + ECR - 1, eJ0 + ECR - 1);
+}
 
 template <int NPT> struct MgtRawE { double es[NPT], en[NPT], tab; };
 template <int NPT> struct MgtRawF { double fz[NPT], fx[NPT]; };
@@ -2216,12 +2258,12 @@
 struct MgtRawC { double ez, ex; };
 #define MGT_SLOT(q) const int idx = tid + (q) * NT; const bool have = idx < CR * CR; \
     const int ra = have ? idx / CR : 0, rb = have ? idx % CR : 0, i = ci0 + ra, j = cj0 + rb; \
-    const bool inmem = have && i - g.gi0 >= -PL_RING && i - g.gi0 < g.lnz + PL_RING && j - g.gj0 >= -PL_RING && j - g.gj0 < g.lnx + PL_RING; \
+    const bool inmem = have && (IN || (i - g.gi0 >= -PL_RING && i - g.gi0 < g.lnz + PL_RING && j - g.gj0 >= -PL_RING && j - g.gj0 < g.lnx + PL_RING)); \
     const long long c = inmem ? pl_idx(g, i - g.gi0, j - g.gj0) : pl_idx(g, 0, 0);
 #define MGT_TAB_SLOT const int w = __builtin_amdgcn_readfirstlane(tid >> 6), k = tid & 63; \
     const int gk = (w < 2 ? ci0 : cj0) - 1 + k, n = w < 2 ? g.nz : g.nx; \
-    const bool intab = w < 4 && k < CR + 3 && gk >= -PL_TOFF && gk < n + PL_TOFF;
-template <int NPT, int NT, int CR, int HC, int TS>
+    const bool intab = w < 4 && k < CR + 3 && (IN || (gk >= -PL_TOFF && gk < n + PL_TOFF));
+template <int NPT, int NT, int CR, int HC, int TS, bool IN>
 __device__ inline void mgt_fetch_visc(MgtRawE<NPT>& r, const MgTileArgs& a, int tile, int tid) {
     static_assert(CR + 3 <= 64 && NT >= 256, "one table per wave");
     const PlGeom& g = a.op.g;
@@ -2235,7 +2277,7 @@
         r.es[q] = a.op.etas[c]; r.en[q] = a.op.etan[c];
     }
 }
-template <int NPT, int NT, int CR, int HC, int TS>
+template <int NPT, int NT, int CR, int HC, int TS, bool IN>
 __device__ inline void mgt_store_visc(const MgtRawE<NPT>& r, const MgTileArgs& a, int tile, double* es, double* en, double* tab, int tid) {
     const PlGeom& g = a.op.g;
     const int ci0 = g.gi0 + tile / a.tiles_x * TS - HC, cj0 = g.gj0 + tile % a.tiles_x * TS - HC;
@@ -2248,21 +2290,21 @@
     MGT_TAB_SLOT
     if (w < 4 && k < CR + 3) tab[w * (CR + 4) + k] = intab ? r.tab : 0.0;
 }
-template <int NPT, int NT, int CR, int HC, int TS>
+template <int NPT, int NT, int CR, int HC, int TS, bool IN>
 __device__ inline void mgt_fetch_rhs(MgtRawF<NPT>& r, const MgTileArgs& a, const double* fsrc, int tile, int tid) {
     const PlGeom& g = a.op.g;
     const int ci0 = g.gi0 + tile / a.tiles_x * TS - HC, cj0 = g.gj0 + tile % a.tiles_x * TS - HC;
 #pragma unroll
     for (int q = 0; q < NPT; q++) {
         MGT_SLOT(q)
-        const MgtC kz = mgt_classify<true>(a.op, CR, CR, ci0, cj0, ra, rb), kx = mgt_classify<false>(a.op, CR, CR, ci0, cj0, ra, rb);
+        const MgtC kz = mgt_classify<true, IN>(a.op, CR, CR, ci0, cj0, ra, rb), kx = mgt_classify<false, IN>(a.op, CR, CR, ci0, cj0, ra, rb);
         const long long c0 = pl_idx(g, 0, 0), cn = pl_idx(g, i - g.gi0, j - g.gj0);
         (void)c;
         r.fz[q] = fsrc[kz.on ? cn + kz.d : c0];
         r.fx[q] = fsrc[(kx.on ? cn + (long long)kx.d * g.pitch : c0) + g.plane];
     }
 }
-template <int NPT, int NT, int CR, int HC, int TS>
+template <int NPT, int NT, int CR, int HC, int TS, bool IN>
 __device__ inline void mgt_fetch_v(MgtRawV<NPT>& r, const MgTileArgs& a, int tile, int tid) {
     const PlGeom& g = a.op.g;
     const int ci0 = g.gi0 + tile / a.tiles_x * TS - HC, cj0 = g.gj0 + tile % a.tiles_x * TS - HC;
@@ -2272,7 +2314,7 @@
         r.vz[q] = a.v[c]; r.vx[q] = a.v[c + g.plane];
     }
 }
-template <int NPT, int NT, int CR, int HC, int TS>
+template <int NPT, int NT, int CR, int HC, int TS, bool IN>
 __device__ inline void mgt_store_v(const MgtRawV<NPT>& r, const MgTileArgs& a, int tile, double* pvz, double* pvx, int tid) {
     const PlGeom& g = a.op.g;
     const int ci0 = g.gi0 + tile / a.tiles_x * TS - HC, cj0 = g.gj0 + tile % a.tiles_x * TS - HC;
@@ -2285,15 +2327,15 @@
 }
 #define MGT_EC_SLOT const PlGeom& gc = a.opc.g; \
     const int e = min(tid, ECR * ECR - 1), I = ((a.op.g.gi0 + tile / a.tiles_x * TS - H) >> 1) - 2 + e / ECR, J = ((a.op.g.gj0 + tile % a.tiles_x * TS - H) >> 1) - 2 + e % ECR; \
-    const bool inmem = I - gc.gi0 >= -PL_RING && I - gc.gi0 < gc.lnz + PL_RING && J - gc.gj0 >= -PL_RING && J - gc.gj0 < gc.lnx + PL_RING; \
+    const bool inmem = IN || (I - gc.gi0 >= -PL_RING && I - gc.gi0 < gc.lnz + PL_RING && J - gc.gj0 >= -PL_RING && J - gc.gj0 < gc.lnx + PL_RING); \
     const long long cc = inmem ? pl_idx(gc, I - gc.gi0, J - gc.gj0) : pl_idx(gc, 0, 0);
-template <int NT, int TS, int H, int ECR>
+template <int NT, int TS, int H, int ECR, bool IN>
 __device__ inline void mgt_fetch_ec(MgtRawC& r, const MgTileArgs& a, int tile, int tid) {
     static_assert(ECR * ECR <= NT, "one node of the coarse window per thread");
     MGT_EC_SLOT
     r.ez = a.ec[cc]; r.ex = a.ec[cc + gc.plane];
 }
-template <int NT, int TS, int H, int ECR>
+template <int NT, int TS, int H, int ECR, bool IN>
 __device__ inline void mgt_store_ec(const MgtRawC& r, const MgTileArgs& a, int tile, double* ecz, double* ecx, int tid) {
     MGT_EC_SLOT
     (void)cc;
@@ -2303,12 +2345,16 @@
 #undef MGT_SLOT
 #undef MGT_TAB_SLOT
 
-template <int NS, bool L0, int TS, int EXT = 0>
-__global__ __launch_bounds__(mgt_nt(mgt_pre_nn(NS + EXT, TS))) void k_mg_pre(MgTileArgs a) {
+template <int NN, int ZN, int CR> struct MgtPreLds {
+    double V[2][2][NN];
+    double ZP[ZN];
+    double TAB[4][CR + 4];
+};
+template <int NS, bool L0, int TS, int EXT, bool IN>
+__device__ __forceinline__ void mgt_pre_tile(const MgTileArgs& a, int tile, MgtPreLds<mgt_pre_nn(NS + EXT, TS), L0 ? mgt_pre_nn(NS + EXT, TS) : 1, TS + 2 * (NS + 2 + EXT)>& lds) {
     constexpr int H = NS + 1 + EXT, HC = H + 1, CR = TS + 2 * HC, NN = CR * CR, NPT = mgt_npt(NN), NT = mgt_nt(NN);
-    __shared__ double V[2][2][NN];
-    __shared__ double ZP[L0 ? NN : 1];
-    __shared__ double TAB[4][CR + 4];
+    static_assert(!IN || (!L0 && !EXT), "level 0 and distributed levels keep the general path");
+    auto& V = lds.V; auto& ZP = lds.ZP; auto& TAB = lds.TAB;
     double* const ES = V[1][0]; double* const EN = V[1][1];
     const PlGeom& g = a.op.g;
     const int tid = threadIdx.x;
@@ -2317,10 +2363,10 @@
     const double* const fsrc = L0 ? a.rs : a.f;
     MgtRawE<NPT> rawe;
     MgtRawF<NPT> rawf;
-    mgt_fetch_visc<NPT, NT, CR, HC, TS>(rawe, a, blockIdx.x, tid);
-    mgt_fetch_rhs<NPT, NT, CR, HC, TS>(rawf, a, fsrc, blockIdx.x, tid);
-    mgt_store_visc<NPT, NT, CR, HC, TS>(rawe, a, blockIdx.x, ES, EN, TAB[0], tid);
-    const int tile = blockIdx.x, ty = tile / a.tiles_x, tx = tile % a.tiles_x;
+    mgt_fetch_visc<NPT, NT, CR, HC, TS, IN>(rawe, a, tile, tid);
+    mgt_fetch_rhs<NPT, NT, CR, HC, TS, IN>(rawf, a, fsrc, tile, tid);
+    mgt_store_visc<NPT, NT, CR, HC, TS, IN>(rawe, a, tile, ES, EN, TAB[0], tid);
+    const int ty = tile / a.tiles_x, tx = tile % a.tiles_x;
     const int ti0 = g.gi0 + ty * TS, tj0 = g.gj0 + tx * TS;
     const int ci0 = ti0 - HC, cj0 = tj0 - HC;
     MgtC kz[NPT], kx[NPT];
@@ -2331,10 +2377,10 @@
         const bool have = idx < NN;
         const int ra = have ? idx / CR : 0, rb = have ? idx % CR : 0, i = ci0 + ra, j = cj0 + rb;
         depth[q] = have ? min(min(ra, CR - 1 - ra), min(rb, CR - 1 - rb)) : -1;
-        kz[q] = mgt_classify<true>(a.op, CR, CR, ci0, cj0, ra, rb);
-        kx[q] = mgt_classify<false>(a.op, CR, CR, ci0, cj0, ra, rb);
-        if (kz[q].on) kz[q].f = rawf.fz[q];
-        if (kx[q].on) kx[q].f = rawf.fx[q];
+        kz[q] = mgt_classify<true, IN>(a.op, CR, CR, ci0, cj0, ra, rb);
+        kx[q] = mgt_classify<false, IN>(a.op, CR, CR, ci0, cj0, ra, rb);
+        if (IN || kz[q].on) kz[q].f = rawf.fz[q];
+        if (IN || kx[q].on) kx[q].f = rawf.fx[q];
         if (L0 && have) {
             const long long c = pl_idx(g, i - g.gi0, j - g.gj0);
             const bool indom = i >= 0 && i < g.nz && j >= 0 && j < g.nx;
@@ -2361,8 +2407,8 @@
     for (int q = 0; q < NPT; q++) {
         const int idx = tid + q * NT;
         if (depth[q] >= HC - H) {
-            V[0][0][idx] = kz[q].on ? (-kz[q].s * a.c2[0] * kz[q].f) * kz[q].rdg : 0.0;
-            V[0][1][idx] = kx[q].on ? (-kx[q].s * a.c2[0] * kx[q].f) * kx[q].rdg : 0.0;
+            V[0][0][idx] = (IN || kz[q].on) ? (-kz[q].s * a.c2[0] * kz[q].f) * kz[q].rdg : 0.0;
+            V[0][1][idx] = (IN || kx[q].on) ? (-kx[q].s * a.c2[0] * kx[q].f) * kx[q].rdg : 0.0;
         }
     }
     __syncthreads();
@@ -2377,7 +2423,7 @@
             const int idx = tid + q * NT;
             if (depth[q] >= HC - h) {
                 double oz, ox;
-                mgt_cheb(kz[q], kx[q], CR, V[cur][0], V[cur][1], pvz[q], pvx[q], a.c1[k], a.c2[k], oz, ox);
+                mgt_cheb<IN>(kz[q], kx[q], CR, V[cur][0], V[cur][1], pvz[q], pvx[q], a.c1[k], a.c2[k], oz, ox);
                 V[cur ^ 1][0][idx] = oz; V[cur ^ 1][1][idx] = ox;
             }
         }
@@ -2390,15 +2436,15 @@
         const int idx = tid + q * NT;
         if (depth[q] >= HC - 1) {
             double v0, rz = 0.0, rx = 0.0;
-            if (kz[q].interior) rz = kz[q].f - mgt_av_z(kz[q], CR, V[cur][0], V[cur][1], v0);
-            if (kx[q].interior) rx = kx[q].f - mgt_av_x(kx[q], CR, V[cur][0], V[cur][1], v0);
+            if (IN || kz[q].interior) rz = kz[q].f - mgt_av_z(kz[q], CR, V[cur][0], V[cur][1], v0);
+            if (IN || kx[q].interior) rx = kx[q].f - mgt_av_x(kx[q], CR, V[cur][0], V[cur][1], v0);
             V[nxt][0][idx] = rz; V[nxt][1][idx] = rx;
         }
-        if (depth[q] >= HC - (EXT ? NS : 1)) {
+        if (depth[q] >= HC - (IN ? 0 : EXT ? NS : 1)) {
             const int ra = idx / CR, rb = idx % CR, i = ci0 + ra, j = cj0 + rb, li = i - g.gi0, lj = j - g.gj0;
             const bool owned = li >= 0 && li < g.lnz && lj >= 0 && lj < g.lnx;
             const bool ring = EXT && !owned && li >= -NS && li < g.lnz + NS && lj >= -NS && lj < g.lnx + NS;
-            if (i >= 0 && i < g.nz && j >= 0 && j < g.nx && ((owned && mgt_owns(ra, rb, HC, TS, i, j, g)) || ring)) {
+            if (IN || (i >= 0 && i < g.nz && j >= 0 && j < g.nx && ((owned && mgt_owns(ra, rb, HC, TS, i, j, g)) || ring))) {
                 const long long c = pl_idx(g, li, lj);
                 a.v[c] = V[cur][0][idx]; a.v[c + P] = V[cur][1][idx];
             }
@@ -2406,22 +2452,23 @@
     }
     __syncthreads();
     const PlGeom& gc = a.opc.g;
-    for (int idx = tid; idx < (TS / 2 + 1) * (TS / 2 + 1); idx += NT) {
-        const int u_ = idx / (TS / 2 + 1), w_ = idx % (TS / 2 + 1);
+    constexpr int RW = TS / 2 + (IN ? 0 : 1);
+    for (int idx = tid; idx < RW * RW; idx += NT) {
+        const int u_ = idx / RW, w_ = idx % RW;
         const int I = (ti0 >> 1) + u_, J = (tj0 >> 1) + w_;
-        if ((u_ == TS / 2 && I != gc.nz - 1) || (w_ == TS / 2 && J != gc.nx - 1)) continue;
-        if (I >= gc.nz || J >= gc.nx || 2 * I - g.gi0 >= g.lnz || 2 * J - g.gj0 >= g.lnx) continue;
+        if (!IN && ((u_ == TS / 2 && I != gc.nz - 1) || (w_ == TS / 2 && J != gc.nx - 1))) continue;
+        if (!IN && (I >= gc.nz || J >= gc.nx || 2 * I - g.gi0 >= g.lnz || 2 * J - g.gj0 >= g.lnx)) continue;
         const int b0 = (2 * I - ci0) * CR + (2 * J - cj0);
         int d; double s;
         double oz = 0.0, ox = 0.0;
-        if (vv_cls_z(a.opc, I, J, d, s) == VV_INT) {
+        if (IN || vv_cls_z(a.opc, I, J, d, s) == VV_INT) {
             const double wz[3] = {0.25, 0.5, 0.25}, wx[4] = {0.125, 0.375, 0.375, 0.125};
 #pragma unroll
             for (int u = 0; u < 3; u++)
 #pragma unroll
                 for (int w = 0; w < 4; w++) oz += wz[u] * wx[w] * V[nxt][0][b0 + (u - 1) * CR + (w - 1)];
         }
-        if (vv_cls_x(a.opc, I, J, d, s) == VV_INT) {
+        if (IN || vv_cls_x(a.opc, I, J, d, s) == VV_INT) {
             const double wz[4] = {0.125, 0.375, 0.375, 0.125}, wx[3] = {0.25, 0.5, 0.25};
 #pragma unroll
             for (int u = 0; u < 4; u++)
@@ -2432,13 +2479,30 @@
         a.fc[cc] = oz; a.fc[cc + gc.plane] = ox;
     }
 }
-
-template <int NS, int TS>
-__global__ __launch_bounds__(mgt_nt(mgt_post_nn(NS, TS))) void k_mg_post(MgTileArgs a) {
-    constexpr int H = NS, HC = H + 1, CR = TS + 2 * HC, NN = CR * CR, ECR = TS / 2 + H + 6, ENN = ECR * ECR, NPT = mgt_npt(NN), NT = mgt_nt(NN);
-    __shared__ double V[2][2][NN];
-    __shared__ double EC[2][ENN];
-    __shared__ double TAB[4][CR + 4];
+template <int NS, bool L0, int TS, int EXT = 0>
+__global__ __launch_bounds__(mgt_nt(mgt_pre_nn(NS + EXT, TS))) void k_mg_pre(MgTileArgs a) {
+    constexpr int HC = NS + 2 + EXT, NN = mgt_pre_nn(NS + EXT, TS);
+    __shared__ MgtPreLds<NN, L0 ? NN : 1, TS + 2 * HC> lds;
+    const int tile = mgt_tile_of(a, blockIdx.x);
+    if constexpr (!L0 && !EXT) {
+        mgt_request_args(a, false);
+        if (mgt_in_box(a, tile)) {
+            mgt_pre_tile<NS, L0, TS, EXT, true>(a, tile, lds);
+            return;
+        }
+    }
+    mgt_pre_tile<NS, L0, TS, EXT, false>(a, tile, lds);
+}
+
+template <int NN, int ENN, int CR> struct MgtPostLds {
+    double V[2][2][NN];
+    double EC[2][ENN];
+    double TAB[4][CR + 4];
+};
+template <int NS, int TS, bool IN>
+__device__ __forceinline__ void mgt_post_tile(const MgTileArgs& a, int tile, MgtPostLds<mgt_post_nn(NS, TS), (TS / 2 + NS + 6) * (TS / 2 + NS + 6), TS + 2 * (NS + 1)>& lds) {
+    constexpr int H = NS, HC = H + 1, CR = TS + 2 * HC, NN = CR * CR, ECR = TS / 2 + H + 6, NPT = mgt_npt(NN), NT = mgt_nt(NN);
+    auto& V = lds.V; auto& EC = lds.EC; auto& TAB = lds.TAB;
     double* const ES = V[0][0]; double* const EN = V[0][1];
     double* const PVz = V[1][0]; double* const PVx = V[1][1];
     const PlGeom& g = a.op.g; const PlGeom& gc = a.opc.g;
@@ -2448,14 +2512,14 @@
     MgtRawC rawc;
     MgtRawE<NPT> rawe;
     MgtRawF<NPT> rawf;
-    mgt_fetch_v<NPT, NT, CR, HC, TS>(rawv, a, blockIdx.x, tid);
-    mgt_fetch_ec<NT, TS, H, ECR>(rawc, a, blockIdx.x, tid);
-    mgt_fetch_visc<NPT, NT, CR, HC, TS>(rawe, a, blockIdx.x, tid);
-    mgt_fetch_rhs<NPT, NT, CR, HC, TS>(rawf, a, a.f, blockIdx.x, tid);
-    mgt_store_v<NPT, NT, CR, HC, TS>(rawv, a, blockIdx.x, PVz, PVx, tid);
-    mgt_store_ec<NT, TS, H, ECR>(rawc, a, blockIdx.x, EC[0], EC[1], tid);
-    mgt_store_visc<NPT, NT, CR, HC, TS>(rawe, a, blockIdx.x, ES, EN, TAB[0], tid);
-    const int tile = blockIdx.x, ty = tile / a.tiles_x, tx = tile % a.tiles_x;
+    mgt_fetch_v<NPT, NT, CR, HC, TS, IN>(rawv, a, tile, tid);
+    mgt_fetch_ec<NT, TS, H, ECR, IN>(rawc, a, tile, tid);
+    mgt_fetch_visc<NPT, NT, CR, HC, TS, IN>(rawe, a, tile, tid);
+    mgt_fetch_rhs<NPT, NT, CR, HC, TS, IN>(rawf, a, a.f, tile, tid);
+    mgt_store_v<NPT, NT, CR, HC, TS, IN>(rawv, a, tile, PVz, PVx, tid);
+    mgt_store_ec<NT, TS, H, ECR, IN>(rawc, a, tile, EC[0], EC[1], tid);
+    mgt_store_visc<NPT, NT, CR, HC, TS, IN>(rawe, a, tile, ES, EN, TAB[0], tid);
+    const int ty = tile / a.tiles_x, tx = tile % a.tiles_x;
     const int ti0 = g.gi0 + ty * TS, tj0 = g.gj0 + tx * TS;
     const int ci0 = ti0 - HC, cj0 = tj0 - HC;
     const int eI0 = ((ti0 - H) >> 1) - 2, eJ0 = ((tj0 - H) >> 1) - 2;
@@ -2467,10 +2531,10 @@
         const bool have = idx < NN;
         const int ra = have ? idx / CR : 0, rb = have ? idx % CR : 0;
         depth[q] = have ? min(min(ra, CR - 1 - ra), min(rb, CR - 1 - rb)) : -1;
-        kz[q] = mgt_classify<true>(a.op, CR, CR, ci0, cj0, ra, rb);
-        kx[q] = mgt_classify<false>(a.op, CR, CR, ci0, cj0, ra, rb);
-        if (kz[q].on) kz[q].f = rawf.fz[q];
-        if (kx[q].on) kx[q].f = rawf.fx[q];
+        kz[q] = mgt_classify<true, IN>(a.op, CR, CR, ci0, cj0, ra, rb);
+        kx[q] = mgt_classify<false, IN>(a.op, CR, CR, ci0, cj0, ra, rb);
+        if (IN || kz[q].on) kz[q].f = rawf.fz[q];
+        if (IN || kx[q].on) kx[q].f = rawf.fx[q];
     }
     __syncthreads();
 #pragma unroll
@@ -2483,21 +2547,21 @@
         const int idx = tid + q * NT;
         if (depth[q] >= HC - H) {
             const int ra = idx / CR, rb = idx % CR, i = ci0 + ra, j = cj0 + rb;
-            int d; double s;
+            int d = 0; double s = 1.0;
             double oz = 0.0, ox = 0.0;
-            if (mgt_cls_z(a.op, i, j, d, s) != VV_ZERO) {
+            if (IN || mgt_cls_z(a.op, i, j, d, s) != VV_ZERO) {
                 const int jm = j + d;
                 const int I0 = i >> 1, I1 = (i + 1) >> 1;
                 int Jn = jm >> 1, Jo = (jm & 1) ? Jn + 1 : Jn - 1;
-                Jn = min(max(Jn, 0), gc.nx - 2); Jo = min(max(Jo, 0), gc.nx - 2);
+                if (!IN) { Jn = min(max(Jn, 0), gc.nx - 2); Jo = min(max(Jo, 0), gc.nx - 2); }
                 const double pa = 0.5 * (ecz(I0, Jn) + ecz(I1, Jn)), pb = 0.5 * (ecz(I0, Jo) + ecz(I1, Jo));
                 oz = s * (PVz[idx + d] + (0.75 * pa + 0.25 * pb));
             }
-            if (mgt_cls_x(a.op, i, j, d, s) != VV_ZERO) {
+            if (IN || mgt_cls_x(a.op, i, j, d, s) != VV_ZERO) {
                 const int im = i + d;
                 const int J0 = j >> 1, J1 = (j + 1) >> 1;
                 int In = im >> 1, Io = (im & 1) ? In + 1 : In - 1;
-                In = min(max(In, 0), gc.nz - 2); Io = min(max(Io, 0), gc.nz - 2);
+                if (!IN) { In = min(max(In, 0), gc.nz - 2); Io = min(max(Io, 0), gc.nz - 2); }
                 const double pa = 0.5 * (ecx(In, J0) + ecx(In, J1)), pb = 0.5 * (ecx(Io, J0) + ecx(Io, J1));
                 ox = s * (PVx[idx + d * CR] + (0.75 * pa + 0.25 * pb));
             }
@@ -2517,10 +2581,10 @@
             const int idx = tid + q * NT;
             if (depth[q] >= HC - h) {
                 double oz, ox;
-                mgt_cheb(kz[q], kx[q], CR, V[cur][0], V[cur][1], pvz[q], pvx[q], k == 0 ? 0.0 : a.c1[k], a.c2[k], oz, ox);
+                mgt_cheb<IN>(kz[q], kx[q], CR, V[cur][0], V[cur][1], pvz[q], pvx[q], k == 0 ? 0.0 : a.c1[k], a.c2[k], oz, ox);
                 if (k == NS - 1) {
                     const int ra = idx / CR, rb = idx % CR, i = ci0 + ra, j = cj0 + rb;
-                    if (i < g.nz && j < g.nx && i - g.gi0 < g.lnz && j - g.gj0 < g.lnx) {
+                    if (IN || (i < g.nz && j < g.nx && i - g.gi0 < g.lnz && j - g.gj0 < g.lnx)) {
                         const long long c = pl_idx(g, i - g.gi0, j - g.gj0); a.out[c] = oz * a.oscale; a.out[c + a.out_plane] = ox * a.oscale;
                     }
                 } else { V[cur ^ 1][0][idx] = oz; V[cur ^ 1][1][idx] = ox; }
@@ -2528,6 +2592,7 @@
         }
         if (k < NS - 1) { __syncthreads(); cur ^= 1; }
     }
+    if (IN) return;
 #pragma unroll
     for (int q = 0; q < NPT; q++) {
         const int idx = tid + q * NT;
@@ -2538,6 +2603,15 @@
             }
         }
     }
+}
+template <int NS, int TS>
+__global__ __launch_bounds__(mgt_nt(mgt_post_nn(NS, TS))) void k_mg_post(MgTileArgs a) {
+    constexpr int HC = NS + 1, ECR = TS / 2 + NS + 6;
+    __shared__ MgtPostLds<mgt_post_nn(NS, TS), ECR * ECR, TS + 2 * HC> lds;
+    const int tile = mgt_tile_of(a, blockIdx.x);
+    mgt_request_args(a, true);
+    if (mgt_in_box(a, tile)) mgt_post_tile<NS, TS, true>(a, tile, lds);
+    else mgt_post_tile<NS, TS, false>(a, tile, lds);
 }
 
 #define MGT_TAIL_POOL 18600
@@ -2831,6 +2905,27 @@
         if (k == 0) { c1[k] = 0.0; c2[k] = 1.0 / theta; }
         else { const double rho = 1.0 / (2.0 * sigma - rho_old); c1[k] = rho * rho_old; c2[k] = 2.0 * rho / delta; rho_old = rho; }
     }
+}
+static long long mgt_interior_box(MgLevel* L, const PlVvOp& opc, int which, int TS, int HC, int tiles_z, MgTileArgs& a) {
+    const PlVvOp& op = L->op;
+    const int tiles_x = a.tiles_x;
+    const long long key = 1 + TS + 64LL * HC + 4096LL * (op.slave_x + 2 * op.slave_z0 + 4 * op.slave_zL + 8 * opc.slave_x + 16 * opc.slave_z0 + 32 * opc.slave_zL) +
+                          (1LL << 20) * tiles_x + (1LL << 40) * tiles_z;
+    int* b = L->mgt_box[which];
+    if (L->mgt_key[which] != key) {
+        b[0] = tiles_z; b[1] = -1; b[2] = tiles_x; b[3] = -1;
+        long long n = 0;
+        for (int ty = 0; ty < tiles_z; ty++)
+            for (int tx = 0; tx < tiles_x; tx++)
+                if (mgt_tile_interior(op, opc, TS, HC, ty, tx)) {
+                    n++; b[0] = std::min(b[0], ty); b[1] = std::max(b[1], ty); b[2] = std::min(b[2], tx); b[3] = std::max(b[3], tx);
+                }
+        if (n != (long long)(b[1] - b[0] + 1) * (b[3] - b[2] + 1)) n = 0;
+        if (n == 0) { b[0] = 1; b[1] = 0; b[2] = 1; b[3] = 0; }
+        L->mgt_key[which] = key; L->mgt_in[which] = n;
+    }
+    a.in_ty0 = b[0]; a.in_ty1 = b[1]; a.in_tx0 = b[2]; a.in_tx1 = b[3];
+    return L->mgt_in[which];
 }
 static bool mg_fused_level_ok(pl_ctx* ctx, const PlSolver* S, size_t l) {
     if (!S->fused || l + 1 >= S->levels.size() || S->any_line) return false;
@@ -2865,7 +2960,15 @@
     const int TS = (long long)g.lnz * g.lnx >= S->tile32_min_nodes ? 32 : MGT_TS;
     const int own_z = g.lnz - (g.gi0 + g.lnz == g.nz ? 1 : 0), own_x = g.lnx - (g.gj0 + g.lnx == g.nx ? 1 : 0);
     a.tiles_x = (own_x + TS - 1) / TS;
-    const dim3 grid((unsigned)(a.tiles_x * ((own_z + TS - 1) / TS)));
+    const int tiles_z = (own_z + TS - 1) / TS;
+    const dim3 grid((unsigned)(a.tiles_x * tiles_z));
+    const bool interior = S->mg_interior && !L->dist;
+    a.ntiles = (int)grid.x; a.xcd_order = S->mg_xcd_order ? 1 : 0;
+    a.in_ty0 = a.in_tx0 = 1; a.in_ty1 = a.in_tx1 = 0;
+    {
+        const long long n = interior && !rs ? mgt_interior_box(L, C->op, 0, TS, npre + 2, tiles_z, a) : 0;
+        S->mgt_tiles_interior += n; S->mgt_tiles_rim += (long long)grid.x - n;
+    }
     cheb_coeffs(L->lmax, S->cheb_ratio, npre, a.c1, a.c2);
     if (rs) { a.sop = *sop; a.rs = rs; a.z = z; }
 #define MGT_PRE(NS, L0, EXT) do { if (TS == 32) hipLaunchKernelGGL((k_mg_pre<NS, L0, 32, EXT>), grid, dim3(mgt_nt(mgt_pre_nn(NS + EXT, 32))), 0, ctx->stream, a); \
@@ -2884,6 +2987,11 @@
     if (L->dist && C->dist) (void)pl_halo(ctx, C->gh.d, ec, 2, C->gh.d.plane, 4);
     a.ec = ec; a.out = final_out ? final_out : L->v[2]; a.oscale = final_out ? final_scale : 1.0; a.out_plane = g.plane;
     cheb_coeffs(L->lmax, S->cheb_ratio, npost, a.c1, a.c2);
+    {
+        a.in_ty0 = a.in_tx0 = 1; a.in_ty1 = a.in_tx1 = 0;
+        const long long n = interior ? mgt_interior_box(L, C->op, 1, TS, npost + 1, tiles_z, a) : 0;
+        S->mgt_tiles_interior += n; S->mgt_tiles_rim += (long long)grid.x - n;
+    }
 #define MGT_POST(NS) do { if (TS == 32) hipLaunchKernelGGL((k_mg_post<NS, 32>), grid, dim3(mgt_nt(mgt_post_nn(NS, 32))), 0, ctx->stream, a); \
                           else hipLaunchKernelGGL((k_mg_post<NS, MGT_TS>), grid, dim3(mgt_nt(mgt_post_nn(NS, MGT_TS))), 0, ctx->stream, a); } while (0)
     if (npost == 1) MGT_POST(1); else if (npost == 2) MGT_POST(2); else MGT_POST(3);
@@ -4392,6 +4500,12 @@
     return 0;
 }
 
+extern "C" int pl_mg_interior_tiles(pl_ctx* ctx, long long out[2]) {
+    if (!out) return pl_fail(ctx, "pl_mg_interior_tiles: out is NULL");
+    out[0] = solver_of(ctx)->mgt_tiles_interior; out[1] = solver_of(ctx)->mgt_tiles_rim;
+    return 0;
+}
+
 extern "C" int pl_heat_solve(pl_ctx* ctx, const double* rhs, double* x, double rtol, int maxit,
                              pl_solve_stats* stats) {
     if (!ctx->hop_ready) return pl_fail(ctx, "heat operator not set");
diff --git a/pylamp_amd/pylamp_stokes.py b/pylamp_amd/pylamp_stokes.py
--- a/pylamp_amd/pylamp_stokes.py
+++ b/pylamp_amd/pylamp_stokes.py
@@ -117,6 +117,11 @@
         self._ctx.check(self._ctx.lib.pl_mg_tail_launches(self._ctx.handle(), C.byref(lds), C.byref(glob)))
         return lds.value, glob.value
 
+    def mg_interior_tiles(self):
+        n = (C.c_longlong * 2)()
+        self._ctx.check(self._ctx.lib.pl_mg_interior_tiles(self._ctx.handle(), n))
+        return n[0], n[1]
+
     def mg_plan(self):
         n = self.mg_info()[0]
         sm = (C.c_int * 32)(); nu = (C.c_int * 4)(); ratio = C.c_double(); wall = C.c_int()
```
